# AssemblyAI-Community/MinImagen

Hardware: NVIDIA B200
Metric: denoising steps/sec (SR256 U-Net, batch 32 per GPU per step) (higher is better)
Workload: dtype f16 tensor-core operands, f32 accumulate / residual stream

## Files before the change

### include/minimagen_b200.h

```cpp
#ifndef MINIMAGEN_B200_H_
#define MINIMAGEN_B200_H_

#include <stdint.h>

#ifdef __cplusplus
extern "C" {
#endif

#define MI_ABI_VERSION 2

int mi_abi_version(void);
const char* mi_last_error(void);
int mi_device_ok(void);
int mi_set_launch_mode(int programmatic_dependent_launch);

int mi_pack_conv_weight_f16(const float* w_oihw, int c_out, int c_in, int kh, int kw, float scale, void* out_f16,
                            void* stream);

int mi_pack_conv_weight_dgrad_f16(const float* w_oihw, int c_out, int c_in, int kh, int kw, void* out_f16, void* stream);

int mi_conv2d_igemm_supported(int H, int W, int c_in, int c_out);
int mi_conv2d_igemm_f16(const void* act_f16, int B, int H, int W, int lda, int c_off, int c_in, const void* act2_f16,
                        int lda2, int c_off2, int c_in1, const void* w_f16, int c_out, int kh, int kw, int mode,
                        const float* bias, const float* residual, float* out_f32, void* out_f16, double* out_stats,
                        long long out_sb, long long out_sh, long long out_sw, long long out_sc, int n_valid,
                        int block_n, int* err_flag, void* workspace, long long workspace_bytes, void* stream);
int mi_conv3x3_res1x1_supported(int H, int W, int c_in, int c_out, int x_cin);
int mi_conv3x3_res1x1_f16(const void* act_f16, int B, int H, int W, int lda, int c_in, const void* act2_f16, int lda2,
                          int c_in1, const void* x_f16, int ldx, int x_cin, const void* x2_f16, int ldx2, int x_cin1,
                          const void* w_f16, int c_out, const float* bias, const float* residual, float* out_f32,
                          void* out_f16, double* out_stats, int* err_flag, void* stream);
long long mi_conv2d_igemm_workspace_bytes(void);

int mi_conv3x3_gn_supported(int H, int W, int c0, int c1, int c_out, int groups);
int mi_conv3x3_gn_silu_f16(const float* src0, int c0, const float* src1, int c1, float scale1, int B, int H, int W,
                           int groups, const double* stats0, const double* stats1, const float* gamma,
                           const float* beta, const float* scale_shift, int scale_shift_ld, float eps,
                           const void* w_f16, int c_out, const float* bias, const float* residual, float* out_f32,
                           void* out_f16, double* out_stats, int* err_flag, void* stream);

int mi_conv2d_direct_f32(const float* in, int B, int Hin, int Win, int c_in, int ldi, const float* w_oihw, int c_out,
                         int kh, int kw, int stride, int pad, const float* bias, const float* residual, float* out,
                         int Hout, int Wout, long long out_sb, long long out_sh, long long out_sw, long long out_sc,
                         void* stream);

int mi_gn_stats(const void* src0, int c0, const void* src1, int c1, float scale1, int in_is_f16, int B, int hw,
                int groups, double* sums, void* stream);
int mi_gn_apply_silu(const void* src0, int c0, const void* src1, int c1, float scale1, int in_is_f16, int B, int hw,
                     int groups, const double* stats0, int stats0_block, const double* stats1, int stats1_block,
                     const float* gamma, const float* beta, const float* scale_shift, int scale_shift_ld, float eps,
                     void* out, int out_is_f16, void* stream);
int mi_cast_act(const void* src0, int c0, const void* src1, int c1, float scale1, int in_is_f16, int B, int H, int W,
                int mode, void* out, int out_is_f16, void* stream);
int mi_ln_rows(const float* in, long long rows, int C, const float* gamma, const float* beta, float eps, int pre_gelu,
               const float* residual, float* out_f32, void* out_f16, void* stream);

int mi_linear_f32(const float* in, int M, int K, const float* W, const float* bias, int N, int in_act, int out_act,
                  const float* addend, float* out_f32, void* out_f16, float out_scale, void* stream);
int mi_sinusoidal_posemb(const long long* t, int B, int dim, float* out, void* stream);
int mi_text_tokens(const float* proj, int B, int L, int D, const uint8_t* mask, const uint8_t* keep,
                   const float* null_embed, int max_len, float* c_out, int m, int row_off, float* pooled,
                   void* stream);
int mi_place_rows(const float* src, int B, int r, int D, float* dst, int m, int row_off, void* stream);
int mi_select_rows(const float* a, const float* null_row, const uint8_t* keep, const float* addend, int B, int N,
                   float* out, void* stream);
int mi_nchw_to_nhwc(const float* a, int ca, const float* b, int cb, int B, int hw, int c_pad, float* out,
                    void* stream);

int mi_stem_unroll_f16(const float* a, int ca, const float* b, int cb, int B, int H, int W, void* out_f16,
                       void* stream);
int mi_silu_f32(const float* in, long long n, float* out, void* stream);

int mi_resize_separable(const float* in, long long planes, int h_in, int w_in, float* out, int h_out, int w_out,
                        const int* iy, const float* wy, int taps_y, const int* ix, const float* wx, int taps_x,
                        int has_clamp, float lo, float hi, void* stream);

long long mi_attention_workspace_bytes(int B, int heads, int kv_head_stride, int m);
int mi_attention_fwd(const void* q_f16, long long q_bs, int ldq, const void* k_f16, const void* v_f16, long long kv_bs,
                     int ldkv, int kv_head_stride, const float* null_kv, const uint8_t* key_mask, int B, int heads,
                     int n, int m, void* out_f16, long long o_bs, int ldo, void* workspace, long long workspace_bytes,
                     void* stream);

int mi_step_x0(const float* x_t, const float* eps_cond, const float* eps_null, float cond_scale, const long long* t,
               const float* sqrt_recip_alphas_cumprod, const float* sqrt_recipm1_alphas_cumprod, int B, int n,
               float* x0, void* stream);
int mi_step_quantile(const float* x0, int B, int n, int rank_lo, int rank_hi, float weight, float min_s, float* s,
                     void* stream);
int mi_step_posterior(const float* x0, const float* x_t, const float* noise, const float* s, const long long* t,
                      const float* posterior_mean_coef1, const float* posterior_mean_coef2, const float* sigma, int B,
                      int n, float* out, void* stream);
long long mi_step_epilogue_workspace_floats(int B, int n);
int mi_step_epilogue(const float* x_t, const float* eps_cond, const float* eps_null, float cond_scale, const long long* t,
                     const float* sqrt_recip_alphas_cumprod, const float* sqrt_recipm1_alphas_cumprod,
                     const float* posterior_mean_coef1, const float* posterior_mean_coef2, const float* sigma,
                     const float* noise, int B, int n, int rank_lo, int rank_hi, float weight, float min_s, float* out,
                     float* s_out, float* x0_workspace, void* stream);
int mi_step_advance_t(long long* t, int B, void* stream);
int mi_step_finalize(const float* x, long long n, int unnormalize, float* out, void* stream);
int mi_q_sample(const float* x0, const float* noise, const long long* t, const float* sqrt_alphas_cumprod,
                const float* sqrt_one_minus_alphas_cumprod, int B, int n, float post_scale, float post_shift,
                float* out, void* stream);


int mi_gemm_f32(const float* A, const float* B, float* C, int M, int N, int K, long long a_sm, long long a_sk,
                long long b_sk, long long b_sn, long long c_sm, long long c_sn, int Z1, int Z2, long long a_b1,
                long long a_b2, long long b_b1, long long b_b2, long long c_b1, long long c_b2, float alpha,
                int accumulate, void* stream);
int mi_colsum_f32(const float* x, long long M, int N, float* out, int accumulate, void* stream);
int mi_conv2d_dgrad_f32(const float* dy, int B, int Hout, int Wout, int c_out, const float* w_oihw, int c_in, int kh, int kw,
                        int stride, int pad, float* dx, int Hin, int Win, void* stream);
int mi_conv2d_wgrad_f32(const float* dy, const float* x, int B, int Hin, int Win, int c_in, int Hout, int Wout, int c_out,
                        int kh, int kw, int stride, int pad, float* dw, void* stream);
int mi_conv2d_wgrad_f16_supported(int Hout, int Wout, int c_in, int c_out, int kh, int kw, int stride);
long long mi_conv2d_wgrad_f16_workspace_bytes(int B, int Hout, int Wout, int c_in, int c_out, int kh, int kw, int stride);
int mi_conv2d_wgrad_f16(const void* dy_f16, const void* x_f16, int B, int Hout, int Wout, int c_in, int c_out, int kh, int kw,
                        int stride, float* dw, float* workspace, long long workspace_bytes, void* stream);
int mi_gn_silu_bwd(const float* x, const float* dy, const double* sums, int B, int hw, int C, int groups,
                   const float* gamma, const float* beta, const float* scale_shift, int scale_shift_ld, float eps,
                   float* dx, float* dgamma, float* dbeta, float* d_scale_shift, int d_scale_shift_ld, float* workspace,
                   void* stream);
int mi_ln_rows_bwd(const float* in, const float* dy, long long rows, int C, const float* gamma, float eps, int pre_gelu,
                   float* dx, float* dgamma, float* dbeta, void* stream);
int mi_softmax_rows(float* s, long long R, int L, void* stream);
int mi_softmax_rows_bwd(const float* P, float* dP, long long R, int L, void* stream);
int mi_upsample2x_bwd(const float* dy, int B, int H, int W, int C, float* dx, void* stream);

#ifdef __cplusplus
}
#endif
#endif
```

### minimagen_b200/Unet.py

```python
from typing import Union

import torch
from torch import nn

from .helpers import cast_tuple, default, exists, prob_mask_like
from .layers import (Attention, Cat, Context, Conv2d, CrossEmbedLayer, Downsample, Identity, Parallel, ResnetBlock,
                     SinusoidalPosEmb, TokenView, TransformerBlock, Upsample, _no_grad_check, _ResidualAttention)
from . import _native
from .ops import get_ops
from .t5 import get_encoded_dim

F32 = torch.float32


class Unet(nn.Module):
    def __init__(
            self,
            *,
            dim: int = 128,
            dim_mults: tuple = (1, 2, 4),
            channels: int = 3,
            channels_out: int = None,
            cond_dim: int = None,
            text_embed_dim=get_encoded_dim('t5_small'),
# ... 57 lines not shown

        self.skip_connect_scale = 2 ** -0.5
        self.downs = nn.ModuleList([])
        self.ups = nn.ModuleList([])
        layer_params = [num_resnet_blocks, resnet_groups, layer_attns, layer_cross_attns]
        reversed_layer_params = list(map(reversed, layer_params))

        skip_connect_dims = []
        for ind, ((dim_in, dim_out), n_blocks, groups, layer_attn, layer_cross_attn) in enumerate(
                zip(in_out, *layer_params)):
            is_last = ind == (num_resolutions - 1)
            layer_cond_dim = cond_dim if layer_cross_attn else None
            transformer_klass = TransformerBlock if layer_attn else Identity
            current_dim = dim_in
            pre_downsample = None
            if memory_efficient:
                pre_downsample = Downsample(dim_in, dim_out)
                current_dim = dim_out
            skip_connect_dims.append(current_dim)
            post_downsample = None
            if not memory_efficient:
                post_downsample = Downsample(current_dim, dim_out) if not is_last else Parallel(
                    Conv2d(dim_in, dim_out, 3, padding=1), Conv2d(dim_in, dim_out, 1))
            self.downs.append(nn.ModuleList([
                pre_downsample,
                ResnetBlock(current_dim, current_dim, cond_dim=layer_cond_dim, time_cond_dim=time_cond_dim,
                            groups=groups),
                nn.ModuleList([ResnetBlock(current_dim, current_dim, time_cond_dim=time_cond_dim, groups=groups)
                               for _ in range(n_blocks)]),
                transformer_klass(dim=current_dim, heads=attn_heads, dim_head=ATTN_DIM_HEAD),
                post_downsample,
            ]))

        mid_dim = dims[-1]
        self.mid_block1 = ResnetBlock(mid_dim, mid_dim, cond_dim=cond_dim, time_cond_dim=time_cond_dim,
                                      groups=resnet_groups[-1])
        self.mid_attn = TokenView(_ResidualAttention(
            Attention(mid_dim, heads=attn_heads, dim_head=ATTN_DIM_HEAD))) if attend_at_middle else None
        self.mid_block2 = ResnetBlock(mid_dim, mid_dim, cond_dim=cond_dim, time_cond_dim=time_cond_dim,
                                      groups=resnet_groups[-1])

        for ind, ((dim_in, dim_out), n_blocks, groups, layer_attn, layer_cross_attn) in enumerate(
                zip(reversed(in_out), *reversed_layer_params)):
            is_last = ind == (num_resolutions - 1)
            layer_cond_dim = cond_dim if layer_cross_attn else None
            transformer_klass = TransformerBlock if layer_attn else Identity
            skip_connect_dim = skip_connect_dims.pop()
            self.ups.append(nn.ModuleList([
                ResnetBlock(dim_out + skip_connect_dim, dim_out, cond_dim=layer_cond_dim,
                            time_cond_dim=time_cond_dim, groups=groups),
                nn.ModuleList([ResnetBlock(dim_out + skip_connect_dim, dim_out, time_cond_dim=time_cond_dim,
                                           groups=groups) for _ in range(n_blocks)]),
                transformer_klass(dim=dim_out, heads=attn_heads, dim_head=ATTN_DIM_HEAD),
                Upsample(dim_out, dim_in) if not is_last or memory_efficient else Identity()
            ]))

        self.init_conv_to_final_conv_residual = False
        self.final_res_block = ResnetBlock(dim, dim, time_cond_dim=time_cond_dim, groups=resnet_groups[0])
        self.final_conv = Conv2d(dim, self.channels_out, 3, padding=3 // 2)

    def _cast_model_parameters(self, *, lowres_cond, text_embed_dim, channels, channels_out):
        if lowres_cond == self.lowres_cond and channels == self.channels and \
                text_embed_dim == self.text_embed_dim and channels_out == self.channels_out:
            return self
        updated = dict(lowres_cond=lowres_cond, text_embed_dim=text_embed_dim, channels=channels,
                       channels_out=channels_out)
        return self.__class__(**{**self._locals, **updated})

    def forward(self, x, time, *, lowres_cond_img=None, lowres_noise_times=None, text_embeds=None, text_mask=None,
                cond_drop_prob: float = 0.):
        return self._forward_impl(x, time, lowres_cond_img=lowres_cond_img, lowres_noise_times=lowres_noise_times,
                                  text_embeds=text_embeds, text_mask=text_mask, cond_drop_prob=cond_drop_prob)

    def _forward_impl(self, x, *args, **kwargs):
        with _native.device_of(x):
            if torch.is_grad_enabled() and (x.requires_grad or any(p.requires_grad for p in self.parameters())):
                from .train_path import unet_forward_train
                return unet_forward_train(self, x, *args, **kwargs)
            return self._forward_dev(x, *args, **kwargs)

    def _forward_dev(self, x, time, *, lowres_cond_img=None, lowres_noise_times=None, text_embeds=None, text_mask=None,
                      cond_drop_prob: float = 0., cond_keep=None):
        assert not (self.lowres_cond and not exists(lowres_cond_img)), \
            'low resolution conditioning image must be present'
        assert not (self.lowres_cond and not exists(lowres_noise_times)), \
            'low resolution conditioning noise time must be present'
        B, Cx, H, W = x.shape
        device = x.device
        x = x.to(F32).contiguous()
        lowres = lowres_cond_img.to(F32).contiguous() if exists(lowres_cond_img) else None

        t, time_tokens = self._generate_t_tokens(time, lowres_noise_times)
        t, c = self._text_condition(text_embeds, B, cond_drop_prob, device, text_mask, t, time_tokens, cond_keep)
        ss = self._all_scale_shifts(t)

        out = torch.empty((B, self.channels_out, H, W), dtype=F32, device=device)
        chunks = self._batch_chunks(B, x.is_cuda)
        if len(chunks) == 1:
            self._forward_body(x, lowres, t, c, ss, out)
            return out
        main = torch.cuda.current_stream(device)
        streams = self._side_streams(len(chunks), device)
        for (b0, b1), s in zip(chunks, streams):
            s.wait_stream(main)
            with torch.cuda.stream(s):
                self._forward_body(x[b0:b1], lowres[b0:b1] if exists(lowres) else None, t[b0:b1], c[b0:b1],
                                   {k: v[b0:b1] for k, v in ss.items()}, out[b0:b1])
        for s in streams:
            main.wait_stream(s)
        return out

    batch_streams = 1
    min_chunk_batch = 8

    def _batch_chunks(self, B, is_cuda):
        n = self.batch_streams if is_cuda else 1
        while n > 1 and (B % n != 0 or B // n < self.min_chunk_batch):
            n -= 1
        per = B // n
        return [(i * per, (i + 1) * per) for i in range(n)]

    def _side_streams(self, n, device):
        key = (n, str(device))
        if getattr(self, "_streams_key", None) != key:
            self._streams = [torch.cuda.Stream(device=device) for _ in range(n)]
            self._streams_key = key
        return self._streams

    def _forward_body(self, x, lowres, t, c, ss, out):
        from . import layers as _layers
        ops = get_ops()
        B, _, H, W = x.shape
        device = x.device
        ctx = Context(c)
        n_res = sum(1 for m in self.modules() if isinstance(m, ResnetBlock))
        if x.is_cuda:
            _layers._ARENA = _layers.ZeroArena(device, B * (self.dim * max(8, 1)) // 8 * 4 * (2 * n_res + 8))
        try:
            return self._forward_body_impl(x, lowres, t, c, ss, out, ctx)
        finally:
            _layers._ARENA = None

    def _forward_body_impl(self, x, lowres, t, c, ss, out, ctx):
        ops = get_ops()
        B, _, H, W = x.shape
        device = x.device

        h = self.init_conv.run_stem(x, lowres)

        hiddens = []
        for pre_downsample, init_block, resnet_blocks, attn_block, post_downsample in self.downs:
            if exists(pre_downsample):
                h = pre_downsample.run(h)
            h = init_block.run(h, t, ctx, ss[init_block])
            for resnet_block in resnet_blocks:
                h = resnet_block.run(h, t, None, ss[resnet_block])
                hiddens.append(h)
            h = attn_block.run(h)
            hiddens.append(h)
            if exists(post_downsample):
                h = post_downsample.run(h)

        h = self.mid_block1.run(h, t, ctx, ss[self.mid_block1])
        if exists(self.mid_attn):
            h = self.mid_attn.run(h)
        h = self.mid_block2.run(h, t, ctx, ss[self.mid_block2])

        skip = lambda cur: Cat(cur, hiddens.pop(), self.skip_connect_scale)
        for init_block, resnet_blocks, attn_block, upsample in self.ups:
            h = init_block.run(skip(h), t, ctx, ss[init_block])
            for resnet_block in resnet_blocks:
                h = resnet_block.run(skip(h), t, None, ss[resnet_block])
            h = attn_block.run(h)
            h = upsample.run(h)

        h = self.final_res_block.run(h, t, None, ss[self.final_res_block], out_f32=False)

        fc = self.final_conv
        if ops.igemm_supported(H, W, fc.in_channels, 16):
            fc.run_prepared_nchw(h.need_f16(), B, H, W, out)
        else:
            fc.run_prepared_nchw(h.need_f32(), B, H, W, out)

    def _all_scale_shifts(self, t):
        from .layers import ResnetBlock
        ops = get_ops()
        blocks = [m for m in self.modules() if isinstance(m, ResnetBlock) and exists(m.time_mlp)]
        key = tuple((m.time_mlp[1].weight.data_ptr(), m.time_mlp[1].weight._version, m.time_mlp[1].bias._version)
                    for m in blocks)
        if getattr(self, "_tm_key", None) != key:
            self._tm_w = torch.cat([m.time_mlp[1].weight.detach() for m in blocks], dim=0).contiguous()
            self._tm_b = torch.cat([m.time_mlp[1].bias.detach() for m in blocks], dim=0).contiguous()
            self._tm_key = key
        B, tcd = t.shape
        total = self._tm_w.shape[0]
        st = torch.empty_like(t)
        ops.silu(t.contiguous(), st)
        buf = torch.empty((B, total), dtype=F32, device=t.device)
        ops.linear_f32(st, B, tcd, self._tm_w, self._tm_b, total, 0, 0, None, buf, None)
        out, off = {}, 0
        for m in blocks:
            n = m.time_mlp[1].out_features
            out[m] = buf[:, off:off + n]
            off += n
        return out

    def forward_with_cond_scale(self, *args, cond_scale: float = 1., **kwargs):
        logits = self.forward(*args, **kwargs)
        if cond_scale == 1:
            return logits
        null_logits = self.forward(*args, cond_drop_prob=1., **kwargs)
        return null_logits + (logits - null_logits) * cond_scale

    def _time_branch(self, times, hiddens_seq, cond_seq, tokens_seq, t_addend):
        ops = get_ops()
        B = times.shape[0]
        dev = times.device
        tcd, D, nt = self.time_cond_dim, self.cond_dim, self.num_time_tokens
        pos = hiddens_seq[0](times)
        lin = hiddens_seq[1]
        hid = torch.empty((B, tcd), dtype=F32, device=dev)
        ops.linear_f32(pos, B, lin.in_features, lin.weight, lin.bias, tcd, 0, 1, None, hid, None)
        lin = cond_seq[0]
        t = torch.empty((B, tcd), dtype=F32, device=dev)
        ops.linear_f32(hid, B, tcd, lin.weight, lin.bias, tcd, 0, 0, t_addend, t, None)
        lin = tokens_seq[0]
        tok = torch.empty((B, nt * D), dtype=F32, device=dev)
        ops.linear_f32(hid, B, tcd, lin.weight, lin.bias, nt * D, 0, 0, None, tok, None)
        return t, tok.reshape(B, nt, D)

    def _generate_t_tokens(self, time, lowres_noise_times):
        t, tokens = self._time_branch(time, self.to_time_hiddens, self.to_time_cond, self.to_time_tokens, None)
        if self.lowres_cond:
            t, lowres_tokens = self._time_branch(lowres_noise_times, self.to_lowres_time_hiddens,
                                                 self.to_lowres_time_cond, self.to_lowres_time_tokens, t)
            tokens = torch.cat((tokens, lowres_tokens), dim=-2)
        return t, tokens

    def _text_condition(self, text_embeds, batch_size, cond_drop_prob, device, text_mask, t, time_tokens, cond_keep=None):
        ops = get_ops()
        B, D, tcd = batch_size, self.cond_dim, self.time_cond_dim
        nt = time_tokens.shape[1]
        has_text = exists(text_embeds)
        m = nt + (self.max_text_len if has_text else 0)
        c_pre = torch.empty((B, m, D), dtype=F32, device=device)
        ops.place_rows(time_tokens.contiguous(), B, nt, D, c_pre, m, 0)
        if has_text:
            L, E = text_embeds.shape[1], text_embeds.shape[2]
            proj = self._static_text_proj(text_embeds)
            if proj is None:
                proj = torch.empty((B * L, D), dtype=F32, device=device)
                ops.linear_f32(text_embeds.to(F32).contiguous().reshape(B * L, E), B * L, E, self.text_to_cond.weight,
                               self.text_to_cond.bias, D, 0, 0, None, proj, None)
            keep = (cond_keep.to(device=device, dtype=torch.uint8).contiguous() if exists(cond_keep)
                    else prob_mask_like((B,), 1 - cond_drop_prob, device=device).to(torch.uint8))
            mask_u8 = text_mask.to(torch.uint8).contiguous() if exists(text_mask) else None
            pooled = torch.empty((B, D), dtype=F32, device=device)
            ops.text_tokens(proj, B, L, D, mask_u8, keep, self.null_text_embed.detach().reshape(self.max_text_len, D),
                            self.max_text_len, c_pre, m, nt, pooled)
            ln, lin1, _, lin2 = self.to_text_non_attn_cond
            pn = torch.empty((B, D), dtype=F32, device=device)
            ops.ln_rows(pooled, B, D, ln.weight, ln.bias, ln.eps, 0, None, pn, None)
            h1 = torch.empty((B, tcd), dtype=F32, device=device)
            ops.linear_f32(pn, B, D, lin1.weight, lin1.bias, tcd, 0, 1, None, h1, None)
            h2 = torch.empty((B, tcd), dtype=F32, device=device)
            ops.linear_f32(h1, B, tcd, lin2.weight, lin2.bias, tcd, 0, 0, None, h2, None)
            t_new = torch.empty((B, tcd), dtype=F32, device=device)
            ops.select_rows(h2, self.null_text_hidden.detach().reshape(tcd), keep, t, B, tcd, t_new)
            t = t_new
        c = torch.empty((B, m, D), dtype=F32, device=device)
        ops.ln_rows(c_pre.reshape(B * m, D), B * m, D, self.norm_cond.weight, self.norm_cond.bias, self.norm_cond.eps,
                    0, None, c.reshape(B * m, D), None)
        return t, c


    def register_static_text(self, text_embeds):
        ops = get_ops()
        B, L, E = text_embeds.shape
        cache = self.__dict__.setdefault("_static_text", {})
        entry = cache.get(text_embeds.data_ptr())
        buf = entry[0] if entry is not None and entry[0].shape == (B * L, self.cond_dim) else \
            torch.empty((B * L, self.cond_dim), dtype=F32, device=text_embeds.device)
        with _native.device_of(text_embeds):
            ops.linear_f32(text_embeds.reshape(B * L, E), B * L, E, self.text_to_cond.weight, self.text_to_cond.bias,
                           self.cond_dim, 0, 0, None, buf, None)
        cache[text_embeds.data_ptr()] = (buf, text_embeds._version, self.text_to_cond.weight._version)
        return buf

    def unregister_static_text(self, text_embeds=None):
        cache = self.__dict__.get("_static_text", {})
        if text_embeds is None:
            cache.clear()
        else:
            cache.pop(text_embeds.data_ptr(), None)

    def _static_text_proj(self, text_embeds):
        entry = self.__dict__.get("_static_text", {}).get(text_embeds.data_ptr())
        if entry is None or text_embeds.dtype != F32 or not text_embeds.is_contiguous():
            return None
        buf, version, wversion = entry
        B, L, _ = text_embeds.shape
        if version != text_embeds._version or wversion != self.text_to_cond.weight._version or buf.shape[0] != B * L:
            return None
        return buf


class Base(Unet):
    defaults = dict(
        dim=512,
        dim_mults=(1, 2, 3, 4),
# ... 51 lines not shown
```

### minimagen_b200/_native.py

```python
import ctypes
import os
from ctypes import c_char_p, c_float, c_int, c_longlong, c_void_p

import torch

_HERE = os.path.dirname(os.path.abspath(__file__))
LIB_PATH = os.path.join(_HERE, "lib", "libminimagen_b200.so")

_P, _I, _L, _F = c_void_p, c_int, c_longlong, c_float

SIGNATURES = {
    "mi_abi_version": [],
    "mi_last_error": [],
    "mi_device_ok": [],
    "mi_set_launch_mode": [_I],
    "mi_pack_conv_weight_f16": [_P, _I, _I, _I, _I, _F, _P, _P],
    "mi_pack_conv_weight_dgrad_f16": [_P, _I, _I, _I, _I, _P, _P],
    "mi_conv2d_igemm_supported": [_I, _I, _I, _I],
    "mi_conv2d_igemm_f16": [_P, _I, _I, _I, _I, _I, _I, _P, _I, _I, _I, _P, _I, _I, _I, _I, _P, _P, _P, _P, _P, _L, _L, _L, _L,
                            _I, _I, _P, _P, _L, _P],
    "mi_conv3x3_res1x1_supported": [_I, _I, _I, _I, _I],
    "mi_conv3x3_res1x1_f16": [_P, _I, _I, _I, _I, _I, _P, _I, _I, _P, _I, _I, _P, _I, _I, _P, _I, _P, _P, _P, _P, _P, _P, _P],
    "mi_conv2d_igemm_workspace_bytes": [],
    "mi_conv3x3_gn_supported": [_I, _I, _I, _I, _I, _I],
    "mi_conv3x3_gn_silu_f16": [_P, _I, _P, _I, _F, _I, _I, _I, _I, _P, _P, _P, _P, _P, _I, _F, _P, _I, _P, _P, _P, _P, _P, _P,
                               _P],
    "mi_conv2d_direct_f32": [_P, _I, _I, _I, _I, _I, _P, _I, _I, _I, _I, _I, _P, _P, _P, _I, _I, _L, _L, _L, _L, _P],
    "mi_gn_stats": [_P, _I, _P, _I, _F, _I, _I, _I, _I, _P, _P],
    "mi_gn_apply_silu": [_P, _I, _P, _I, _F, _I, _I, _I, _I, _P, _I, _P, _I, _P, _P, _P, _I, _F, _P, _I, _P],
    "mi_cast_act": [_P, _I, _P, _I, _F, _I, _I, _I, _I, _I, _P, _I, _P],
    "mi_ln_rows": [_P, _L, _I, _P, _P, _F, _I, _P, _P, _P, _P],
    "mi_linear_f32": [_P, _I, _I, _P, _P, _I, _I, _I, _P, _P, _P, _F, _P],
    "mi_sinusoidal_posemb": [_P, _I, _I, _P, _P],
    "mi_text_tokens": [_P, _I, _I, _I, _P, _P, _P, _I, _P, _I, _I, _P, _P],
    "mi_place_rows": [_P, _I, _I, _I, _P, _I, _I, _P],
    "mi_select_rows": [_P, _P, _P, _P, _I, _I, _P, _P],
    "mi_nchw_to_nhwc": [_P, _I, _P, _I, _I, _I, _I, _P, _P],
    "mi_stem_unroll_f16": [_P, _I, _P, _I, _I, _I, _I, _P, _P],
    "mi_resize_separable": [_P, _L, _I, _I, _P, _I, _I, _P, _P, _I, _P, _P, _I, _I, _F, _F, _P],
    "mi_silu_f32": [_P, _L, _P, _P],
    "mi_attention_workspace_bytes": [_I, _I, _I, _I],
    "mi_attention_fwd": [_P, _L, _I, _P, _P, _L, _I, _I, _P, _P, _I, _I, _I, _I, _P, _L, _I, _P, _L, _P],
    "mi_step_x0": [_P, _P, _P, _F, _P, _P, _P, _I, _I, _P, _P],
    "mi_step_quantile": [_P, _I, _I, _I, _I, _F, _F, _P, _P],
    "mi_step_posterior": [_P, _P, _P, _P, _P, _P, _P, _P, _I, _I, _P, _P],
    "mi_step_epilogue_workspace_floats": [_I, _I],
    "mi_step_epilogue": [_P, _P, _P, _F, _P, _P, _P, _P, _P, _P, _P, _I, _I, _I, _I, _F, _F, _P, _P, _P, _P],
    "mi_step_advance_t": [_P, _I, _P],
    "mi_step_finalize": [_P, _L, _I, _P, _P],
    "mi_q_sample": [_P, _P, _P, _P, _P, _I, _I, _F, _F, _P, _P],
    "mi_gemm_f32": [_P, _P, _P, _I, _I, _I, _L, _L, _L, _L, _L, _L, _I, _I, _L, _L, _L, _L, _L, _L, _F, _I, _P],
    "mi_colsum_f32": [_P, _L, _I, _P, _I, _P],
    "mi_conv2d_dgrad_f32": [_P, _I, _I, _I, _I, _P, _I, _I, _I, _I, _I, _P, _I, _I, _P],
    "mi_conv2d_wgrad_f32": [_P, _P, _I, _I, _I, _I, _I, _I, _I, _I, _I, _I, _I, _P, _P],
    "mi_conv2d_wgrad_f16_supported": [_I, _I, _I, _I, _I, _I, _I],
    "mi_conv2d_wgrad_f16_workspace_bytes": [_I, _I, _I, _I, _I, _I, _I, _I],
    "mi_conv2d_wgrad_f16": [_P, _P, _I, _I, _I, _I, _I, _I, _I, _I, _P, _P, _L, _P],
    "mi_gn_silu_bwd": [_P, _P, _P, _I, _I, _I, _I, _P, _P, _P, _I, _F, _P, _P, _P, _P, _I, _P, _P],
    "mi_ln_rows_bwd": [_P, _P, _L, _I, _P, _F, _I, _P, _P, _P, _P],
    "mi_softmax_rows": [_P, _L, _I, _P],
    "mi_softmax_rows_bwd": [_P, _P, _L, _I, _P],
    "mi_upsample2x_bwd": [_P, _I, _I, _I, _I, _P, _P],
}
_RESTYPES = {"mi_last_error": c_char_p, "mi_conv2d_igemm_workspace_bytes": c_longlong,
             "mi_attention_workspace_bytes": c_longlong, "mi_conv2d_wgrad_f16_workspace_bytes": c_longlong, "mi_step_epilogue_workspace_floats": c_longlong}

_lib = None
launch_count = 0


def load():
    global _lib
    if _lib is not None:
        return _lib
    if not os.path.exists(LIB_PATH):
        raise RuntimeError(
            f"minimagen_b200: native library not found at {LIB_PATH}. Build it with "
            f"`python -m minimagen_b200.build_ext` (or __graft_entry__.build()). There is no CPU fallback.")
    lib = ctypes.CDLL(LIB_PATH)
    for name, argtypes in SIGNATURES.items():
        fn = getattr(lib, name)
        fn.argtypes = argtypes
        fn.restype = _RESTYPES.get(name, c_int)
    if lib.mi_abi_version() != 2:
        raise RuntimeError("minimagen_b200: ABI version mismatch between _native.py and the shared library")
    _lib = lib
    return lib


def last_error():
    return load().mi_last_error().decode()


_FN = {}


def call(name, *args):
    global launch_count
    fn = _FN.get(name)
    if fn is None:
        fn = _FN[name] = getattr(load(), name)
    rc = fn(*args)
    if rc != 0:
        raise RuntimeError(f"minimagen_b200.{name} failed: {last_error()}")
    launch_count += 1
    return rc


_cur_dev = getattr(torch._C, "_cuda_getDevice", None) or torch.cuda.current_device
_raw_stream = getattr(torch._C, "_cuda_getCurrentRawStream", None)


def ptr(t):
    if t is None:
        return None
    d = t.get_device()
    if d < 0:
        raise RuntimeError("minimagen_b200: tensor is not on a CUDA device; the kernels have no CPU fallback")
    if d != _cur_dev():
        raise RuntimeError(
            f"minimagen_b200: tensor lives on {t.device} but the current CUDA device is cuda:{torch.cuda.current_device()}; "
            f"enter `torch.cuda.device(tensor.device)` (Unet.forward / Imagen.sample do this for their inputs)")
    return t.data_ptr()


def stream():
    if _raw_stream is not None:
        return _raw_stream(_cur_dev())
    return torch.cuda.current_stream().cuda_stream


def device_of(*tensors):
    for t in tensors:
        if t is not None and getattr(t, "is_cuda", False):
            return torch.cuda.device(t.device)
    import contextlib
    return contextlib.nullcontext()
```

### minimagen_b200/csrc/capi.cu

```cuda
#include "../../include/minimagen_b200.h"

#include <cuda_runtime.h>
#include <stdio.h>
#include <stdlib.h>
#include <string.h>
#include <string>

#include "conv_tc.cuh"
#include "kernels.cuh"

namespace {

thread_local char g_err[256] = "ok";

int fail(int code, const char* what) {
    snprintf(g_err, sizeof(g_err), "%s (code %d)", what, code);
    return code;
}
int check(int rc, const char* fn) {
    if (rc == 0) return 0;
    if (rc == -1) return fail(rc, (std::string(fn) + ": unsupported shape / alignment").c_str());
    if (rc == -2) {
        cudaError_t e = cudaGetLastError();
        return fail(rc, (std::string(fn) + ": kernel launch failed: " + cudaGetErrorString(e)).c_str());
    }
    return fail(rc, (std::string(fn) + ": error").c_str());
}
inline cudaStream_t S(void* s) { return reinterpret_cast<cudaStream_t>(s); }

}

namespace mi {
static bool g_pdl = false;
bool pdl_enabled() { return g_pdl; }
}

extern "C" {

int mi_abi_version(void) { return MI_ABI_VERSION; }
int mi_set_launch_mode(int programmatic_dependent_launch) {
    mi::g_pdl = programmatic_dependent_launch != 0;
    return 0;
}
const char* mi_last_error(void) { return g_err; }

int mi_device_ok(void) {
    int dev = 0, major = 0;
    if (cudaGetDevice(&dev) != cudaSuccess) return 0;
    if (cudaDeviceGetAttribute(&major, cudaDevAttrComputeCapabilityMajor, dev) != cudaSuccess) return 0;
    return major == 10;
}

int mi_pack_conv_weight_dgrad_f16(const float* w, int c_out, int c_in, int kh, int kw, void* out, void* stream) {
    return check(mi::pack_conv_weight_dgrad(w, c_out, c_in, kh, kw, (__half*)out, S(stream)), "mi_pack_conv_weight_dgrad_f16");
}
int mi_pack_conv_weight_f16(const float* w, int c_out, int c_in, int kh, int kw, float scale, void* out, void* stream) {
    return check(mi::pack_conv_weight(w, c_out, c_in, kh, kw, scale, (__half*)out, S(stream)), "mi_pack_conv_weight_f16");
}

int mi_conv2d_igemm_supported(int H, int W, int c_in, int c_out) { return mi::conv_tc_supported(H, W, c_in, c_out) ? 1 : 0; }

static int igemm_common(const void* act, int B, int H, int W, int lda, int c_off, int c_in, const void* act2, int lda2,
                        int c_off2, int c_in1, const void* w, int c_out, int kh, int kw, int mode, const float* bias,
                        const float* residual, float* out_f32, void* out_f16, double* out_stats, long long out_sb,
                        long long out_sh, long long out_sw, long long out_sc, int n_valid, int block_n, int* err_flag,
                        void* workspace, long long workspace_bytes, const void* x_act, int ldx, int x_off, int x_cin,
                        const void* x_act2, int ldx2, int x_off2, int x_cin1, void* stream) {
    mi::ConvTcProblem p{};
    p.x_act = x_act; p.x_lda = ldx; p.x_chan_off = x_off; p.Cx = x_cin;
    p.x_act2 = x_act2; p.x_lda2 = ldx2; p.x_chan_off2 = x_off2; p.Cx1 = x_cin1;
    if (x_act && !(mode == 0 && kh == 3 && kw == 3)) return fail(-9, "mi_conv3x3_res1x1_f16: the folded 1x1 operand needs a 3x3 stride-1 conv");
    (void)workspace; (void)workspace_bytes;
    p.act = act; p.B = B; p.H = H; p.W = W; p.lda = lda; p.a_channels = lda; p.a_chan_off = c_off; p.Cin = c_in;
    p.wpacked = w; p.Cout = c_out;
    p.act2 = act2; p.lda2 = lda2; p.a_chan_off2 = c_off2; p.Cin1 = c_in1; p.stats = out_stats;
    if (out_stats && (out_sc > 1 || (c_out % 32) != 0)) return fail(-8, "mi_conv2d_igemm_f16: out_stats needs channel-contiguous output and c_out % 32 == 0");
    if (out_stats && ((long long)H * W) % 32 != 0)
        return fail(-8, "mi_conv2d_igemm_f16: out_stats needs H*W % 32 == 0 (a warp's 32 output rows must belong to one image)");
    p.out_f32 = out_f32; p.out_f16 = (__half*)out_f16; p.bias = bias; p.residual = residual;
    p.out_sb = out_sb; p.out_sh = out_sh; p.out_sw = out_sw; p.out_sc = out_sc; p.n_valid = n_valid;
    p.block_n_hint = block_n; p.err_flag = err_flag;
    if (mode == 0) {
        if (!(kh & 1) || !(kw & 1) || kh * kw > mi::kConvMaxTaps) return fail(-4, "mi_conv2d_igemm_f16: mode 0 needs odd kh,kw with kh*kw <= 16");
        p.phases = 1; p.num_taps = kh * kw;
        for (int r = 0; r < kh; ++r)
            for (int s = 0; s < kw; ++s) {
                const int t = r * kw + s;
                p.dh[t] = (int8_t)(r - kh / 2); p.dw[t] = (int8_t)(s - kw / 2); p.ph[t] = 0;
            }
    } else if (mode == 1) {
        if (kh != 4 || kw != 4) return fail(-4, "mi_conv2d_igemm_f16: mode 1 is the 4x4 stride-2 pad-1 conv");
        p.phases = 4; p.num_taps = 16;
        for (int r = 0; r < 4; ++r)
            for (int s = 0; s < 4; ++s) {
                const int t = r * 4 + s, rr = r - 1, ss = s - 1;
                p.dh[t] = (int8_t)(rr < 0 ? -1 : (rr >> 1)); p.dw[t] = (int8_t)(ss < 0 ? -1 : (ss >> 1));
                p.ph[t] = (int8_t)((rr & 1) * 2 + (ss & 1));
            }
    } else if (mode == 6) {
        if (kh != 4 || kw != 4) return fail(-4, "mi_conv2d_igemm_f16: mode 6 is the 4x4 stride-2 pad-1 conv");
        if (act2) return fail(-4, "mi_conv2d_igemm_f16: mode 6 takes one activation tensor");
        p.phases = 1; p.num_taps = 16; p.in_stride = 2;
        for (int r = 0; r < 4; ++r)
            for (int s = 0; s < 4; ++s) {
                const int t = r * 4 + s;
                p.dh[t] = (int8_t)(r - 1); p.dw[t] = (int8_t)(s - 1); p.ph[t] = 0;
            }
    } else if (mode >= 2 && mode <= 5) {
        if (kh != 2 || kw != 2) return fail(-4, "mi_conv2d_igemm_f16: modes 2..5 take the 2x2 phase kernel");
        const int a = (mode - 2) >> 1, b = (mode - 2) & 1;
        p.phases = 1; p.num_taps = 4;
        for (int r = 0; r < 2; ++r)
            for (int s = 0; s < 2; ++s) {
                const int t = r * 2 + s;
                p.dh[t] = (int8_t)(a - 1 + r); p.dw[t] = (int8_t)(b - 1 + s); p.ph[t] = 0;
            }
    } else {
        return fail(-4, "mi_conv2d_igemm_f16: unknown mode");
    }
    if (out_sc <= 1 && ((out_sw % 4) || (out_sh % 4) || (out_sb % 4)))
        return fail(-8, "mi_conv2d_igemm_f16: channel-contiguous output strides must be multiples of 4 elements");
    if (out_sc > 1 && residual) return fail(-8, "mi_conv2d_igemm_f16: residual needs channel-contiguous output");
    p.halo = (mode == 0 && kh == 3 && kw == 3) ? 1 : ((mode == 0 && kh == 15 && kw == 1) ? 3 : 0);
    if (mode >= 2 && mode <= 5 && !getenv("MI_SUBPIX_PAIR")) p.halo = 4;
    const int rc = mi::conv_tc_launch(p, S(stream));
    if (rc != 0) return fail(rc, mi::conv_tc_strerror(rc));
    return 0;
}

int mi_conv2d_igemm_f16(const void* act, int B, int H, int W, int lda, int c_off, int c_in, const void* act2, int lda2,
                        int c_off2, int c_in1, const void* w, int c_out, int kh, int kw, int mode, const float* bias,
                        const float* residual, float* out_f32, void* out_f16, double* out_stats, long long out_sb,
                        long long out_sh, long long out_sw, long long out_sc, int n_valid, int block_n, int* err_flag,
                        void* workspace, long long workspace_bytes, void* stream) {
    return igemm_common(act, B, H, W, lda, c_off, c_in, act2, lda2, c_off2, c_in1, w, c_out, kh, kw, mode, bias, residual,
                        out_f32, out_f16, out_stats, out_sb, out_sh, out_sw, out_sc, n_valid, block_n, err_flag, workspace,
                        workspace_bytes, nullptr, 0, 0, 0, nullptr, 0, 0, 0, stream);
}

int mi_conv3x3_res1x1_supported(int H, int W, int c_in, int c_out, int x_cin) {
    const bool t16 = W == 16 && H % 16 == 0, t32 = !t16 && H % 32 == 0 && W % 8 == 0;
    return (t16 || t32) && c_in > 0 && c_in % 64 == 0 && x_cin > 0 && x_cin % 64 == 0 && c_out % 128 == 0;
}

int mi_conv3x3_res1x1_f16(const void* act, int B, int H, int W, int lda, int c_in, const void* act2, int lda2, int c_in1,
                          const void* x_act, int ldx, int x_cin, const void* x_act2, int ldx2, int x_cin1, const void* w,
                          int c_out, const float* bias, const float* residual, float* out_f32, void* out_f16,
                          double* out_stats, int* err_flag, void* stream) {
    if (!mi_conv3x3_res1x1_supported(H, W, c_in, c_out, x_cin))
        return fail(-9, "mi_conv3x3_res1x1_f16: unsupported geometry (see mi_conv3x3_res1x1_supported)");
    return igemm_common(act, B, H, W, lda, 0, c_in, act2, lda2, 0, c_in1, w, c_out, 3, 3, 0, bias, residual, out_f32, out_f16,
                        out_stats, (long long)H * W * c_out, (long long)W * c_out, c_out, 1, 0, 0, err_flag, nullptr, 0, x_act,
                        ldx, 0, x_cin, x_act2, ldx2, 0, x_cin1, stream);
}

long long mi_conv2d_igemm_workspace_bytes(void) { return 0; }

int mi_conv3x3_gn_supported(int H, int W, int c0, int c1, int c_out, int groups) {
    return mi::conv_gn_supported(H, W, c0, c1, c_out, groups) ? 1 : 0;
}

int mi_conv3x3_gn_silu_f16(const float* src0, int c0, const float* src1, int c1, float scale1, int B, int H, int W,
                           int groups, const double* stats0, const double* stats1, const float* gamma,
                           const float* beta, const float* scale_shift, int scale_shift_ld, float eps, const void* w,
                           int c_out, const float* bias, const float* residual, float* out_f32, void* out_f16,
                           double* out_stats, int* err_flag, void* stream) {
    mi::ConvGnProblem p{};
    p.src0 = src0; p.C0 = c0; p.src1 = src1; p.C1 = c1; p.scale1 = scale1; p.B = B; p.H = H; p.W = W; p.groups = groups;
    p.stats0 = stats0; p.stats1 = stats1; p.gamma = gamma; p.beta = beta; p.scale_shift = scale_shift;
    p.ss_ld = scale_shift_ld; p.eps = eps; p.wpacked = w; p.Cout = c_out; p.bias = bias; p.residual = residual;
    p.out_f32 = out_f32; p.out_f16 = (__half*)out_f16; p.out_stats = out_stats; p.err_flag = err_flag;
    if (scale_shift && scale_shift_ld < 2 * (c0 + c1)) return fail(-8, "mi_conv3x3_gn_silu_f16: scale_shift_ld < 2*C");
    const bool pair = mi::conv_gn_pair_supported(H, W, c0, c1, c_out, groups) && !getenv("MI_GN_NO_PAIR");
    const int rc = pair ? mi::conv_gn_pair_launch(p, S(stream)) : mi::conv_gn_launch(p, S(stream));
    if (rc != 0) return fail(rc, rc == -3 ? "mi_conv3x3_gn_silu_f16: unsupported geometry (see mi_conv3x3_gn_supported)"
                                          : mi::conv_tc_strerror(rc));
    return 0;
}

int mi_conv2d_direct_f32(const float* in, int B, int Hin, int Win, int c_in, int ldi, const float* w, int c_out, int kh,
                         int kw, int stride, int pad, const float* bias, const float* residual, float* out, int Hout,
                         int Wout, long long out_sb, long long out_sh, long long out_sw, long long out_sc,
                         void* stream) {
    return check(mi::conv_direct_f32(in, B, Hin, Win, c_in, ldi, w, c_out, kh, kw, stride, pad, bias, residual, out,
                                     Hout, Wout, out_sb, out_sh, out_sw, out_sc, S(stream)),
                 "mi_conv2d_direct_f32");
}

int mi_gn_stats(const void* src0, int c0, const void* src1, int c1, float scale1, int in_is_f16, int B, int hw,
                int groups, double* sums, void* stream) {
    return check(mi::gn_stats(src0, c0, src1, c1, scale1, in_is_f16, B, hw, groups, sums, S(stream)), "mi_gn_stats");
}
int mi_gn_apply_silu(const void* src0, int c0, const void* src1, int c1, float scale1, int in_is_f16, int B, int hw,
                     int groups, const double* stats0, int stats0_block, const double* stats1, int stats1_block,
                     const float* gamma, const float* beta, const float* scale_shift, int scale_shift_ld, float eps,
                     void* out, int out_is_f16, void* stream) {
    return check(mi::gn_apply_silu(src0, c0, src1, c1, scale1, in_is_f16, B, hw, groups, stats0, stats0_block, stats1,
                                   stats1_block, gamma, beta, scale_shift, scale_shift_ld, eps, out, out_is_f16,
                                   S(stream)),
                 "mi_gn_apply_silu");
}
int mi_cast_act(const void* src0, int c0, const void* src1, int c1, float scale1, int in_is_f16, int B, int H, int W,
                int mode, void* out, int out_is_f16, void* stream) {
    return check(mi::cast_act(src0, c0, src1, c1, scale1, in_is_f16, B, H, W, mode, out, out_is_f16, S(stream)),
                 "mi_cast_act");
}
int mi_ln_rows(const float* in, long long rows, int C, const float* gamma, const float* beta, float eps, int pre_gelu,
               const float* residual, float* out_f32, void* out_f16, void* stream) {
    return check(mi::ln_rows(in, rows, C, gamma, beta, eps, pre_gelu, residual, out_f32, (__half*)out_f16, S(stream)),
                 "mi_ln_rows");
}
int mi_linear_f32(const float* in, int M, int K, const float* W, const float* bias, int N, int in_act, int out_act,
                  const float* addend, float* out_f32, void* out_f16, float out_scale, void* stream) {
    return check(mi::linear_f32(in, M, K, W, bias, N, in_act, out_act, addend, out_f32, (__half*)out_f16, out_scale,
                                S(stream)),
                 "mi_linear_f32");
}
int mi_sinusoidal_posemb(const long long* t, int B, int dim, float* out, void* stream) {
    return check(mi::posemb(t, B, dim, out, S(stream)), "mi_sinusoidal_posemb");
}
int mi_text_tokens(const float* proj, int B, int L, int D, const uint8_t* mask, const uint8_t* keep,
                   const float* null_embed, int max_len, float* c_out, int m, int row_off, float* pooled, void* stream) {
    return check(mi::text_tokens(proj, B, L, D, mask, keep, null_embed, max_len, c_out, m, row_off, pooled, S(stream)),
                 "mi_text_tokens");
}
int mi_place_rows(const float* src, int B, int r, int D, float* dst, int m, int row_off, void* stream) {
    return check(mi::place_rows(src, B, r, D, dst, m, row_off, S(stream)), "mi_place_rows");
}
int mi_select_rows(const float* a, const float* null_row, const uint8_t* keep, const float* addend, int B, int N,
                   float* out, void* stream) {
    return check(mi::select_rows(a, null_row, keep, addend, B, N, out, S(stream)), "mi_select_rows");
}
int mi_nchw_to_nhwc(const float* a, int ca, const float* b, int cb, int B, int hw, int c_pad, float* out, void* stream) {
    return check(mi::nchw_to_nhwc(a, ca, b, cb, B, hw, c_pad, out, S(stream)), "mi_nchw_to_nhwc");
}
int mi_stem_unroll_f16(const float* a, int ca, const float* b, int cb, int B, int H, int W, void* out, void* stream) {
    return check(mi::stem_unroll(a, ca, b, cb, B, H, W, (__half*)out, S(stream)), "mi_stem_unroll_f16");
}
int mi_resize_separable(const float* in, long long planes, int h_in, int w_in, float* out, int h_out, int w_out,
                        const int* iy, const float* wy, int taps_y, const int* ix, const float* wx, int taps_x,
                        int has_clamp, float lo, float hi, void* stream) {
    return check(mi::resize_sep(in, planes, h_in, w_in, out, h_out, w_out, iy, wy, taps_y, ix, wx, taps_x, has_clamp, lo, hi,
                                S(stream)),
                 "mi_resize_separable");
}
int mi_silu_f32(const float* in, long long n, float* out, void* stream) {
    return check(mi::silu_f32(in, n, out, S(stream)), "mi_silu_f32");
}
long long mi_attention_workspace_bytes(int B, int heads, int kv_head_stride, int m) {
    return mi::attention_tc_workspace_bytes(B, heads, kv_head_stride, m);
}
int mi_attention_fwd(const void* q, long long q_bs, int ldq, const void* k, const void* v, long long kv_bs, int ldkv,
                     int kv_head_stride, const float* null_kv, const uint8_t* key_mask, int B, int heads, int n, int m,
                     void* out, long long o_bs, int ldo, void* workspace, long long workspace_bytes, void* stream) {
    if (workspace && m >= 128 && mi::attention_tc_supported(n, ldq, ldo, q_bs, key_mask) &&
        workspace_bytes >= mi::attention_tc_workspace_bytes(B, heads, kv_head_stride, m))
        return check(mi::attention_tc_fwd((const __half*)q, q_bs, ldq, (const __half*)k, (const __half*)v, kv_bs, ldkv,
                                          kv_head_stride, null_kv, key_mask, B, heads, n, m, (__half*)out, o_bs, ldo, workspace,
                                          workspace_bytes, nullptr, S(stream)),
                     "mi_attention_fwd (tcgen05)");
    return check(mi::attention_fwd((const __half*)q, q_bs, ldq, (const __half*)k, (const __half*)v, kv_bs, ldkv,
                                   kv_head_stride, null_kv, key_mask, B, heads, n, m, (__half*)out, o_bs, ldo, S(stream)),
                 "mi_attention_fwd");
}
int mi_step_x0(const float* x_t, const float* eps_cond, const float* eps_null, float cond_scale, const long long* t,
               const float* tab_a, const float* tab_b, int B, int n, float* x0, void* stream) {
    return check(mi::step_x0(x_t, eps_cond, eps_null, cond_scale, t, tab_a, tab_b, B, n, x0, S(stream)), "mi_step_x0");
}
int mi_step_quantile(const float* x0, int B, int n, int rank_lo, int rank_hi, float weight, float min_s, float* s,
                     void* stream) {
    return check(mi::step_quantile(x0, B, n, rank_lo, rank_hi, weight, min_s, s, S(stream)), "mi_step_quantile");
}
int mi_step_posterior(const float* x0, const float* x_t, const float* noise, const float* s, const long long* t,
                      const float* c1, const float* c2, const float* sigma, int B, int n, float* out, void* stream) {
    return check(mi::step_posterior(x0, x_t, noise, s, t, c1, c2, sigma, B, n, out, S(stream)), "mi_step_posterior");
}
long long mi_step_epilogue_workspace_floats(int B, int n) {
    return mi::step_epilogue_fused_ok(n) ? 0 : (long long)B * n;
}
int mi_step_epilogue(const float* x_t, const float* eps_cond, const float* eps_null, float cond_scale, const long long* t,
                     const float* tab_a, const float* tab_b, const float* c1, const float* c2, const float* sigma,
                     const float* noise, int B, int n, int rank_lo, int rank_hi, float weight, float min_s, float* out,
                     float* s_out, float* x0_workspace, void* stream) {
    return check(mi::step_epilogue(x_t, eps_cond, eps_null, cond_scale, t, tab_a, tab_b, c1, c2, sigma, noise, B, n, rank_lo,
                                   rank_hi, weight, min_s, out, s_out, x0_workspace, S(stream)),
                 "mi_step_epilogue");
}
int mi_step_advance_t(long long* t, int B, void* stream) {
    return check(mi::step_advance_t(t, B, S(stream)), "mi_step_advance_t");
}
int mi_step_finalize(const float* x, long long n, int unnormalize, float* out, void* stream) {
    return check(mi::step_finalize(x, n, unnormalize, out, S(stream)), "mi_step_finalize");
// ... 63 lines not shown
```

### minimagen_b200/csrc/conv_tc.cu

```cuda
#include "conv_tc.cuh"

#include <cuda_runtime.h>
#include <mutex>
#include <stdio.h>

#include "conv_epilogue.cuh"
#include "kernels.cuh"
#include "ptx.cuh"
#include "launch.cuh"
#include "sat_half.cuh"

namespace mi {

namespace {

constexpr int kNumThreads = 128 + 32 * 8;
constexpr uint32_t kABytes = kConvBlockM * kConvBlockK * 2;
constexpr uint32_t kRingBudget = 192 * 1024;

template <int BLOCK_N>
struct Cfg {
    static constexpr uint32_t kBBytes = BLOCK_N * kConvBlockK * 2;
    static constexpr uint32_t kStageBytes = kABytes + kBBytes;
    static constexpr int kStages = (kRingBudget / kStageBytes) > 8 ? 8 : (kRingBudget / kStageBytes);
// ... 393 lines not shown

    if (warp == 0 && lane == 0) {
        ptx::prefetch_tensormap(&tmA);
        ptx::prefetch_tensormap(&tmB);
    }
    if (warp == 1 && lane == 0) {
        for (int i = 0; i < NA; ++i) { ptx::mbar_init(&fullA[i], 1); ptx::mbar_init(&emptyA[i], 1); }
        for (int i = 0; i < NBB; ++i) { ptx::mbar_init(&fullB[i], 1); ptx::mbar_init(&emptyB[i], 1); }
        for (int i = 0; i < 2; ++i) { ptx::mbar_init(&tfull_bar[i], 1); ptx::mbar_init(&tempty_bar[i], 32 * kEpiWarps); }
        ptx::fence_barrier_init();
    }
    if (warp == 2) {
        ptx::tmem_alloc(tmem_ptr_smem, C::kTmemCols);
        ptx::tmem_relinquish();
    }
    ptx::tc_fence_before();
    __syncthreads();
    ptx::tc_fence_after();
    const uint32_t tmem_base = *tmem_ptr_smem;
    pdl_wait();

    const int chunks = args.chunks_per_tap;
    const int tiles_m = args.tiles_w * args.tiles_h * args.tiles_b;
    const int total_tiles = tiles_m * args.tiles_n;
    const int Cin = chunks * kConvBlockK;

    if (warp == 0) {
        int sa = 0, sb = 0;
        uint32_t pa = 0, pb = 0;
        if constexpr (C::kBRes) {
            if (ptx::elect_one()) {
                ptx::mbar_arrive_expect_tx(&fullB[0], 9 * chunks * C::kBBytes);
                for (int j = 0; j < chunks; ++j)
                    for (int t = 0; t < 9; ++t)
                        ptx::tma_load_2d(&tmB, &fullB[0], smem_b + (j * 9 + t) * C::kBBytes, t * Cin + j * kConvBlockK, 0);
            }
        }
        for (int tile = blockIdx.x; tile < total_tiles; tile += gridDim.x) {
            const int nt = tile % args.tiles_n;
            const int mt = tile / args.tiles_n;
            const int w0 = (mt % args.tiles_w) * kHaloTW;
            const int h0 = ((mt / args.tiles_w) % args.tiles_h) * kHaloTH;
            const int b0 = mt / (args.tiles_w * args.tiles_h);
            const int n0 = nt * BLOCK_N;
            for (int j = 0; j < chunks; ++j) {
                ptx::mbar_wait(&emptyA[sa], pa ^ 1, err, 2100 + sa);
                if (ptx::elect_one()) {
                    ptx::mbar_arrive_expect_tx(&fullA[sa], kHaloABytes);
                    ptx::tma_load_5d(&tmA, &fullA[sa], smem + sa * kHaloAStride, args.a_chan_off + j * kConvBlockK,
                                     w0 - 1, h0 - 1, 0, b0);
                }
                if (++sa == NA) { sa = 0; pa ^= 1; }
                if constexpr (!C::kBRes) {
                    for (int t = 0; t < 9; ++t) {
                        ptx::mbar_wait(&emptyB[sb], pb ^ 1, err, 2200 + sb);
                        if (ptx::elect_one()) {
                            ptx::mbar_arrive_expect_tx(&fullB[sb], C::kBBytes);
                            ptx::tma_load_2d(&tmB, &fullB[sb], smem_b + sb * C::kBBytes, t * Cin + j * kConvBlockK, n0);
                        }
                        if (++sb == NB) { sb = 0; pb ^= 1; }
                    }
                }
            }
        }
        pdl_trigger();
    } else if (warp == 1) {
        constexpr uint32_t idesc = ptx::make_idesc_f16(kConvBlockM, BLOCK_N, 0);
        int sa = 0, sb = 0;
        uint32_t pa = 0, pb = 0;
        int iter = 0;
        if constexpr (C::kBRes) ptx::mbar_wait(&fullB[0], 0, err, 2500);
        for (int tile = blockIdx.x; tile < total_tiles; tile += gridDim.x, ++iter) {
            const int as = iter & 1;
            const uint32_t aphase = (iter >> 1) & 1;
            ptx::mbar_wait(&tempty_bar[as], aphase ^ 1, err, 2300 + as);
            ptx::tc_fence_after();
            const uint32_t tmem_d = tmem_base + as * BLOCK_N;
            for (int j = 0; j < chunks; ++j) {
                ptx::mbar_wait(&fullA[sa], pa, err, 2400 + sa);
                const uint32_t a_base = ptx::smem_u32(smem + sa * kHaloAStride);
                for (int t = 0; t < 9; ++t) {
                    if constexpr (C::kBRes) sb = j * 9 + t;
                    else ptx::mbar_wait(&fullB[sb], pb, err, 2500 + sb);
                    ptx::tc_fence_after();
                    if (ptx::elect_one()) {
                        const uint32_t a_win = a_base + ((t / 3) * kHaloW + (t % 3)) * 128;
                        const uint64_t da = make_halo_desc(a_win);
                        const uint64_t db = ptx::make_kmajor_sw128_desc(ptx::smem_u32(smem_b + sb * C::kBBytes));
#pragma unroll
                        for (int k = 0; k < kConvBlockK / 16; ++k)
                            ptx::umma_f16(tmem_d, da + 2 * k, db + 2 * k, idesc, (j | t | k) != 0);
                        if constexpr (!C::kBRes) ptx::umma_commit(&emptyB[sb]);
                    }
                    if constexpr (!C::kBRes) {
                        if (++sb == NB) { sb = 0; pb ^= 1; }
                    }
                }
                if (ptx::elect_one()) ptx::umma_commit(&emptyA[sa]);
                if (++sa == NA) { sa = 0; pa ^= 1; }
            }
            if (ptx::elect_one()) ptx::umma_commit(&tfull_bar[as]);
        }
    } else if (warp >= 4) {
        const int ew = warp & 3;
        const int c_half = BLOCK_N / 2;
        const int c_begin = warp >= 8 ? c_half : 0;
        const int c_end = c_begin + c_half;
        const int m = ew * 32 + lane;
        const int bw = m & (kHaloTW - 1);
        const int bh = m >> 3;
        int iter = 0;
        for (int tile = blockIdx.x; tile < total_tiles; tile += gridDim.x, ++iter) {
            const int nt = tile % args.tiles_n;
            const int mt = tile / args.tiles_n;
            const int w = (mt % args.tiles_w) * kHaloTW + bw;
            const int h = ((mt / args.tiles_w) % args.tiles_h) * kHaloTH + bh;
            const int b = mt / (args.tiles_w * args.tiles_h);
            const int n0 = nt * BLOCK_N;
            const bool valid = (b < args.B) && (h < args.H) && (w < args.W);
            const long long pix = (long long)b * args.out_sb + (long long)h * args.out_sh + (long long)w * args.out_sw;
            const int as = iter & 1;
            const uint32_t aphase = (iter >> 1) & 1;
            ptx::mbar_wait(&tfull_bar[as], aphase, err, 2600 + as);
            ptx::tc_fence_after();
            const uint32_t taddr = tmem_base + (static_cast<uint32_t>(ew * 32) << 16) + as * BLOCK_N;
            epilogue_tile<BLOCK_N>(args, taddr, n0, pix, valid, epi_stage, c_begin, c_end, b);
            ptx::tc_fence_before();
            ptx::mbar_arrive(&tempty_bar[as]);
        }
    }
    ptx::tc_fence_before();
    __syncthreads();
    if (warp == 2) {
        ptx::tc_fence_after();
        ptx::tmem_dealloc(tmem_base, C::kTmemCols);
    }
}

constexpr int kHtPix = 256;
enum { kG32x8 = 0, kG16x16 = 1, kGV15 = 2, kGSub = 4 };
template <int G>
struct CfgT {
    static constexpr bool kW16 = G == kG16x16;
    static constexpr int kTaps = G == kGV15 ? 15 : (G == kGSub ? 4 : 9);
    static constexpr int kTH = kW16 ? 16 : 32, kTW = kW16 ? 16 : 8;
    static constexpr int kBoxH = G == kGV15 ? kTH + 14 : (G == kGSub ? kTH + 1 : kTH + 2);
    static constexpr int kBoxW = G == kG32x8 ? 10 : (kW16 ? 16 : (G == kGSub ? 9 : 8));
    static constexpr uint32_t kHaloBytes = kBoxH * kBoxW * 128;
    static constexpr uint32_t kHaloStride = (kHaloBytes + 1023) & ~1023u;
    static constexpr uint32_t kWBytes = 128 * kConvBlockK * 2;
    static constexpr int kHStages = kW16 ? 3 : 2;
    static constexpr int kWStages = (kRingBudget - kHStages * kHaloStride) / kWBytes;
    static constexpr uint32_t kTmemCols = 2 * kHtPix;
    static constexpr uint32_t kSmemBytes = kHStages * kHaloStride + kWStages * kWBytes + 1024 + 256;
};

__device__ __forceinline__ uint64_t make_halo_t_desc(uint32_t smem_addr, uint32_t sbo_bytes) {
    uint64_t d = 0;
    d |= static_cast<uint64_t>((smem_addr >> 4) & 0x3FFF);
    d |= static_cast<uint64_t>(sbo_bytes >> 4) << 32;
    d |= static_cast<uint64_t>(1) << 46;
    d |= static_cast<uint64_t>(2) << 61;
    return d;
}

template <int G>
__global__ void __launch_bounds__(kNumThreads, 1)
conv3x3_halo_t_kernel(const __grid_constant__ CUtensorMap tmA, const __grid_constant__ CUtensorMap tmA2,
                      const __grid_constant__ CUtensorMap tmB, const __grid_constant__ CUtensorMap tmX,
                      const __grid_constant__ CUtensorMap tmX2, const __grid_constant__ ConvTcArgs args) {
    using C = CfgT<G>;
    constexpr bool kW16 = C::kW16;
    constexpr int NH = C::kHStages, NW = C::kWStages;
    constexpr int kLoads = kW16 ? 3 : 1;
    constexpr int kTapsPerLoad = C::kTaps / kLoads;
    extern __shared__ uint8_t smem_raw[];
    uint8_t* smem = reinterpret_cast<uint8_t*>((reinterpret_cast<uintptr_t>(smem_raw) + 1023) & ~uintptr_t(1023));
    uint8_t* smem_w = smem + NH * C::kHaloStride;
    uint64_t* bars = reinterpret_cast<uint64_t*>(smem_w + NW * C::kWBytes);
    uint64_t* fullH = bars;
    uint64_t* emptyH = bars + NH;
    uint64_t* fullW = bars + 2 * NH;
    uint64_t* emptyW = bars + 2 * NH + NW;
    uint64_t* tfull_bar = bars + 2 * NH + 2 * NW;
    uint64_t* tempty_bar = tfull_bar + 2;
    uint32_t* tmem_ptr_smem = reinterpret_cast<uint32_t*>(tempty_bar + 2);
    static_assert((2 * NH + 2 * NW + 4) * 8 + 8 <= 256, "barrier block too large");

    const int warp = threadIdx.x >> 5;
    const int lane = threadIdx.x & 31;
    int* err = args.err_flag;

    if (warp == 0 && lane == 0) {
        ptx::prefetch_tensormap(&tmA);
        ptx::prefetch_tensormap(&tmB);
    }
    if (warp == 1 && lane == 0) {
        for (int i = 0; i < NH; ++i) { ptx::mbar_init(&fullH[i], 1); ptx::mbar_init(&emptyH[i], 1); }
        for (int i = 0; i < NW; ++i) { ptx::mbar_init(&fullW[i], 1); ptx::mbar_init(&emptyW[i], 1); }
        for (int i = 0; i < 2; ++i) { ptx::mbar_init(&tfull_bar[i], 1); ptx::mbar_init(&tempty_bar[i], 32 * kEpiWarps); }
        ptx::fence_barrier_init();
    }
    if (warp == 2) {
        ptx::tmem_alloc(tmem_ptr_smem, C::kTmemCols);
        ptx::tmem_relinquish();
    }
    ptx::tc_fence_before();
    __syncthreads();
    ptx::tc_fence_after();
    const uint32_t tmem_base = *tmem_ptr_smem;
    pdl_wait();

    const int chunks = args.chunks_per_tap;
    const int tiles_m = args.tiles_w * args.tiles_h * args.tiles_b;
    const int total_tiles = tiles_m * args.tiles_n;
    const int Cin = chunks * kConvBlockK;

    if (warp == 0) {
        int sh = 0, sw = 0;
        uint32_t ph = 0, pw = 0;
        for (int tile = blockIdx.x; tile < total_tiles; tile += gridDim.x) {
            const int nt = tile % args.tiles_n;
            const int mt = tile / args.tiles_n;
            const int w0 = (mt % args.tiles_w) * C::kTW;
            const int h0 = ((mt / args.tiles_w) % args.tiles_h) * C::kTH;
            const int b0 = mt / (args.tiles_w * args.tiles_h);
            const int n0 = nt * 128;
            for (int j = 0; j < chunks; ++j) {
                for (int l = 0; l < kLoads; ++l) {
                    ptx::mbar_wait(&emptyH[sh], ph ^ 1, err, 3100 + sh);
                    if (ptx::elect_one()) {
                        const int wc = kW16 ? w0 + l - 1 : (G == kGV15 ? w0 : (G == kGSub ? w0 + args.dw[0] : w0 - 1));
                        const int hc = G == kGV15 ? h0 - 7 : (G == kGSub ? h0 + args.dh[0] : h0 - 1);
                        ptx::mbar_arrive_expect_tx(&fullH[sh], C::kHaloBytes);
                        if (j < args.a_split)
                            ptx::tma_load_5d(&tmA, &fullH[sh], smem + sh * C::kHaloStride,
                                             args.a_chan_off + j * kConvBlockK, wc, hc, 0, b0);
                        else
                            ptx::tma_load_5d(&tmA2, &fullH[sh], smem + sh * C::kHaloStride,
                                             args.a_chan_off2 + (j - args.a_split) * kConvBlockK, wc, hc, 0, b0);
                    }
                    if (++sh == NH) { sh = 0; ph ^= 1; }
                    for (int u = 0; u < kTapsPerLoad; ++u) {
                        const int t = kW16 ? u * 3 + l : u;
                        ptx::mbar_wait(&emptyW[sw], pw ^ 1, err, 3200 + sw);
                        if (ptx::elect_one()) {
                            ptx::mbar_arrive_expect_tx(&fullW[sw], C::kWBytes);
                            ptx::tma_load_2d(&tmB, &fullW[sw], smem_w + sw * C::kWBytes, t * Cin + j * kConvBlockK, n0);
                        }
                        if (++sw == NW) { sw = 0; pw ^= 1; }
                    }
                }
            }
            if constexpr (G == kG32x8 || G == kG16x16) {
                for (int jx = 0; jx < args.x_chunks; ++jx) {
                    ptx::mbar_wait(&emptyH[sh], ph ^ 1, err, 3150 + sh);
                    if (ptx::elect_one()) {
                        ptx::mbar_arrive_expect_tx(&fullH[sh], C::kHaloBytes);
                        if (jx < args.x_split)
                            ptx::tma_load_5d(&tmX, &fullH[sh], smem + sh * C::kHaloStride, args.x_chan_off + jx * kConvBlockK,
                                             kW16 ? w0 : w0 - 1, h0 - 1, 0, b0);
                        else
                            ptx::tma_load_5d(&tmX2, &fullH[sh], smem + sh * C::kHaloStride,
                                             args.x_chan_off2 + (jx - args.x_split) * kConvBlockK, kW16 ? w0 : w0 - 1, h0 - 1, 0, b0);
                    }
                    if (++sh == NH) { sh = 0; ph ^= 1; }
                    ptx::mbar_wait(&emptyW[sw], pw ^ 1, err, 3250 + sw);
                    if (ptx::elect_one()) {
                        ptx::mbar_arrive_expect_tx(&fullW[sw], C::kWBytes);
                        ptx::tma_load_2d(&tmB, &fullW[sw], smem_w + sw * C::kWBytes, C::kTaps * Cin + jx * kConvBlockK, n0);
                    }
                    if (++sw == NW) { sw = 0; pw ^= 1; }
                }
            }
        }
        pdl_trigger();
    } else if (warp == 1) {
        constexpr uint32_t idesc = ptx::make_idesc_f16(128, kHtPix, 0);
        int sh = 0, sw = 0;
        uint32_t ph = 0, pw = 0;
        int iter = 0;
        for (int tile = blockIdx.x; tile < total_tiles; tile += gridDim.x, ++iter) {
            const int as = iter & 1;
            const uint32_t aphase = (iter >> 1) & 1;
            ptx::mbar_wait(&tempty_bar[as], aphase ^ 1, err, 3300 + as);
            ptx::tc_fence_after();
            const uint32_t tmem_d = tmem_base + as * kHtPix;
            for (int j = 0; j < chunks; ++j) {
                for (int l = 0; l < kLoads; ++l) {
                    ptx::mbar_wait(&fullH[sh], ph, err, 3400 + sh);
                    const uint32_t h_base = ptx::smem_u32(smem + sh * C::kHaloStride);
                    for (int u = 0; u < kTapsPerLoad; ++u) {
                        ptx::mbar_wait(&fullW[sw], pw, err, 3500 + sw);
                        ptx::tc_fence_after();
                        if (ptx::elect_one()) {
                            const uint64_t da = ptx::make_kmajor_sw128_desc(ptx::smem_u32(smem_w + sw * C::kWBytes));
                            const uint64_t db = kW16 ? make_halo_t_desc(h_base + u * 16 * 128, 1024)
                                : (G == kGV15 ? make_halo_t_desc(h_base + u * 8 * 128, 1024)
                                : G == kGSub ? make_halo_t_desc(h_base + ((u >> 1) * C::kBoxW + (u & 1)) * 128, C::kBoxW * 128)
                                              : make_halo_t_desc(h_base + ((u / 3) * C::kBoxW + (u % 3)) * 128, C::kBoxW * 128));
#pragma unroll
                            for (int k = 0; k < kConvBlockK / 16; ++k)
                                ptx::umma_f16(tmem_d, da + 2 * k, db + 2 * k, idesc, (j | l | u | k) != 0);
                            ptx::umma_commit(&emptyW[sw]);
                        }
                        if (++sw == NW) { sw = 0; pw ^= 1; }
                    }
                    if (ptx::elect_one()) ptx::umma_commit(&emptyH[sh]);
                    if (++sh == NH) { sh = 0; ph ^= 1; }
                }
            }
            if constexpr (G == kG32x8 || G == kG16x16) {
                for (int jx = 0; jx < args.x_chunks; ++jx) {
                    ptx::mbar_wait(&fullH[sh], ph, err, 3450 + sh);
                    const uint32_t h_base = ptx::smem_u32(smem + sh * C::kHaloStride);
                    ptx::mbar_wait(&fullW[sw], pw, err, 3550 + sw);
                    ptx::tc_fence_after();
                    if (ptx::elect_one()) {
                        const uint64_t da = ptx::make_kmajor_sw128_desc(ptx::smem_u32(smem_w + sw * C::kWBytes));
                        const uint64_t db = kW16 ? make_halo_t_desc(h_base + 16 * 128, 1024)
                                                 : make_halo_t_desc(h_base + (C::kBoxW + 1) * 128, C::kBoxW * 128);
#pragma unroll
                        for (int k = 0; k < kConvBlockK / 16; ++k) ptx::umma_f16(tmem_d, da + 2 * k, db + 2 * k, idesc, 1);
                        ptx::umma_commit(&emptyW[sw]);
                        ptx::umma_commit(&emptyH[sh]);
                    }
                    if (++sw == NW) { sw = 0; pw ^= 1; }
                    if (++sh == NH) { sh = 0; ph ^= 1; }
                }
            }
            if (ptx::elect_one()) ptx::umma_commit(&tfull_bar[as]);
        }
    } else if (warp >= 4) {
        constexpr int kTwLog2 = kW16 ? 4 : 3;
        const int q = warp & 3;
        const int half = warp >= 8 ? 1 : 0;
        int iter = 0;
        for (int tile = blockIdx.x; tile < total_tiles; tile += gridDim.x, ++iter) {
            const int nt = tile % args.tiles_n;
            const int mt = tile / args.tiles_n;
            const int w0 = (mt % args.tiles_w) * C::kTW;
            const int h0 = ((mt / args.tiles_w) % args.tiles_h) * C::kTH;
            const int b = mt / (args.tiles_w * args.tiles_h);
            const int n = nt * 128 + q * 32 + lane;
            const float bias_v = args.bias ? __ldg(args.bias + n) : 0.f;
            const long long base = (long long)b * args.out_sb + (long long)(h0 + half * (C::kTH / 2)) * args.out_sh +
                                   (long long)w0 * args.out_sw + n;
            const int as = iter & 1;
            const uint32_t aphase = (iter >> 1) & 1;
            ptx::mbar_wait(&tfull_bar[as], aphase, err, 3600 + as);
            ptx::tc_fence_after();
            const uint32_t taddr = tmem_base + (static_cast<uint32_t>(q * 32) << 16) + as * kHtPix + half * 128;
            float st_s = 0.f, st_q = 0.f;
#pragma unroll 1
            for (int c = 0; c < 128; c += 32) {
                uint32_t v0[16], v1[16];
                ptx::tmem_ld_x16(taddr + c, v0);
                ptx::tmem_ld_x16(taddr + c + 16, v1);
                const long long rowb = base + (long long)(c >> kTwLog2) * args.out_sh;
                float r[32];
                if (args.residual) {
#pragma unroll
                    for (int i = 0; i < 32; ++i)
                        r[i] = args.residual[rowb + (long long)(i >> kTwLog2) * args.out_sh +
                                             (long long)(i & (C::kTW - 1)) * args.out_sw];
                }
                ptx::tmem_ld_wait();
#pragma unroll
                for (int i = 0; i < 32; ++i) {
                    float f = __uint_as_float(i < 16 ? v0[i] : v1[i - 16]) + bias_v;
                    if (args.residual) f += r[i];
                    st_s += f;
                    st_q += f * f;
                    const long long o = rowb + (long long)(i >> kTwLog2) * args.out_sh +
                                        (long long)(i & (C::kTW - 1)) * args.out_sw;
                    if (args.out_f32) args.out_f32[o] = f;
                    if (args.out_f16) args.out_f16[o] = sat_half(f);
                }
            }
            if (args.stats) {
#pragma unroll
                for (int o = 1; o <= 8; o <<= 1) {
                    st_s += __shfl_xor_sync(0xffffffffu, st_s, o);
                    st_q += __shfl_xor_sync(0xffffffffu, st_q, o);
                }
                if ((lane & 15) == 0) {
                    double* dst = args.stats + ((long long)b * args.stats_blocks + (n >> 4)) * 2;
                    atomicAdd(dst, (double)st_s);
                    atomicAdd(dst + 1, (double)st_q);
                }
            }
            ptx::tc_fence_before();
            ptx::mbar_arrive(&tempty_bar[as]);
        }
    }
    ptx::tc_fence_before();
    __syncthreads();
    if (warp == 2) {
        ptx::tc_fence_after();
        ptx::tmem_dealloc(tmem_base, C::kTmemCols);
    }
}


typedef CUresult (*PFN_encodeTiled)(CUtensorMap*, CUtensorMapDataType, cuuint32_t, void*, const cuuint64_t*,
                                    const cuuint64_t*, const cuuint32_t*, const cuuint32_t*, CUtensorMapInterleave,
                                    CUtensorMapSwizzle, CUtensorMapL2promotion, CUtensorMapFloatOOBfill);

PFN_encodeTiled get_encode() {
    static PFN_encodeTiled fn = nullptr;
    static std::once_flag once;
    std::call_once(once, [] {
        void* p = nullptr;
        cudaDriverEntryPointQueryResult q;
        if (cudaGetDriverEntryPoint("cuTensorMapEncodeTiled", &p, cudaEnableDefault, &q) == cudaSuccess &&
            q == cudaDriverEntryPointSuccess)
            fn = reinterpret_cast<PFN_encodeTiled>(p);
    });
    return fn;
}

int ilog2_exact(int v) {
    int l = 0;
    while ((1 << l) < v) ++l;
    return ((1 << l) == v) ? l : -1;
}

template <int BLOCK_N>
int launch(const CUtensorMap& tmA, const CUtensorMap& tmA2, const CUtensorMap& tmB, const ConvTcArgs& args,
           int total_tiles, int num_sms, cudaStream_t stream) {
    using C = Cfg<BLOCK_N>;
    static bool attr_set = false;
    if (!attr_set) {
        cudaError_t e = cudaFuncSetAttribute(conv_tc_kernel<BLOCK_N>, cudaFuncAttributeMaxDynamicSharedMemorySize,
                                             C::kSmemBytes);
        if (e != cudaSuccess) return -10;
        attr_set = true;
    }
    const int grid = total_tiles < num_sms ? total_tiles : num_sms;
    launch_k(conv_tc_kernel<BLOCK_N>, grid, kNumThreads, C::kSmemBytes, stream, tmA, tmA2, tmB, args);
    return cudaGetLastError() == cudaSuccess ? 0 : -11;
}

template <int BLOCK_N, int KC>
int launch2(const CUtensorMap& tmA, const CUtensorMap& tmA2, const CUtensorMap& tmB, const ConvTcArgs& args,
            int total_pairs, int num_sms, cudaStream_t stream) {
    using C = Cfg2<BLOCK_N, KC>;
    static bool attr_set = false;
    if (!attr_set) {
        if (cudaFuncSetAttribute(conv_tc2_kernel<BLOCK_N, KC>, cudaFuncAttributeMaxDynamicSharedMemorySize, C::kSmemBytes) !=
            cudaSuccess)
            return -10;
        attr_set = true;
    }
    int clusters = num_sms / 2;
    if (clusters > total_pairs) clusters = total_pairs;
    launch_k(conv_tc2_kernel<BLOCK_N, KC>, 2 * clusters, kNumThreads, C::kSmemBytes, stream, tmA, tmA2, tmB, args);
    return cudaGetLastError() == cudaSuccess ? 0 : -11;
}

template <int BLOCK_N>
int launch_halo(const CUtensorMap& tmA, const CUtensorMap& tmB, const ConvTcArgs& args, int total_tiles, int num_sms,
                cudaStream_t stream) {
    using C = CfgH<BLOCK_N>;
    static bool attr_set = false;
    if (!attr_set) {
        if (cudaFuncSetAttribute(conv3x3_halo_kernel<BLOCK_N>, cudaFuncAttributeMaxDynamicSharedMemorySize,
                                 C::kSmemBytes) != cudaSuccess)
            return -10;
        attr_set = true;
    }
    const int grid = total_tiles < num_sms ? total_tiles : num_sms;
    launch_k(conv3x3_halo_kernel<BLOCK_N>, grid, kNumThreads, C::kSmemBytes, stream, tmA, tmB, args);
    return cudaGetLastError() == cudaSuccess ? 0 : -11;
}

template <int G>
int launch_halo_t(const CUtensorMap& tmA, const CUtensorMap& tmA2, const CUtensorMap& tmB, const CUtensorMap& tmX,
                  const CUtensorMap& tmX2, const ConvTcArgs& args, int total_tiles, int num_sms, cudaStream_t stream) {
    using C = CfgT<G>;
    static bool attr_set = false;
    if (!attr_set) {
        if (cudaFuncSetAttribute(conv3x3_halo_t_kernel<G>, cudaFuncAttributeMaxDynamicSharedMemorySize,
                                 C::kSmemBytes) != cudaSuccess)
            return -10;
        attr_set = true;
    }
    const int grid = total_tiles < num_sms ? total_tiles : num_sms;
    launch_k(conv3x3_halo_t_kernel<G>, grid, kNumThreads, C::kSmemBytes, stream, tmA, tmA2, tmB, tmX, tmX2, args);
    return cudaGetLastError() == cudaSuccess ? 0 : -11;
}

}

PFN_tmaEncodeTiled get_tma_encode() { return get_encode(); }

const char* conv_tc_strerror(int code) {
    switch (code) {
        case 0: return "ok";
        case -1: return "conv_tc: C_in (per tap) must be a positive multiple of 64";
        case -2: return "conv_tc: C_out must be a multiple of 16";
        case -3: return "conv_tc: W must be a power of two >= 8 or a multiple of 128; H*W tiling unsupported";
        case -4: return "conv_tc: too many taps (max 16)";
        case -5: return "conv_tc: cuTensorMapEncodeTiled unavailable";
        case -6: return "conv_tc: tensor map encode failed (activations)";
        case -7: return "conv_tc: tensor map encode failed (weights)";
        case -8: return "conv_tc: pointer/stride alignment (16 B) violated";
        case -9: return "conv_tc: folded 1x1 operand needs the swapped-operand 3x3 kernel (C_out % 128, H % 32 / W % 8 or 16x16 tiles)";
        case -10: return "conv_tc: cudaFuncSetAttribute(max dynamic smem) failed";
        case -11: return "conv_tc: kernel launch failed";
        default: return "conv_tc: unknown error";
    }
}

bool conv_tc_supported(int H, int W, int Cin, int Cout) {
    if (Cin <= 0 || Cin % kConvBlockK != 0 || Cout <= 0 || Cout % 16 != 0) return false;
    if (W >= 128) return true;
    if (ilog2_exact(W) < 3) return false;
    const int bh = 128 / W;
    if (H >= bh) return H % bh == 0;
    return ilog2_exact(H) >= 0;
}

int conv_tc_launch(const ConvTcProblem& p, cudaStream_t stream) {
    if (p.Cin <= 0 || p.Cin % kConvBlockK != 0) return -1;
    if (p.Cout % 16 != 0) return -2;
    if (p.num_taps < 1 || p.num_taps > kConvMaxTaps) return -4;
    if (!conv_tc_supported(p.H, p.W, p.Cin, p.Cout)) return -3;
    if ((reinterpret_cast<uintptr_t>(p.act) & 15) || (reinterpret_cast<uintptr_t>(p.wpacked) & 15) ||
        (p.lda % 8) != 0)
        return -8;
    PFN_encodeTiled enc = get_encode();
    if (!enc) return -5;

    const bool t16 = p.W == 16 && p.H % 16 == 0;
    const bool t32 = !t16 && p.H % 32 == 0 && p.W % 8 == 0;
    const bool v15 = p.halo == 3 && p.num_taps == 15 && t32 && !p.act2;
    const bool sub = p.halo == 4 && p.num_taps == 4 && t32 && !p.act2 && !p.x_act;
    if (p.halo && p.halo != 2 && (v15 || sub || (p.halo != 3 && p.halo != 4 && p.num_taps == 9)) && p.phases == 1 && (t16 || t32) &&
        p.Cout % 128 == 0 && p.out_sc <= 1 && (p.n_valid == 0 || p.n_valid == p.Cout) && p.dbg == 0) {
        bool canon = true;
        if (v15) for (int t = 0; t < 15; ++t) canon = canon && p.dh[t] == t - 7 && p.dw[t] == 0 && p.ph[t] == 0;
        else if (sub) for (int t = 0; t < 4; ++t) canon = canon && p.dh[t] == p.dh[0] + (t >> 1) && p.dw[t] == p.dw[0] + (t & 1) && p.ph[t] == 0;
        else for (int t = 0; t < 9; ++t) canon = canon && p.dh[t] == t / 3 - 1 && p.dw[t] == t % 3 - 1 && p.ph[t] == 0;
        if (p.act2 && (p.Cin1 <= 0 || p.Cin1 % kConvBlockK || p.Cin1 >= p.Cin || (p.lda2 % 8) ||
                       (reinterpret_cast<uintptr_t>(p.act2) & 15)))
            return -8;
        if (canon) {
            ConvTcArgs h{};
            h.num_taps = p.num_taps; h.chunks_per_tap = p.Cin / kConvBlockK;
            h.tiles_w = t16 ? 1 : p.W / 8; h.tiles_h = t16 ? p.H / 16 : p.H / 32; h.tiles_b = p.B; h.tiles_n = p.Cout / 128;
            h.B = p.B; h.H = p.H; h.W = p.W; h.a_chan_off = p.a_chan_off;
            h.a_split = (p.act2 ? p.Cin1 : p.Cin) / kConvBlockK; h.a_chan_off2 = p.a_chan_off2;
            h.out_sb = p.out_sb; h.out_sh = p.out_sh; h.out_sw = p.out_sw; h.out_sc = 1; h.n_valid = p.Cout;
            h.out_f32 = p.out_f32; h.out_f16 = p.out_f16; h.bias = p.bias; h.residual = p.residual; h.err_flag = p.err_flag;
            h.stats = p.stats; h.stats_blocks = p.Cout / 16;
            h.dh[0] = p.dh[0]; h.dw[0] = p.dw[0];
            int dev = 0, num_sms = 148;
            cudaGetDevice(&dev);
            cudaDeviceGetAttribute(&num_sms, cudaDevAttrMultiProcessorCount, dev);
            CUtensorMap tmA, tmA2, tmB;
            cuuint32_t box[5] = {kConvBlockK, (cuuint32_t)(t16 ? 16 : (v15 ? 8 : (sub ? 9 : 10))),
                                 (cuuint32_t)(t16 ? 18 : (v15 ? 46 : (sub ? 33 : 34))), 1, 1};
            cuuint32_t estr[5] = {1, 1, 1, 1, 1};
            {
                cuuint64_t gdim[5] = {(cuuint64_t)p.a_channels, (cuuint64_t)p.W, (cuuint64_t)p.H, 1, (cuuint64_t)p.B};
                cuuint64_t gstr[4] = {(cuuint64_t)p.lda * 2, (cuuint64_t)p.W * p.lda * 2, (cuuint64_t)p.H * p.W * p.lda * 2,
                                      (cuuint64_t)p.H * p.W * p.lda * 2};
                if (enc(&tmA, CU_TENSOR_MAP_DATA_TYPE_FLOAT16, 5, const_cast<void*>(p.act), gdim, gstr, box, estr,
                        CU_TENSOR_MAP_INTERLEAVE_NONE, CU_TENSOR_MAP_SWIZZLE_128B, CU_TENSOR_MAP_L2_PROMOTION_L2_256B,
                        CU_TENSOR_MAP_FLOAT_OOB_FILL_NONE) != CUDA_SUCCESS)
                    return -6;
            }
            tmA2 = tmA;
            if (p.act2) {
                cuuint64_t gdim[5] = {(cuuint64_t)p.lda2, (cuuint64_t)p.W, (cuuint64_t)p.H, 1, (cuuint64_t)p.B};
                cuuint64_t gstr[4] = {(cuuint64_t)p.lda2 * 2, (cuuint64_t)p.W * p.lda2 * 2, (cuuint64_t)p.H * p.W * p.lda2 * 2,
                                      (cuuint64_t)p.H * p.W * p.lda2 * 2};
                if (enc(&tmA2, CU_TENSOR_MAP_DATA_TYPE_FLOAT16, 5, const_cast<void*>(p.act2), gdim, gstr, box, estr,
                        CU_TENSOR_MAP_INTERLEAVE_NONE, CU_TENSOR_MAP_SWIZZLE_128B, CU_TENSOR_MAP_L2_PROMOTION_L2_256B,
                        CU_TENSOR_MAP_FLOAT_OOB_FILL_NONE) != CUDA_SUCCESS)
                    return -6;
            }
            CUtensorMap tmX = tmA, tmX2 = tmA;
            if (p.x_act) {
                if (v15 || p.Cx <= 0 || p.Cx % kConvBlockK || (p.x_lda % 8) || (reinterpret_cast<uintptr_t>(p.x_act) & 15)) return -8;
                if (p.x_act2 && (p.Cx1 <= 0 || p.Cx1 % kConvBlockK || p.Cx1 >= p.Cx || (p.x_lda2 % 8) ||
                                 (reinterpret_cast<uintptr_t>(p.x_act2) & 15)))
                    return -8;
                h.x_chunks = p.Cx / kConvBlockK;
                h.x_split = (p.x_act2 ? p.Cx1 : p.Cx) / kConvBlockK;
                h.x_chan_off = p.x_chan_off; h.x_chan_off2 = p.x_chan_off2;
                for (int which = 0; which < (p.x_act2 ? 2 : 1); ++which) {
                    const void* ptr = which ? p.x_act2 : p.x_act;
                    const cuuint64_t ld = which ? p.x_lda2 : p.x_lda;
                    cuuint64_t gdim[5] = {ld, (cuuint64_t)p.W, (cuuint64_t)p.H, 1, (cuuint64_t)p.B};
                    cuuint64_t gstr[4] = {ld * 2, (cuuint64_t)p.W * ld * 2, (cuuint64_t)p.H * p.W * ld * 2,
                                          (cuuint64_t)p.H * p.W * ld * 2};
                    if (enc(which ? &tmX2 : &tmX, CU_TENSOR_MAP_DATA_TYPE_FLOAT16, 5, const_cast<void*>(ptr), gdim, gstr, box, estr,
                            CU_TENSOR_MAP_INTERLEAVE_NONE, CU_TENSOR_MAP_SWIZZLE_128B, CU_TENSOR_MAP_L2_PROMOTION_L2_256B,
                            CU_TENSOR_MAP_FLOAT_OOB_FILL_NONE) != CUDA_SUCCESS)
                        return -6;
                }
                if (!p.x_act2) tmX2 = tmX;
            }
            const cuuint64_t K = (cuuint64_t)p.num_taps * p.Cin + (p.x_act ? (cuuint64_t)p.Cx : 0);
            cuuint64_t wdim[2] = {K, (cuuint64_t)p.Cout};
            cuuint64_t wstr[1] = {K * 2};
            cuuint32_t wbox[2] = {kConvBlockK, 128};
            cuuint32_t westr[2] = {1, 1};
            if (enc(&tmB, CU_TENSOR_MAP_DATA_TYPE_FLOAT16, 2, const_cast<void*>(p.wpacked), wdim, wstr, wbox, westr,
                    CU_TENSOR_MAP_INTERLEAVE_NONE, CU_TENSOR_MAP_SWIZZLE_128B, CU_TENSOR_MAP_L2_PROMOTION_L2_256B,
                    CU_TENSOR_MAP_FLOAT_OOB_FILL_NONE) != CUDA_SUCCESS)
                return -7;
            const int total = h.tiles_w * h.tiles_h * h.tiles_b * h.tiles_n;
            if (v15) return launch_halo_t<kGV15>(tmA, tmA2, tmB, tmX, tmX2, h, total, num_sms, stream);
            if (sub) return launch_halo_t<kGSub>(tmA, tmA2, tmB, tmX, tmX2, h, total, num_sms, stream);
            return t16 ? launch_halo_t<kG16x16>(tmA, tmA2, tmB, tmX, tmX2, h, total, num_sms, stream)
                       : launch_halo_t<kG32x8>(tmA, tmA2, tmB, tmX, tmX2, h, total, num_sms, stream);
        }
    }

    if (p.x_act) return -9;

    if (p.halo && !p.act2 && p.num_taps == 9 && p.phases == 1 && p.H % kHaloTH == 0 && p.W % kHaloTW == 0 &&
        ((p.Cout % 128 == 0 && (p.halo == 2 || p.Cout % 256 != 0)) ||
         (p.Cout == 16 && p.Cin <= kHaloResChunks * kConvBlockK))) {
        bool canon = true;
        for (int t = 0; t < 9; ++t) canon = canon && p.dh[t] == t / 3 - 1 && p.dw[t] == t % 3 - 1 && p.ph[t] == 0;
        if (canon) {
            ConvTcArgs h{};
            h.num_taps = 9; h.chunks_per_tap = p.Cin / kConvBlockK;
            h.tiles_w = p.W / kHaloTW; h.tiles_h = p.H / kHaloTH; h.tiles_b = p.B;
            h.B = p.B; h.H = p.H; h.W = p.W; h.a_chan_off = p.a_chan_off;
            h.out_sb = p.out_sb; h.out_sh = p.out_sh; h.out_sw = p.out_sw;
            h.out_sc = p.out_sc > 0 ? p.out_sc : 1; h.n_valid = p.n_valid > 0 ? p.n_valid : p.Cout;
            h.out_f32 = p.out_f32; h.out_f16 = p.out_f16; h.bias = p.bias; h.residual = p.residual; h.err_flag = p.err_flag;
            h.stats = p.stats; h.stats_blocks = p.Cout / 16;
            int dev = 0, num_sms = 148;
            cudaGetDevice(&dev);
            cudaDeviceGetAttribute(&num_sms, cudaDevAttrMultiProcessorCount, dev);
            const int bn = p.Cout == 16 ? 16 : ((p.Cout % 256 == 0 && p.block_n_hint != 128) ? 256 : 128);
            h.tiles_n = p.Cout / bn;
            CUtensorMap tmA, tmB;
            cuuint64_t gdim[5] = {(cuuint64_t)p.a_channels, (cuuint64_t)p.W, (cuuint64_t)p.H, 1, (cuuint64_t)p.B};
            cuuint64_t gstr[4] = {(cuuint64_t)p.lda * 2, (cuuint64_t)p.W * p.lda * 2, (cuuint64_t)p.H * p.W * p.lda * 2,
                                  (cuuint64_t)p.H * p.W * p.lda * 2};
            cuuint32_t box[5] = {kConvBlockK, kHaloW, kHaloH, 1, 1};
            cuuint32_t estr[5] = {1, 1, 1, 1, 1};
            if (enc(&tmA, CU_TENSOR_MAP_DATA_TYPE_FLOAT16, 5, const_cast<void*>(p.act), gdim, gstr, box, estr,
                    CU_TENSOR_MAP_INTERLEAVE_NONE, CU_TENSOR_MAP_SWIZZLE_128B, CU_TENSOR_MAP_L2_PROMOTION_L2_256B,
                    CU_TENSOR_MAP_FLOAT_OOB_FILL_NONE) != CUDA_SUCCESS)
                return -6;
            const cuuint64_t K = (cuuint64_t)9 * p.Cin;
            cuuint64_t wdim[2] = {K, (cuuint64_t)p.Cout};
            cuuint64_t wstr[1] = {K * 2};
            cuuint32_t wbox[2] = {kConvBlockK, (cuuint32_t)bn};
            cuuint32_t westr[2] = {1, 1};
            if (enc(&tmB, CU_TENSOR_MAP_DATA_TYPE_FLOAT16, 2, const_cast<void*>(p.wpacked), wdim, wstr, wbox, westr,
                    CU_TENSOR_MAP_INTERLEAVE_NONE, CU_TENSOR_MAP_SWIZZLE_128B, CU_TENSOR_MAP_L2_PROMOTION_L2_256B,
                    CU_TENSOR_MAP_FLOAT_OOB_FILL_NONE) != CUDA_SUCCESS)
                return -7;
            const int total = h.tiles_w * h.tiles_h * h.tiles_b * h.tiles_n;
            if (bn == 16) return launch_halo<16>(tmA, tmB, h, total, num_sms, stream);
            return bn == 256 ? launch_halo<256>(tmA, tmB, h, total, num_sms, stream)
                             : launch_halo<128>(tmA, tmB, h, total, num_sms, stream);
        }
    }

    ConvTcArgs a{};
    a.num_taps = p.num_taps;
    a.chunks_per_tap = p.Cin / kConvBlockK;
    int BW = p.W >= 128 ? 128 : p.W;
    int BH = 128 / BW;
    if (BH > p.H) BH = p.H;
    int BB = 128 / (BW * BH);
    a.bw_log2 = ilog2_exact(BW);
    a.bh_log2 = ilog2_exact(BH);
    a.tiles_w = (p.W + BW - 1) / BW;
    a.tiles_h = p.H / BH;
    a.tiles_b = (p.B + BB - 1) / BB;
    a.B = p.B; a.H = p.H; a.W = p.W;
    a.a_chan_off = p.a_chan_off;
    a.in_stride = p.in_stride == 2 ? 2 : 1;
    a.out_sb = p.out_sb; a.out_sh = p.out_sh; a.out_sw = p.out_sw;
    a.out_sc = p.out_sc > 0 ? p.out_sc : 1;
    a.n_valid = p.n_valid > 0 ? p.n_valid : p.Cout;
    a.out_f32 = p.out_f32; a.out_f16 = p.out_f16; a.bias = p.bias; a.residual = p.residual;
    a.err_flag = p.err_flag;
    a.dbg = p.dbg;
    a.stats = p.stats; a.stats_blocks = p.Cout / 16;
    for (int t = 0; t < p.num_taps; ++t) { a.dh[t] = p.dh[t]; a.dw[t] = p.dw[t]; a.ph[t] = p.ph[t]; }

    int dev = 0;
    cudaGetDevice(&dev);
    static int num_sms_cache[64] = {0};
    if (dev < 64 && num_sms_cache[dev] == 0)
        cudaDeviceGetAttribute(&num_sms_cache[dev], cudaDevAttrMultiProcessorCount, dev);
    const int num_sms = dev < 64 ? num_sms_cache[dev] : 148;
    const int tiles_m = a.tiles_w * a.tiles_h * a.tiles_b;
    int block_n = 0;
    const int cands[5] = {256, 128, 64, 32, 16};
    bool pair = false;
    if (p.cta_pair != 1 && p.block_n_hint >= 0) {
        const int pairs_m = (tiles_m + 1) / 2;
        int want = (p.block_n_hint == 128 || p.block_n_hint == 256) ? p.block_n_hint : (p.Cout % 256 == 0 ? 256 : 128);
        if (p.Cout % want == 0 && (p.cta_pair == 2 || (p.num_taps > 1 && pairs_m * (p.Cout / want) >= num_sms / 4))) {
            pair = true;
            block_n = want;
        }
    }
    const int hint = p.block_n_hint < 0 ? -p.block_n_hint : p.block_n_hint;
    if (!pair && hint > 0 && p.Cout % hint == 0) {
        for (int i = 0; i < 5; ++i)
            if (cands[i] == hint) block_n = cands[i];
    }
    if (block_n == 0) {
        for (int i = 0; i < 5; ++i) {
            if (p.Cout % cands[i] != 0) continue;
            block_n = cands[i];
            if (tiles_m * (p.Cout / cands[i]) >= num_sms || cands[i] <= 64) break;
        }
    }
    a.tiles_n = p.Cout / block_n;
    const int total_tiles = tiles_m * a.tiles_n;

    CUtensorMap tmA, tmA2, tmB;
    a.a_split = (p.act2 ? p.Cin1 : p.Cin) / kConvBlockK;
    a.a_chan_off2 = p.a_chan_off2;
    if (p.act2) {
        if (p.Cin1 <= 0 || p.Cin1 % kConvBlockK || p.Cin1 >= p.Cin || (p.lda2 % 8) || (reinterpret_cast<uintptr_t>(p.act2) & 15) ||
            a.in_stride != 1)
            return -8;
        cuuint64_t gdim[5] = {(cuuint64_t)p.lda2, (cuuint64_t)p.W, (cuuint64_t)p.H, (cuuint64_t)p.phases, (cuuint64_t)p.B};
        cuuint64_t gstr[4] = {(cuuint64_t)p.lda2 * 2, (cuuint64_t)p.W * p.lda2 * 2, (cuuint64_t)p.H * p.W * p.lda2 * 2,
                              (cuuint64_t)p.phases * p.H * p.W * p.lda2 * 2};
        cuuint32_t box[5] = {kConvBlockK, (cuuint32_t)BW, (cuuint32_t)BH, 1, (cuuint32_t)BB};
        cuuint32_t estr[5] = {1, 1, 1, 1, 1};
        if (enc(&tmA2, CU_TENSOR_MAP_DATA_TYPE_FLOAT16, 5, const_cast<void*>(p.act2), gdim, gstr, box, estr,
                CU_TENSOR_MAP_INTERLEAVE_NONE, CU_TENSOR_MAP_SWIZZLE_128B, CU_TENSOR_MAP_L2_PROMOTION_L2_256B,
                CU_TENSOR_MAP_FLOAT_OOB_FILL_NONE) != CUDA_SUCCESS)
            return -6;
    }
    {
        const cuuint64_t IS = a.in_stride;
        cuuint64_t gdim[5] = {(cuuint64_t)p.a_channels, (cuuint64_t)p.W * IS, (cuuint64_t)p.H * IS, (cuuint64_t)p.phases,
                              (cuuint64_t)p.B};
        cuuint64_t gstr[4] = {(cuuint64_t)p.lda * 2, (cuuint64_t)p.W * IS * p.lda * 2,
                              (cuuint64_t)p.H * IS * p.W * IS * p.lda * 2,
                              (cuuint64_t)p.phases * p.H * IS * p.W * IS * p.lda * 2};
        cuuint32_t box[5] = {kConvBlockK, (cuuint32_t)(BW * IS), (cuuint32_t)(BH * IS), 1, (cuuint32_t)BB};
        cuuint32_t estr[5] = {1, (cuuint32_t)IS, (cuuint32_t)IS, 1, 1};
        CUresult r = enc(&tmA, CU_TENSOR_MAP_DATA_TYPE_FLOAT16, 5, const_cast<void*>(p.act), gdim, gstr, box, estr,
                         CU_TENSOR_MAP_INTERLEAVE_NONE, CU_TENSOR_MAP_SWIZZLE_128B, CU_TENSOR_MAP_L2_PROMOTION_L2_256B,
                         CU_TENSOR_MAP_FLOAT_OOB_FILL_NONE);
        if (r != CUDA_SUCCESS) return -6;
        if (!p.act2) tmA2 = tmA;
    }
    {
        const cuuint64_t K = (cuuint64_t)p.num_taps * p.Cin;
        cuuint64_t gdim[2] = {K, (cuuint64_t)p.Cout};
        cuuint64_t gstr[1] = {K * 2};
        cuuint32_t box[2] = {kConvBlockK, (cuuint32_t)(pair ? block_n / 2 : block_n)};
        cuuint32_t estr[2] = {1, 1};
        CUresult r = enc(&tmB, CU_TENSOR_MAP_DATA_TYPE_FLOAT16, 2, const_cast<void*>(p.wpacked), gdim, gstr, box, estr,
                         CU_TENSOR_MAP_INTERLEAVE_NONE, CU_TENSOR_MAP_SWIZZLE_128B, CU_TENSOR_MAP_L2_PROMOTION_L2_256B,
                         CU_TENSOR_MAP_FLOAT_OOB_FILL_NONE);
        if (r != CUDA_SUCCESS) return -7;
    }

    if (pair) {
        const int total_pairs = ((tiles_m + 1) / 2) * a.tiles_n;
        const bool kc2 = p.kmerge != 1 && (a.chunks_per_tap % 2 == 0) && (a.a_split % 2 == 0);
        if (block_n == 256)
            return kc2 ? launch2<256, 2>(tmA, tmA2, tmB, a, total_pairs, num_sms, stream)
                       : launch2<256, 1>(tmA, tmA2, tmB, a, total_pairs, num_sms, stream);
// ... 14 lines not shown
```

### minimagen_b200/csrc/conv_tc.cuh

```cuda
#pragma once
#include <cuda_fp16.h>
#include <cuda_runtime.h>
#include <stdint.h>

namespace mi {

constexpr int kConvBlockM = 128;
constexpr int kConvBlockK = 64;
constexpr int kConvMaxTaps = 16;

struct ConvTcArgs {
    int num_taps, chunks_per_tap;
    int bw_log2, bh_log2;
    int tiles_w, tiles_h, tiles_b, tiles_n;
    int B, H, W;
    int a_chan_off;
    int in_stride;
    int a_split, a_chan_off2;
    int x_chunks, x_split;
    int x_chan_off, x_chan_off2;
    long long out_sb, out_sh, out_sw;
    long long out_sc;
    int n_valid;
    float* out_f32;
    __half* out_f16;
    const float* bias;
    const float* residual;
    int* err_flag;
    int dbg;
    double* stats;
    int stats_blocks;
    int8_t dh[kConvMaxTaps], dw[kConvMaxTaps], ph[kConvMaxTaps];
};

struct ConvTcProblem {
    const void* act;
    int B, H, W;
    int phases;
    int in_stride;
    int lda;
    int a_channels;
    int a_chan_off;
    int Cin;
    const void* act2;
    int lda2, a_chan_off2, Cin1;
    const void* wpacked;
    int Cout;
    const void* x_act; int x_lda, x_chan_off, Cx;
    const void* x_act2; int x_lda2, x_chan_off2, Cx1;
    int num_taps;
    int8_t dh[kConvMaxTaps], dw[kConvMaxTaps], ph[kConvMaxTaps];
    float* out_f32; __half* out_f16; const float* bias; const float* residual;
    long long out_sb, out_sh, out_sw;
    long long out_sc;
    int n_valid;
    int block_n_hint;
    int cta_pair;
    int halo;
    int kmerge;
    int dbg;
    double* stats;
    int* err_flag;
};

struct GnPrologueArgs {
    const float* src0;
    const float* src1;
    int C0, C1, groups;
    float scale1, eps;
    const double* stats0;
    const double* stats1;
    const float* gamma;
    const float* beta;
    const float* scale_shift;
    int ss_ld;
};

struct ConvGnProblem {
    const float* src0; int C0;
    const float* src1; int C1;
    float scale1;
    int B, H, W, groups;
    const double* stats0; const double* stats1;
    const float* gamma; const float* beta; const float* scale_shift; int ss_ld; float eps;
    const void* wpacked; int Cout;
    const float* bias; const float* residual;
    float* out_f32; __half* out_f16; double* out_stats;
    int* err_flag;
};

bool conv_gn_supported(int H, int W, int C0, int C1, int Cout, int groups);
int conv_gn_launch(const ConvGnProblem& p, cudaStream_t stream);
bool conv_gn_pair_supported(int H, int W, int C0, int C1, int Cout, int groups);
int conv_gn_pair_launch(const ConvGnProblem& p, cudaStream_t stream);

bool conv_tc_supported(int H, int W, int Cin, int Cout);
int conv_tc_launch(const ConvTcProblem& p, cudaStream_t stream);
const char* conv_tc_strerror(int code);

}
```

### minimagen_b200/csrc/launch.cuh

```cuda
#pragma once
#include <cuda_runtime.h>

namespace mi {

bool pdl_enabled();

__device__ __forceinline__ void pdl_wait() { asm volatile("griddepcontrol.wait;" ::: "memory"); }
__device__ __forceinline__ void pdl_trigger() {
#ifndef MI_PDL_NO_EARLY_TRIGGER
    asm volatile("griddepcontrol.launch_dependents;" ::: "memory");
#endif
}

template <typename... KArgs, typename... Args>
inline cudaError_t launch_k(void (*kernel)(KArgs...), dim3 grid, dim3 block, size_t smem, cudaStream_t stream,
                            Args&&... args) {
    cudaLaunchConfig_t cfg{};
    cfg.gridDim = grid;
    cfg.blockDim = block;
    cfg.dynamicSmemBytes = smem;
    cfg.stream = stream;
    cudaLaunchAttribute attr[1];
    attr[0].id = cudaLaunchAttributeProgrammaticStreamSerialization;
    attr[0].val.programmaticStreamSerializationAllowed = 1;
    cfg.attrs = attr;
    cfg.numAttrs = pdl_enabled() ? 1 : 0;
    return cudaLaunchKernelEx(&cfg, kernel, static_cast<KArgs>(args)...);
}

}
```

### minimagen_b200/csrc/ptx.cuh

```cuda
#pragma once
#include <cuda.h>
#include <cuda_fp16.h>
#include <stdint.h>

namespace mi {
namespace ptx {

__device__ __forceinline__ uint32_t smem_u32(const void* p) {
    return static_cast<uint32_t>(__cvta_generic_to_shared(p));
}

__device__ __forceinline__ void mbar_init(uint64_t* bar, uint32_t count) {
    asm volatile("mbarrier.init.shared::cta.b64 [%0], %1;" ::"r"(smem_u32(bar)), "r"(count));
}
__device__ __forceinline__ void fence_barrier_init() {
    asm volatile("fence.mbarrier_init.release.cluster;" ::: "memory");
}
__device__ __forceinline__ void fence_proxy_async_smem() {
    asm volatile("fence.proxy.async.shared::cta;" ::: "memory");
}
__device__ __forceinline__ void mbar_arrive(uint64_t* bar) {
    asm volatile("mbarrier.arrive.shared::cta.b64 _, [%0];" ::"r"(smem_u32(bar)) : "memory");
}
__device__ __forceinline__ void mbar_arrive_expect_tx(uint64_t* bar, uint32_t bytes) {
// ... 41 lines not shown
    asm volatile("ld.acquire.gpu.global.s32 %0, [%1];" : "=r"(v) : "l"(p) : "memory");
    return v;
}

__device__ __forceinline__ void prefetch_tensormap(const CUtensorMap* m) {
    asm volatile("prefetch.tensormap [%0];" ::"l"(reinterpret_cast<uint64_t>(m)) : "memory");
}
__device__ __forceinline__ void tma_load_2d(const CUtensorMap* m, uint64_t* bar, void* dst, int c0, int c1) {
    asm volatile(
        "cp.async.bulk.tensor.2d.shared::cluster.global.mbarrier::complete_tx::bytes [%0], [%1, {%3, %4}], [%2];"
        ::"r"(smem_u32(dst)), "l"(reinterpret_cast<uint64_t>(m)), "r"(smem_u32(bar)), "r"(c0), "r"(c1)
        : "memory");
}
__device__ __forceinline__ void tma_load_5d(const CUtensorMap* m, uint64_t* bar, void* dst, int c0, int c1, int c2,
                                            int c3, int c4) {
    asm volatile(
        "cp.async.bulk.tensor.5d.shared::cluster.global.mbarrier::complete_tx::bytes [%0], [%1, {%3, %4, %5, %6, "
        "%7}], [%2];"
        ::"r"(smem_u32(dst)), "l"(reinterpret_cast<uint64_t>(m)), "r"(smem_u32(bar)), "r"(c0), "r"(c1), "r"(c2),
        "r"(c3), "r"(c4)
        : "memory");
}

__device__ __forceinline__ void tmem_alloc(uint32_t* dst_smem, uint32_t ncols) {
    asm volatile("tcgen05.alloc.cta_group::1.sync.aligned.shared::cta.b32 [%0], %1;" ::"r"(smem_u32(dst_smem)),
                 "r"(ncols)
                 : "memory");
}
__device__ __forceinline__ void tmem_relinquish() {
    asm volatile("tcgen05.relinquish_alloc_permit.cta_group::1.sync.aligned;" ::: "memory");
}
__device__ __forceinline__ void tmem_dealloc(uint32_t taddr, uint32_t ncols) {
    asm volatile("tcgen05.dealloc.cta_group::1.sync.aligned.b32 %0, %1;" ::"r"(taddr), "r"(ncols) : "memory");
}
__device__ __forceinline__ void tc_fence_before() { asm volatile("tcgen05.fence::before_thread_sync;" ::: "memory"); }
__device__ __forceinline__ void tc_fence_after() { asm volatile("tcgen05.fence::after_thread_sync;" ::: "memory"); }

__device__ __forceinline__ void umma_f16(uint32_t tmem_d, uint64_t desc_a, uint64_t desc_b, uint32_t idesc,
                                         uint32_t accumulate) {
    asm volatile(
        "{\n\t"
        ".reg .pred p;\n\t"
        "setp.ne.b32 p, %4, 0;\n\t"
        "tcgen05.mma.cta_group::1.kind::f16 [%0], %1, %2, %3, p;\n\t"
        "}"
        ::"r"(tmem_d), "l"(desc_a), "l"(desc_b), "r"(idesc), "r"(accumulate)
        : "memory");
}
__device__ __forceinline__ void umma_f16_ts(uint32_t tmem_d, uint32_t tmem_a, uint64_t desc_b, uint32_t idesc,
                                            uint32_t accumulate) {
    asm volatile(
        "{\n\t"
        ".reg .pred p;\n\t"
        "setp.ne.b32 p, %4, 0;\n\t"
        "tcgen05.mma.cta_group::1.kind::f16 [%0], [%1], %2, %3, p;\n\t"
        "}"
        ::"r"(tmem_d), "r"(tmem_a), "l"(desc_b), "r"(idesc), "r"(accumulate)
        : "memory");
}
__device__ __forceinline__ void umma_commit(uint64_t* bar) {
    asm volatile("tcgen05.commit.cta_group::1.mbarrier::arrive::one.shared::cluster.b64 [%0];" ::"r"(smem_u32(bar))
                 : "memory");
}
__device__ __forceinline__ void tmem_ld_x16(uint32_t taddr, uint32_t (&v)[16]) {
    asm volatile(
        "tcgen05.ld.sync.aligned.32x32b.x16.b32 "
        "{%0, %1, %2, %3, %4, %5, %6, %7, %8, %9, %10, %11, %12, %13, %14, %15}, [%16];"
        : "=r"(v[0]), "=r"(v[1]), "=r"(v[2]), "=r"(v[3]), "=r"(v[4]), "=r"(v[5]), "=r"(v[6]), "=r"(v[7]),
          "=r"(v[8]), "=r"(v[9]), "=r"(v[10]), "=r"(v[11]), "=r"(v[12]), "=r"(v[13]), "=r"(v[14]), "=r"(v[15])
        : "r"(taddr)
        : "memory");
}
__device__ __forceinline__ void tmem_ld_wait() { asm volatile("tcgen05.wait::ld.sync.aligned;" ::: "memory"); }
__device__ __forceinline__ void tmem_st_x16(uint32_t taddr, const uint32_t (&v)[16]) {
    asm volatile(
        "tcgen05.st.sync.aligned.32x32b.x16.b32 [%0], {%1, %2, %3, %4, %5, %6, %7, %8, %9, %10, %11, %12, %13, %14, %15, %16};"
        ::"r"(taddr), "r"(v[0]), "r"(v[1]), "r"(v[2]), "r"(v[3]), "r"(v[4]), "r"(v[5]), "r"(v[6]), "r"(v[7]), "r"(v[8]),
          "r"(v[9]), "r"(v[10]), "r"(v[11]), "r"(v[12]), "r"(v[13]), "r"(v[14]), "r"(v[15])
        : "memory");
}
__device__ __forceinline__ void tmem_st_wait() { asm volatile("tcgen05.wait::st.sync.aligned;" ::: "memory"); }

__device__ __forceinline__ uint64_t make_kmajor_sw128_desc(uint32_t smem_addr) {
    uint64_t d = 0;
    d |= static_cast<uint64_t>((smem_addr >> 4) & 0x3FFF);
    d |= static_cast<uint64_t>(1024u >> 4) << 32;
    d |= static_cast<uint64_t>(1) << 46;
    d |= static_cast<uint64_t>(2) << 61;
    return d;
}
__host__ __device__ constexpr uint32_t make_idesc_f16(uint32_t M, uint32_t N, uint32_t ab_fmt = 0) {
    return (1u << 4) | (ab_fmt << 7) | (ab_fmt << 10) | ((N >> 3) << 17) | ((M >> 4) << 24);
}

}
}

namespace mi {
namespace ptx {

constexpr uint32_t kPeerBitMask = 0xFEFFFFFFu;

__device__ __forceinline__ uint32_t cluster_ctarank() {
    uint32_t r;
    asm volatile("mov.u32 %0, %%cluster_ctarank;" : "=r"(r));
    return r;
}
__device__ __forceinline__ void cluster_sync_all() {
    asm volatile("barrier.cluster.arrive.aligned;\n\tbarrier.cluster.wait.aligned;" ::: "memory");
}
__device__ __forceinline__ void mbar_arrive_cluster(uint64_t* bar, uint32_t cta) {
    asm volatile(
        "{\n\t"
        ".reg .b32 remAddr32;\n\t"
        "mapa.shared::cluster.u32 remAddr32, %0, %1;\n\t"
        "mbarrier.arrive.shared::cluster.b64 _, [remAddr32];\n\t"
        "}"
        ::"r"(smem_u32(bar)), "r"(cta)
        : "memory");
}
__device__ __forceinline__ void mbar_arrive_release_cluster(uint64_t* bar, uint32_t cta) {
    asm volatile(
        "{\n\t"
        ".reg .b32 remAddr32;\n\t"
        "mapa.shared::cluster.u32 remAddr32, %0, %1;\n\t"
        "mbarrier.arrive.release.cluster.shared::cluster.b64 _, [remAddr32];\n\t"
        "}"
        ::"r"(smem_u32(bar)), "r"(cta)
        : "memory");
}
__device__ __forceinline__ bool mbar_try_wait_acquire_cluster(uint64_t* bar, uint32_t parity) {
    uint32_t ok;
    asm volatile(
        "{\n\t"
        ".reg .pred p;\n\t"
        "mbarrier.try_wait.parity.acquire.cluster.shared::cta.b64 p, [%1], %2;\n\t"
        "selp.u32 %0, 1, 0, p;\n\t"
        "}"
        : "=r"(ok)
        : "r"(smem_u32(bar)), "r"(parity)
        : "memory");
    return ok != 0;
}
__device__ __forceinline__ void mbar_wait_acquire_cluster(uint64_t* bar, uint32_t parity, int* err, int code) {
    if (mbar_try_wait_acquire_cluster(bar, parity)) return;
    const long long t0 = clock64();
    while (!mbar_try_wait_acquire_cluster(bar, parity)) {
        if (clock64() - t0 > 4000000000LL) {
            if (err) { atomicExch(err, code); __threadfence_system(); }
            __trap();
        }
    }
}
__device__ __forceinline__ void tma_load_2d_2sm(const CUtensorMap* m, uint64_t* bar, void* dst, int c0, int c1) {
    asm volatile(
        "cp.async.bulk.tensor.2d.cta_group::2.shared::cluster.global.mbarrier::complete_tx::bytes [%0], [%1, {%3, %4}], "
        "[%2];"
        ::"r"(smem_u32(dst)), "l"(reinterpret_cast<uint64_t>(m)), "r"(smem_u32(bar) & kPeerBitMask), "r"(c0), "r"(c1)
        : "memory");
}
__device__ __forceinline__ void tma_load_5d_2sm(const CUtensorMap* m, uint64_t* bar, void* dst, int c0, int c1, int c2,
                                                int c3, int c4) {
    asm volatile(
        "cp.async.bulk.tensor.5d.cta_group::2.shared::cluster.global.mbarrier::complete_tx::bytes [%0], [%1, {%3, %4, "
        "%5, %6, %7}], [%2];"
        ::"r"(smem_u32(dst)), "l"(reinterpret_cast<uint64_t>(m)), "r"(smem_u32(bar) & kPeerBitMask), "r"(c0), "r"(c1),
        "r"(c2), "r"(c3), "r"(c4)
        : "memory");
}
__device__ __forceinline__ void tmem_alloc_2sm(uint32_t* dst_smem, uint32_t ncols) {
    asm volatile("tcgen05.alloc.cta_group::2.sync.aligned.shared::cta.b32 [%0], %1;" ::"r"(smem_u32(dst_smem)),
                 "r"(ncols)
                 : "memory");
}
__device__ __forceinline__ void tmem_relinquish_2sm() {
    asm volatile("tcgen05.relinquish_alloc_permit.cta_group::2.sync.aligned;" ::: "memory");
}
__device__ __forceinline__ void tmem_dealloc_2sm(uint32_t taddr, uint32_t ncols) {
    asm volatile("tcgen05.dealloc.cta_group::2.sync.aligned.b32 %0, %1;" ::"r"(taddr), "r"(ncols) : "memory");
}
__device__ __forceinline__ void umma_f16_2sm(uint32_t tmem_d, uint64_t desc_a, uint64_t desc_b, uint32_t idesc,
                                             uint32_t accumulate) {
    asm volatile(
        "{\n\t"
        ".reg .pred p;\n\t"
        "setp.ne.b32 p, %4, 0;\n\t"
        "tcgen05.mma.cta_group::2.kind::f16 [%0], %1, %2, %3, p;\n\t"
        "}"
        ::"r"(tmem_d), "l"(desc_a), "l"(desc_b), "r"(idesc), "r"(accumulate)
        : "memory");
}
__device__ __forceinline__ void umma_commit_2sm(uint64_t* bar, uint16_t cta_mask) {
    asm volatile(
        "tcgen05.commit.cta_group::2.mbarrier::arrive::one.shared::cluster.multicast::cluster.b64 [%0], %1;"
        ::"r"(smem_u32(bar)), "h"(cta_mask)
        : "memory");
}

}
}
```

### minimagen_b200/layers.py

```python
import math
import os

import torch
from torch import nn

from .helpers import default, exists
from .ops import get_ops

F16, F32, F64 = torch.float16, torch.float32, torch.float64


STATS_BLOCK = 16

GN_INPUT_F32 = True

FUSE_GN_CONV = {"0": False, "1": True, "pair": "pair", "all": "all"}.get(os.environ.get("MI_FUSE_GN_CONV", "0"), False)
FUSE_OVER_FOLD = os.environ.get("MI_FUSE_OVER_FOLD", "1") == "1"


def fuse_block_ok(c_out):
    if not FUSE_GN_CONV:
        return False
    if FUSE_GN_CONV == 'all':
        return True
    return c_out % 256 == 0 or (FUSE_GN_CONV is True and c_out == 128)


FOLD_RES_CONV = os.environ.get("MI_FOLD_RES_CONV", "1") == "1"

SUBPIXEL_UPSAMPLE = True

INPLACE_DOWNSAMPLE = True


class ZeroArena:

    def __init__(self, device, n_doubles):
        self.buf = torch.zeros((n_doubles,), dtype=F64, device=device)
        self.off = 0

    def take(self, shape):
        n = 1
        for d in shape:
            n *= d
        if self.off + n > self.buf.numel():
            return None
        out = self.buf[self.off:self.off + n].view(shape)
        self.off += (n + 1) // 2 * 2
        return out


_ARENA = None


def stats_zeros(shape, device):
    if _ARENA is not None and _ARENA.buf.device == device:
        t = _ARENA.take(shape)
        if t is not None:
            return t
    return torch.zeros(shape, dtype=F64, device=device)


class Act:
    __slots__ = ("f32", "f16", "stats")

    def __init__(self, f32=None, f16=None, stats=None):
        assert f32 is not None or f16 is not None
        self.f32, self.f16, self.stats = f32, f16, stats

    @property
    def any(self):
        return self.f32 if self.f32 is not None else self.f16

    @property
    def shape(self):
        sh = self.any.shape
        return (sh[0], sh[-3], sh[-2], sh[-1])

    @property
    def device(self):
        return self.any.device

    def need_f32(self):
        if self.f32 is None:
            B, H, W, C = self.shape
            self.f32 = torch.empty((B, H, W, C), dtype=F32, device=self.device)
            get_ops().cast_act(self.f16, C, None, 0, 1.0, B, H, W, 0, self.f32)
        return self.f32

    def need_f16(self):
        if self.f16 is None:
            B, H, W, C = self.shape
            self.f16 = torch.empty((B, 1, H, W, C), dtype=F16, device=self.device)
            get_ops().cast_act(self.f32, C, None, 0, 1.0, B, H, W, 0, self.f16)
        return self.f16

    def need_stats(self):
        if self.stats is None:
            B, H, W, C = self.shape
            self.stats = stats_zeros((B, C // STATS_BLOCK, 2), self.device)
            get_ops().gn_stats(self.any, C, None, 0, 1.0, B, H * W, C // STATS_BLOCK, self.stats)
        return self.stats


def as_act(x):
    return x if isinstance(x, (Act, Cat)) else Act(f32=x)


class Cat:

    def __init__(self, a, b, scale):
        a, b = as_act(a), as_act(b)
        assert a.shape[:3] == b.shape[:3]
        self.a, self.b, self.scale = a, b, float(scale)

    @property
    def shape(self):
        return (*self.a.shape[:3], self.a.shape[3] + self.b.shape[3])

    @property
    def device(self):
        return self.a.device


def _srcs(x, prefer_f16):
    parts = [x.a, x.b] if isinstance(x, Cat) else [x]
    use16 = prefer_f16 and all(p.f16 is not None for p in parts)
    if not use16 and not all(p.f32 is not None for p in parts):
        use16 = all(p.f16 is not None for p in parts)
        if not use16:
            for p in parts:
                p.need_f32()
    t = [(p.f16 if use16 else p.f32) for p in parts]
    if isinstance(x, Cat):
        return t[0], x.a.shape[3], t[1], x.b.shape[3], x.scale
    return t[0], x.shape[3], None, 0, 1.0


def _no_grad_check(*tensors):
    if torch.is_grad_enabled() and any(exists(t) and t.requires_grad for t in tensors):
        raise NotImplementedError(
            "minimagen_b200 implements the inference (sampling) hot path only; autograd through the sm_100a kernels "
            "(training, SURVEY.md 8f-2) is not built yet. Call under torch.no_grad().")


def to_nhwc(x):
    return x.permute(0, 2, 3, 1).contiguous()


def to_nchw(x):
    return x.permute(0, 3, 1, 2).contiguous()


class _PackCache:

    def __init__(self):
        self._key = None
        self._val = None

    def get(self, param, scale=1.0):
        key = (param.data_ptr(), param._version, str(param.device), float(scale))
        if key != self._key:
            self._val = get_ops().pack_conv_weight(param, scale)
            self._key = key
        return self._val


def _linear_rows(x_f32, x_f16, M, K, weight, pack, Nout, bias=None, residual=None, want_f16=False, scale=1.0):
    ops = get_ops()
    dev = (x_f32 if x_f32 is not None else x_f16).device
    out = torch.empty((M, Nout), dtype=F16 if want_f16 else F32, device=dev)
    if x_f16 is not None:
        ops.conv_igemm(x_f16, 1, 1, M, K, 0, K, pack.get(weight, scale), Nout, 1, 1, 0, bias, residual,
                       None if want_f16 else out, out if want_f16 else None, (0, 0, Nout))
    else:
        w2 = weight.detach().reshape(Nout, K)
        ops.linear_f32(x_f32, M, K, w2, bias, Nout, 0, 0, residual, None if want_f16 else out,
                       out if want_f16 else None, scale)
    return out


def _tc_linear_ok(M, K, Nout):
    return get_ops().igemm_supported(1, M, K, Nout) and M >= 128


class Identity(nn.Module):

    def __init__(self, *args, **kwargs):
        super().__init__()

    def forward(self, x, *args, **kwargs):
        return x

    def run(self, x, *args, **kwargs):
        return x


class LayerNorm(nn.Module):

    def __init__(self, dim):
        super().__init__()
        self.gamma = nn.Parameter(torch.ones(dim))
        self.register_buffer('beta', torch.zeros(dim))

    def run_rows(self, rows_f32, R, C, residual=None, out_dtype=F32, pre_gelu=False, both=False):
        o32 = torch.empty((R, C), dtype=F32, device=rows_f32.device) if (both or out_dtype == F32) else None
        o16 = torch.empty((R, C), dtype=F16, device=rows_f32.device) if (both or out_dtype == F16) else None
        get_ops().ln_rows(rows_f32, R, C, self.gamma, self.beta, 1e-5, pre_gelu, residual, o32, o16)
        return (o32, o16) if both else (o32 if out_dtype == F32 else o16)

    def forward(self, x):
        _no_grad_check(x, self.gamma)
        C = x.shape[-1]
        return self.run_rows(x.reshape(-1, C).contiguous(), x.numel() // C, C).reshape(x.shape)


class ChanLayerNorm(nn.Module):

    def __init__(self, dim, eps=1e-5):
        super().__init__()
        self.eps = eps
        self.g = nn.Parameter(torch.ones(1, dim, 1, 1))

    def run_rows(self, rows_f32, R, C, out_dtype=F32, pre_gelu=False):
        out = torch.empty((R, C), dtype=out_dtype, device=rows_f32.device)
        get_ops().ln_rows(rows_f32, R, C, self.g.detach().reshape(C), None, self.eps, pre_gelu, None,
                          out if out_dtype == F32 else None, out if out_dtype == F16 else None)
        return out

    def forward(self, x):
        _no_grad_check(x, self.g)
        B, C, H, W = x.shape
        return to_nchw(self.run_rows(to_nhwc(x).reshape(-1, C), B * H * W, C).reshape(B, H, W, C))


class SinusoidalPosEmb(nn.Module):

    def __init__(self, dim):
        super().__init__()
        self.dim = dim

    def forward(self, x):
        B = x.shape[0]
        out = torch.empty((B, self.dim), dtype=F32, device=x.device)
        get_ops().posemb(x.to(torch.int64).contiguous(), B, self.dim, out)
        return out


class Residual(nn.Module):

    def __init__(self, fn):
        super().__init__()
        self.fn = fn

    def forward(self, x, **kwargs):
        return self.fn(x, **kwargs) + x


class Parallel(nn.Module):

    def __init__(self, *fns):
        super().__init__()
        self.fns = nn.ModuleList(fns)

    def run(self, x):
        x = as_act(x)
        out = None
        for i, fn in enumerate(self.fns):
            last = i == len(self.fns) - 1
            out = fn.run(x, residual=out.f32 if exists(out) else None, f32=True, f16=last, stats=last)
        return out

    def forward(self, x):
        _no_grad_check(x)
        return to_nchw(self.run(to_nhwc(x)).need_f32())


class TokenView(nn.Module):

    def __init__(self, fn):
        super().__init__()
        self.fn = fn

    def run(self, x, **kwargs):
        return self.fn.run(x, **kwargs)

    def forward(self, x, **kwargs):
        _no_grad_check(x)
        if "context" in kwargs and not isinstance(kwargs["context"], Context):
            kwargs["context"] = Context(kwargs["context"])
        return to_nchw(self.run(as_act(to_nhwc(x)), **kwargs).need_f32())


class Conv2d(nn.Conv2d):

    def __init__(self, *args, **kwargs):
        super().__init__(*args, **kwargs)
        self._pack = _PackCache()

    @property
    def _geom(self):
        kh, kw = self.kernel_size
        s, p = self.stride[0], self.padding[0]
        if s == 1 and kh == kw and kh % 2 == 1 and p == kh // 2:
            return 'same'
        if s == 2 and kh == 4 and kw == 4 and p == 1:
            return 'down'
        raise NotImplementedError(f"conv geometry k={self.kernel_size} s={self.stride} p={self.padding}")

    def tc_ok(self, H, W):
        kh, kw = self.kernel_size
        return kh * kw <= 16 and get_ops().igemm_supported(H, W, self.in_channels, self.out_channels)

    def _pack_fold(self, rc, c0, scale):
        key = (self.weight.data_ptr(), self.weight._version, rc.weight.data_ptr(), rc.weight._version, c0, float(scale),
               self.bias._version if exists(self.bias) else -1, rc.bias._version if exists(rc.bias) else -1)
        if getattr(self, "_fold_key", None) != key:
            ops = get_ops()
            w1 = rc.weight.detach().clone()
            if c0 is not None:
                w1[:, c0:] *= scale
            self._fold_w = torch.cat((ops.pack_conv_weight(self.weight), ops.pack_conv_weight(w1)), dim=1).contiguous()
            b = torch.zeros((self.out_channels,), dtype=F32, device=self.weight.device)
            if exists(self.bias):
                b = b + self.bias.detach()
            if exists(rc.bias):
                b = b + rc.bias.detach()
            self._fold_b = b.contiguous()
            self._fold_key = key
        return self._fold_w, self._fold_b

    def run_folded(self, a, B, H, W, xsrc, rc, residual=None, f32=True, f16=False, stats=False):
        ops = get_ops()
        Cin, Cout = self.in_channels, self.out_channels
        dev = a.device
        cat = isinstance(xsrc, Cat)
        parts = [xsrc.a, xsrc.b] if cat else [xsrc]
        x0 = parts[0].need_f16()
        x1 = parts[1].need_f16() if cat else None
        c0 = parts[0].shape[3] if cat else None
        wp, bias = self._pack_fold(rc, c0, xsrc.scale if cat else 1.0)
        st = stats_zeros((B, Cout // STATS_BLOCK, 2), dev) if (stats and Cout % 32 == 0 and (H * W) % 32 == 0) else None
        if not f32 and not f16:
            f32 = True
        o32 = torch.empty((B, H, W, Cout), dtype=F32, device=dev) if f32 else None
        o16 = torch.empty((B, 1, H, W, Cout), dtype=F16, device=dev) if f16 else None
        ops.conv_res1x1(a, B, H, W, a.shape[-1], Cin, None, 0, 0, x0, x0.shape[-1], rc.in_channels, x1,
                        x1.shape[-1] if cat else 0, c0 if cat else 0, wp, Cout, bias, residual, o32, o16, st)
        return Act(o32, o16, st)

    def run_prepared(self, a, B, H, W, residual=None, f32=True, f16=False, stats=False, a2=None, c_in1=0, wp=None,
                     in_place_s2=False):
        ops = get_ops()
        Cin, Cout = self.in_channels, self.out_channels
        kh, kw = self.kernel_size
        strides = (H * W * Cout, W * Cout, Cout)
        dev = a.device
        if a.dtype == F16:
            mode = (6 if in_place_s2 else 1) if self._geom == 'down' else 0
            st = stats_zeros((B, Cout // STATS_BLOCK, 2), dev) if (stats and Cout % 32 == 0 and (H * W) % 32 == 0) else None
            if not f32 and not f16:
                f32 = True
            o32 = torch.empty((B, H, W, Cout), dtype=F32, device=dev) if f32 else None
            o16 = torch.empty((B, 1, H, W, Cout), dtype=F16, device=dev) if f16 else None
            lda = a.shape[-1]
            ops.conv_igemm(a, B, H, W, lda, 0, Cin, wp if exists(wp) else self._pack.get(self.weight), Cout, kh, kw, mode,
                           self.bias, residual, o32, o16, strides, act2=a2, lda2=a2.shape[-1] if exists(a2) else 0,
                           c_in1=c_in1, out_stats=st)
            return Act(o32, o16, st)
        out = torch.empty((B, H, W, Cout), dtype=F32, device=dev)
        Hin, Win = a.shape[1], a.shape[2]
        ops.conv_direct(a, B, Hin, Win, Cin, a.shape[3], self.weight.detach(), Cout, kh, kw, self.stride[0],
                        self.padding[0], self.bias, residual, out, H, W, (*strides, 1))
        return Act(f32=out)

    def _run_subpixel(self, x, B, H, W, f32, f16, stats):
        ops = get_ops()
        Cin, Cout = self.in_channels, self.out_channels
        key = (self.weight.data_ptr(), self.weight._version)
        if getattr(self, "_sub_key", None) != key:
            w = self.weight.detach().to(F32)
            rows = ((slice(0, 1), slice(1, 3)), (slice(0, 2), slice(2, 3)))
            self._sub_w = []
            for a in range(2):
                for b in range(2):
                    k = torch.stack([torch.stack([w[:, :, rows[a][r], rows[b][s]].sum(dim=(2, 3)) for s in range(2)], dim=-1)
                                     for r in range(2)], dim=-2)
                    self._sub_w.append(ops.pack_conv_weight(k))
            self._sub_key = key
        dev = x.device
        Ho, Wo = 2 * H, 2 * W
        if not f32 and not f16:
            f32 = True
        st = stats_zeros((B, Cout // STATS_BLOCK, 2), dev) if (stats and Cout % 32 == 0 and (H * W) % 32 == 0) else None
        o32 = torch.empty((B, Ho, Wo, Cout), dtype=F32, device=dev) if f32 else None
        o16 = torch.empty((B, 1, Ho, Wo, Cout), dtype=F16, device=dev) if f16 else None
        a16 = x.need_f16()
        strides = (Ho * Wo * Cout, 2 * Wo * Cout, 2 * Cout)
        for p in range(4):
            off = ((p >> 1) * Wo + (p & 1)) * Cout
            ops.conv_igemm(a16, B, H, W, a16.shape[-1], 0, Cin, self._sub_w[p], Cout, 2, 2, 2 + p, self.bias, None,
                           o32.reshape(-1)[off:] if f32 else None, o16.reshape(-1)[off:] if f16 else None, strides,
                           out_stats=st)
        return Act(o32, o16, st)

    def _pack_cat(self, c0, scale):
        key = (self.weight.data_ptr(), self.weight._version, c0, float(scale))
        if getattr(self, "_cat_key", None) != key:
            w = self.weight.detach().clone()
            w[:, c0:] *= scale
            self._cat_w = get_ops().pack_conv_weight(w)
            self._cat_key = key
        return self._cat_w

    def run_prepared_nchw(self, a, B, H, W, out=None):
        ops = get_ops()
        Cin, Cout = self.in_channels, self.out_channels
        kh, kw = self.kernel_size
        if out is None:
            out = torch.empty((B, Cout, H, W), dtype=F32, device=a.device)
        if a.dtype == F16:
            Np = (Cout + 15) // 16 * 16
            key = (self.weight.data_ptr(), self.weight._version, self.bias._version if exists(self.bias) else -1)
            if getattr(self, "_nchw_key", None) != key:
                wp = torch.zeros((Np, kh * kw * Cin), dtype=F16, device=a.device)
                wp[:Cout] = ops.pack_conv_weight(self.weight)
                bp = torch.zeros((Np,), dtype=F32, device=a.device)
                if exists(self.bias):
                    bp[:Cout] = self.bias.detach()
                self._nchw_w, self._nchw_b, self._nchw_key = wp, bp, key
            ops.conv_igemm(a, B, H, W, Cin, 0, Cin, self._nchw_w, Np, kh, kw, 0, self._nchw_b, None, out, None,
                           (Cout * H * W, W, 1), out_sc=H * W, n_valid=Cout)
        else:
            ops.conv_direct(a, B, H, W, Cin, a.shape[3], self.weight.detach(), Cout, kh, kw, 1, self.padding[0],
                            self.bias, None, out, H, W, (Cout * H * W, W, 1, H * W))
        return out

    def run(self, x, residual=None, upsample=False, f32=True, f16=False, stats=False):
        ops = get_ops()
        x = as_act(x)
        B, H, W, C = x.shape
        assert C == self.in_channels, (C, self.in_channels)
        geom = self._geom
        if upsample:
            assert geom == 'same'
            Ho, Wo = 2 * H, 2 * W
        elif geom == 'down':
            Ho, Wo = H // 2, W // 2
        else:
            Ho, Wo = H, W
        kw = dict(residual=residual, f32=f32, f16=f16, stats=stats)
        if upsample and SUBPIXEL_UPSAMPLE and not isinstance(x, Cat) and residual is None and self.kernel_size == (3, 3) \
                and get_ops().igemm_supported(H, W, C, self.out_channels):
            return self._run_subpixel(x, B, H, W, f32=f32, f16=f16, stats=stats)
        if self.tc_ok(Ho, Wo):
            if not upsample and geom == 'same':
                if isinstance(x, Cat):
                    c0 = x.a.shape[3]
                    if c0 % 64 == 0:
                        return self.run_prepared(x.a.need_f16(), B, H, W, a2=x.b.need_f16(), c_in1=c0,
                                                 wp=self._pack_cat(c0, x.scale), **kw)
                else:
                    return self.run_prepared(x.need_f16(), B, H, W, **kw)
            if geom == 'down' and INPLACE_DOWNSAMPLE and not isinstance(x, Cat) and x.f16 is not None:
                return self.run_prepared(x.f16, B, Ho, Wo, in_place_s2=True, **kw)
            s0, C0, s1, C1, sc = _srcs(x, True)
            mode = 1 if upsample else (2 if geom == 'down' else 0)
            a = torch.empty((B, 4 if mode == 2 else 1, Ho, Wo, C), dtype=F16, device=x.device)
            ops.cast_act(s0, C0, s1, C1, sc, B, H, W, mode, a)
            return self.run_prepared(a, B, Ho, Wo, **kw)
        if upsample or isinstance(x, Cat):
            s0, C0, s1, C1, sc = _srcs(x, False)
            a = torch.empty((B, Ho if upsample else H, Wo if upsample else W, C), dtype=F32, device=x.device)
            ops.cast_act(s0, C0, s1, C1, sc, B, H, W, 1 if upsample else 0, a)
        else:
            a = x.need_f32()
        return self.run_prepared(a, B, Ho, Wo, **kw)

    def forward(self, x):
        _no_grad_check(x, self.weight)
        return to_nchw(self.run(to_nhwc(x)).need_f32())


def Downsample(dim, dim_out=None):
    return Conv2d(dim, default(dim_out, dim), kernel_size=4, stride=2, padding=1)


class _UpsampleSeq(nn.Sequential):

    def run(self, x):
        return self[1].run(x, upsample=True, f32=GN_INPUT_F32, f16=True, stats=True)

    def forward(self, x):
        _no_grad_check(x)
        return to_nchw(self.run(to_nhwc(x)).need_f32())


def Upsample(dim, dim_out=None):
    return _UpsampleSeq(nn.Upsample(scale_factor=2, mode='nearest'), Conv2d(dim, default(dim_out, dim), 3, padding=1))


class CrossEmbedLayer(nn.Module):

    def __init__(self, dim_in, kernel_sizes, dim_out=None, stride=2):
        super().__init__()
        assert all((k % 2) == (stride % 2) for k in kernel_sizes)
        dim_out = default(dim_out, dim_in)
        kernel_sizes = sorted(kernel_sizes)
        num_scales = len(kernel_sizes)
        dim_scales = [int(dim_out / (2 ** i)) for i in range(1, num_scales)]
        dim_scales = [*dim_scales, dim_out - sum(dim_scales)]
        self.dim_in, self.dim_out, self.stride = dim_in, dim_out, stride
        self.convs = nn.ModuleList([
            Conv2d(dim_in, ds, k, stride=stride, padding=(k - stride) // 2) for k, ds in zip(kernel_sizes, dim_scales)])

    def stem_tc_ok(self, H, W):
        ks = [c.kernel_size[0] for c in self.convs]
        return (self.stride == 1 and self.dim_in <= 8 and max(ks) <= 15 and all(k % 2 == 1 for k in ks)
                and get_ops().igemm_supported(H, W, 128, self.dim_out))

    def _stem_weights(self):
        key = tuple((c.weight.data_ptr(), c.weight._version, c.bias._version) for c in self.convs)
        if getattr(self, "_stem_key", None) != key:
            dev = self.convs[0].weight.device
            wm = torch.zeros((self.dim_out, 15, 16, 8), dtype=F32, device=dev)
            off = 0
            for conv in self.convs:
                k, n = conv.kernel_size[0], conv.out_channels
                lo = 7 - k // 2
                wm[off:off + n, lo:lo + k, lo:lo + k, :self.dim_in] = conv.weight.detach().permute(0, 2, 3, 1)
                off += n
            self._stem_w = wm.reshape(self.dim_out, 15 * 128).to(F16).contiguous()
            self._stem_b = torch.cat([c.bias.detach() for c in self.convs]).contiguous()
            self._stem_key = key
        return self._stem_w, self._stem_b

    def run_stem(self, x, lowres=None):
        ops = get_ops()
        B, Cx, H, W = x.shape
        Cl = lowres.shape[1] if exists(lowres) else 0
        assert Cx + Cl == self.dim_in
        x = x.to(F32).contiguous()
        lowres = lowres.to(F32).contiguous() if exists(lowres) else None
        if self.stem_tc_ok(H, W):
            a = torch.empty((B, 1, H, W, 128), dtype=F16, device=x.device)
            ops.stem_unroll(x, Cx, lowres, Cl, B, H, W, a)
            wp, bias = self._stem_weights()
            C = self.dim_out
            out = torch.empty((B, H, W, C), dtype=F32, device=x.device)
            out16 = torch.empty((B, 1, H, W, C), dtype=F16, device=x.device)
            st = stats_zeros((B, C // STATS_BLOCK, 2), x.device) if (C % 32 == 0 and (H * W) % 32 == 0) else None
            ops.conv_igemm(a, B, H, W, 128, 0, 128, wp, C, 15, 1, 0, bias, None, out, out16, (H * W * C, W * C, C),
                           out_stats=st)
            return Act(out, out16, st)
        cp = (self.dim_in + 3) // 4 * 4
        x_pad = torch.empty((B, H, W, cp), dtype=F32, device=x.device)
        ops.nchw_to_nhwc(x, Cx, lowres, Cl, B, H * W, cp, x_pad)
        return Act(f32=self.run_padded(x_pad, B, H, W))

    def run_padded(self, x_pad, B, H, W):
        assert self.stride == 1
        ops = get_ops()
        out = torch.empty((B, H, W, self.dim_out), dtype=F32, device=x_pad.device)
        C = self.dim_out
        off = 0
        for conv in self.convs:
            k = conv.kernel_size[0]
            ops.conv_direct(x_pad, B, H, W, self.dim_in, x_pad.shape[3], conv.weight.detach(), conv.out_channels, k, k,
                            1, conv.padding[0], conv.bias, None, out[..., off:], H, W, (H * W * C, W * C, C, 1))
            off += conv.out_channels
        return out

    def forward(self, x):
        _no_grad_check(x)
        return to_nchw(self.run_stem(x).need_f32())


class Block(nn.Module):

    def __init__(self, dim, dim_out, groups=8, norm=True):
        super().__init__()
        self.groupnorm = nn.GroupNorm(groups, dim) if norm else Identity()
        self.activation = nn.SiLU()
        self.project = Conv2d(dim, dim_out, 3, padding=1)

    def run(self, x, scale_shift=None, residual=None, f32=True, f16=False, stats=False, fold=None):
        ops = get_ops()
        x = as_act(x)
        B, H, W, C = x.shape
        gn = self.groupnorm
        assert isinstance(gn, nn.GroupNorm), "Block(norm=False) is never instantiated by the U-Net"
        G = gn.num_groups
        Cg = C // G
        tc = self.project.tc_ok(H, W)
        parts = [x.a, x.b] if isinstance(x, Cat) else [x]
        block_mode = tc and Cg % STATS_BLOCK == 0 and all(p.shape[3] % STATS_BLOCK == 0 for p in parts)
        if (fold is None and block_mode and fuse_block_ok(self.project.out_channels)
                and all(p.f32 is not None for p in parts)
                and ops.conv_gn_supported(H, W, parts[0].shape[3], parts[1].shape[3] if len(parts) > 1 else 0,
                                          self.project.out_channels, G)):
            conv = self.project
            Cout = conv.out_channels
            dev = x.device
            if not f32 and not f16:
                f32 = True
            o32 = torch.empty((B, H, W, Cout), dtype=F32, device=dev) if f32 else None
            o16 = torch.empty((B, 1, H, W, Cout), dtype=F16, device=dev) if f16 else None
            st = stats_zeros((B, Cout // STATS_BLOCK, 2), dev) if stats else None
            p1 = parts[1] if len(parts) > 1 else None
            ops.conv_gn(parts[0].f32, parts[0].shape[3], p1.f32 if p1 else None, p1.shape[3] if p1 else 0,
                        x.scale if p1 else 1.0, B, H, W, G, parts[0].need_stats(), p1.need_stats() if p1 else None,
                        gn.weight, gn.bias, scale_shift, scale_shift.stride(0) if exists(scale_shift) else 0, gn.eps,
                        conv._pack.get(conv.weight), Cout, conv.bias, residual, o32, o16, st)
            return Act(o32, o16, st)
        s0, C0, s1, C1, sc = _srcs(x, tc and not GN_INPUT_F32)
        if block_mode:
            st0, sb0 = parts[0].need_stats(), STATS_BLOCK
            st1, sb1 = (parts[1].need_stats(), STATS_BLOCK) if len(parts) > 1 else (None, 0)
        else:
            st0 = stats_zeros((B, G, 2), x.device)
            ops.gn_stats(s0, C0, s1, C1, sc, B, H * W, G, st0)
            sb0, st1, sb1 = 0, None, 0
        a = torch.empty((B, 1, H, W, C) if tc else (B, H, W, C), dtype=F16 if tc else F32, device=x.device)
        ss_ld = scale_shift.stride(0) if exists(scale_shift) else 0
        ops.gn_apply_silu(s0, C0, s1, C1, sc, B, H * W, G, st0, sb0, st1, sb1, gn.weight, gn.bias, scale_shift, ss_ld,
                          gn.eps, a)
        if fold is not None:
            return self.project.run_folded(a, B, H, W, fold[0], fold[1], residual, f32=f32, f16=f16, stats=stats)
        return self.project.run_prepared(a, B, H, W, residual, f32=f32, f16=f16, stats=stats)

    def forward(self, x, scale_shift=None):
        _no_grad_check(x)
        ss = None
        if exists(scale_shift):
            scale, shift = scale_shift
            ss = torch.cat((scale.reshape(x.shape[0], -1), shift.reshape(x.shape[0], -1)), dim=1).contiguous()
        return to_nchw(self.run(to_nhwc(x), ss).need_f32())


class ResnetBlock(nn.Module):

    def __init__(self, dim, dim_out, *, cond_dim=None, time_cond_dim=None, groups=8):
        super().__init__()
        self.time_mlp = None
        if exists(time_cond_dim):
            self.time_mlp = nn.Sequential(nn.SiLU(), nn.Linear(time_cond_dim, dim_out * 2))
        self.cross_attn = None
        if exists(cond_dim):
            self.cross_attn = TokenView(CrossAttention(dim=dim_out, context_dim=cond_dim))
        self.block1 = Block(dim, dim_out, groups=groups)
        self.block2 = Block(dim_out, dim_out, groups=groups)
        self.res_conv = Conv2d(dim, dim_out, 1) if dim != dim_out else Identity()

    def run(self, x, time_emb=None, cond=None, scale_shift=None, out_f32=True):
        ops = get_ops()
        B = x.shape[0]
        if not exists(scale_shift) and exists(self.time_mlp) and exists(time_emb):
            lin = self.time_mlp[1]
            scale_shift = torch.empty((B, lin.out_features), dtype=F32, device=time_emb.device)
            ops.linear_f32(time_emb, B, lin.in_features, lin.weight, lin.bias, lin.out_features, 1, 0, None,
                           scale_shift, None)
        x = as_act(x)
        tc = self.block1.project.tc_ok(x.shape[1], x.shape[2]) and self.block2.project.tc_ok(x.shape[1], x.shape[2])
        attn = exists(self.cross_attn)
        keep32 = attn or not tc or GN_INPUT_F32
        h = self.block1.run(x, f32=keep32, f16=not keep32, stats=tc and not attn)
        if attn:
            assert exists(cond)
            h = self.cross_attn.run(h, context=cond)
        if isinstance(self.res_conv, Identity):
            assert not isinstance(x, Cat)
            res = x.need_f32()
        else:
            _, H, W, _ = x.shape
            c2 = self.block2.project
            xparts = [x.a, x.b] if isinstance(x, Cat) else [x]
            fused_gn = FUSE_OVER_FOLD and fuse_block_ok(c2.out_channels) and ops.conv_gn_supported(
                H, W, c2.in_channels, 0, c2.out_channels, self.block2.groupnorm.num_groups)
            if (FOLD_RES_CONV and tc and not fused_gn and self.res_conv.kernel_size == (1, 1)
                    and all(p.shape[3] % 64 == 0 for p in xparts)
                    and ops.conv_res1x1_supported(H, W, c2.in_channels, c2.out_channels, self.res_conv.in_channels)):
                return self.block2.run(h, scale_shift, residual=None, f32=out_f32 or not tc, f16=tc, stats=tc,
                                       fold=(x, self.res_conv))
            res = self.res_conv.run(x, f32=True).f32
        return self.block2.run(h, scale_shift, residual=res, f32=out_f32 or not tc, f16=tc, stats=tc)

    def forward(self, x, time_emb=None, cond=None):
        _no_grad_check(x)
        ctx = Context(cond) if exists(cond) else None
        return to_nchw(self.run(to_nhwc(x), time_emb, ctx).need_f32())


class Context:

    def __init__(self, c_f32):
        self.f32 = c_f32.contiguous()
        self._f16 = None

    @property
    def f16(self):
        if self._f16 is None:
            B, m, D = self.f32.shape
            self._f16 = torch.empty((B * m, D), dtype=F16, device=self.f32.device)
            get_ops().cast_act(self.f32, D, None, 0, 1.0, 1, 1, B * m, 0, self._f16)
        return self._f16


class CrossAttention(nn.Module):

    def __init__(self, dim, *, context_dim=None, dim_head=64, heads=8, norm_context=False):
        super().__init__()
        assert dim_head == 64, "the fused attention kernel is specialised for dim_head = 64 (the reference's constant)"
        self.scale = dim_head ** -0.5
        self.heads = heads
        inner_dim = dim_head * heads
        context_dim = default(context_dim, dim)
        self.norm = LayerNorm(dim)
        self.norm_context = LayerNorm(context_dim) if norm_context else Identity()
        self.null_kv = nn.Parameter(torch.randn(2, dim_head))
        self.to_q = nn.Linear(dim, inner_dim, bias=False)
        self.to_kv = nn.Linear(context_dim, inner_dim * 2, bias=False)
        self.to_out = nn.Sequential(nn.Linear(inner_dim, dim, bias=False), LayerNorm(dim))
        self._pq, self._pkv, self._po = _PackCache(), _PackCache(), _PackCache()

    def run(self, x, context, mask=None, residual=True):
        ops = get_ops()
        x = as_act(x)
        B, H, W, C = x.shape
        n = H * W
        m, D = context.f32.shape[1], context.f32.shape[2]
        inner = self.heads * 64
        rows = x.need_f32().reshape(B * n, C)
        assert isinstance(self.norm_context, Identity)
        tc_q = _tc_linear_ok(B * n, C, inner)
        xn = self.norm.run_rows(rows, B * n, C, out_dtype=F16 if tc_q else F32)
        q = _linear_rows(None if tc_q else xn, xn if tc_q else None, B * n, C, self.to_q.weight, self._pq, inner,
                         want_f16=True, scale=self.scale)
        tc_kv = _tc_linear_ok(B * m, D, 2 * inner)
        kv = _linear_rows(None if tc_kv else context.f32.reshape(B * m, D), context.f16 if tc_kv else None, B * m, D,
                          self.to_kv.weight, self._pkv, 2 * inner, want_f16=True)
        o = torch.empty((B * n, inner), dtype=F16, device=x.device)
        ops.attention(q, n * inner, inner, kv, kv[:, inner:], m * 2 * inner, 2 * inner, 64, self.null_kv, mask, B,
                      self.heads, n, m, o, n * inner, inner)
        tc_o = _tc_linear_ok(B * n, inner, C)
        if tc_o:
            y = _linear_rows(None, o, B * n, inner, self.to_out[0].weight, self._po, C)
        else:
            y = _linear_rows(o.float(), None, B * n, inner, self.to_out[0].weight, self._po, C)
        o32, o16 = self.to_out[1].run_rows(y, B * n, C, residual=rows if residual else None, both=True)
        return Act(o32.reshape(B, H, W, C), o16.reshape(B, 1, H, W, C))

    def forward(self, x, context, mask=None):
        _no_grad_check(x, context)
        B, n, C = x.shape
        xx = x.contiguous().reshape(B, 1, n, C)
        mk = mask.to(torch.uint8).contiguous() if exists(mask) else None
        return self.run(xx, Context(context), mk, residual=False).f32.reshape(B, n, C)


class Attention(nn.Module):

    def __init__(self, dim, *, dim_head=64, heads=8, context_dim=None):
        super().__init__()
        assert dim_head == 64, "the fused attention kernel is specialised for dim_head = 64 (Unet.py:86 ATTN_DIM_HEAD)"
        assert not exists(context_dim), "Attention(context_dim=...) is never instantiated by the U-Net"
        self.scale = dim_head ** -0.5
        self.heads = heads
        inner_dim = dim_head * heads
        self.norm = LayerNorm(dim)
        self.null_kv = nn.Parameter(torch.randn(2, dim_head))
        self.to_q = nn.Linear(dim, inner_dim, bias=False)
        self.to_kv = nn.Linear(dim, dim_head * 2, bias=False)
        self.to_context = None
        self.to_out = nn.Sequential(nn.Linear(inner_dim, dim, bias=False), LayerNorm(dim))
        self._pq, self._pkv, self._po = _PackCache(), _PackCache(), _PackCache()

    def run(self, x, context=None, mask=None, residual=True):
        assert context is None
        ops = get_ops()
        x = as_act(x)
        B, H, W, C = x.shape
        n = H * W
        inner = self.heads * 64
        rows = x.need_f32().reshape(B * n, C)
        tc = _tc_linear_ok(B * n, C, inner) and _tc_linear_ok(B * n, C, 128)
        xn = self.norm.run_rows(rows, B * n, C, out_dtype=F16 if tc else F32)
        q = _linear_rows(None if tc else xn, xn if tc else None, B * n, C, self.to_q.weight, self._pq, inner,
                         want_f16=True, scale=self.scale)
        kv = _linear_rows(None if tc else xn, xn if tc else None, B * n, C, self.to_kv.weight, self._pkv, 128,
                          want_f16=True)
        o = torch.empty((B * n, inner), dtype=F16, device=x.device)
        ops.attention(q, n * inner, inner, kv, kv[:, 64:], n * 128, 128, 0, self.null_kv, mask, B, self.heads, n, n, o,
                      n * inner, inner)
        if _tc_linear_ok(B * n, inner, C):
            y = _linear_rows(None, o, B * n, inner, self.to_out[0].weight, self._po, C)
        else:
            y = _linear_rows(o.float(), None, B * n, inner, self.to_out[0].weight, self._po, C)
        o32, o16 = self.to_out[1].run_rows(y, B * n, C, residual=rows if residual else None, both=True)
        return Act(o32.reshape(B, H, W, C), o16.reshape(B, 1, H, W, C))

    def forward(self, x, context=None, mask=None, attn_bias=None):
        _no_grad_check(x)
        assert context is None and attn_bias is None
        B, n, C = x.shape
        mk = mask.to(torch.uint8).contiguous() if exists(mask) else None
        return self.run(x.contiguous().reshape(B, 1, n, C), mask=mk, residual=False).f32.reshape(B, n, C)


class _ResidualAttention(Residual):

    def run(self, x):
        return self.fn.run(x, residual=True)


def ChanFeedForward(dim, mult=2):
    hidden_dim = int(dim * mult)
    return nn.Sequential(
        ChanLayerNorm(dim),
        Conv2d(dim, hidden_dim, 1, bias=False),
        nn.GELU(),
        ChanLayerNorm(hidden_dim),
        Conv2d(hidden_dim, dim, 1, bias=False))


class TransformerBlock(nn.Module):

    def __init__(self, dim, *, heads=8, dim_head=32, ff_mult=2, context_dim=None):
        super().__init__()
        self.attn = TokenView(Attention(dim=dim, heads=heads, dim_head=dim_head, context_dim=context_dim))
        self.ff = ChanFeedForward(dim=dim, mult=ff_mult)

    def run(self, x, context=None):
        x = as_act(x)
        B, H, W, C = x.shape
        R = B * H * W
        x = self.attn.run(x, residual=True)
        ln1, conv1, _, ln2, conv2 = self.ff
        hid = conv1.out_channels
# ... 15 lines not shown
```

### minimagen_b200/ops.py

```python
import torch

from . import _native as N

F16, F32, F64, I64, U8 = torch.float16, torch.float32, torch.float64, torch.int64, torch.uint8


def _chk(t, dtype, name):
    if t is None:
        return
    if t.dtype != dtype:
        raise TypeError(f"{name}: expected {dtype}, got {t.dtype}")
    if not t.is_contiguous():
        raise ValueError(f"{name}: tensor must be contiguous")


def _chk_out(t, dtype, name):
    if t is not None and t.dtype != dtype:
        raise TypeError(f"{name}: expected {dtype}, got {t.dtype}")


class NativeOps:
    name = "native-sm100a"
    attention_tc = True

    def set_launch_mode(self, pdl):
        N.load().mi_set_launch_mode(int(bool(pdl)))

    def igemm_supported(self, H, W, c_in, c_out):
        return bool(N.load().mi_conv2d_igemm_supported(int(H), int(W), int(c_in), int(c_out)))

    def pack_conv_weight(self, w, scale=1.0):
        if w.dim() == 2:
            w = w[:, :, None, None]
        w = w.detach().to(F32).contiguous()
        O, I, KH, KW = w.shape
        out = torch.empty((O, KH * KW * I), dtype=F16, device=w.device)
        N.call("mi_pack_conv_weight_f16", N.ptr(w), O, I, KH, KW, float(scale), N.ptr(out), N.stream())
        return out

    def pack_conv_weight_dgrad(self, w):
        if w.dim() == 2:
            w = w[:, :, None, None]
        w = w.detach().to(F32).contiguous()
        O, I, KH, KW = w.shape
        out = torch.empty((I, KH * KW * O), dtype=F16, device=w.device)
        N.call("mi_pack_conv_weight_dgrad_f16", N.ptr(w), O, I, KH, KW, N.ptr(out), N.stream())
        return out

    def conv_igemm(self, act, B, H, W, lda, c_off, c_in, wp, c_out, kh, kw, mode, bias, residual, out_f32, out_f16,
                   out_strides, block_n=0, out_sc=1, n_valid=0, act2=None, lda2=0, c_off2=0, c_in1=0, out_stats=None):
        _chk(act, F16, "act"); _chk(act2, F16, "act2"); _chk(wp, F16, "wp"); _chk(bias, F32, "bias")
        _chk_out(residual, F32, "residual"); _chk_out(out_f32, F32, "out_f32"); _chk_out(out_f16, F16, "out_f16")
        _chk(out_stats, F64, "out_stats")
        sb, sh, sw = out_strides
        N.call("mi_conv2d_igemm_f16", N.ptr(act), B, H, W, lda, c_off, c_in, N.ptr(act2), lda2, c_off2, c_in1,
               N.ptr(wp), c_out, kh, kw, mode, N.ptr(bias), N.ptr(residual), N.ptr(out_f32), N.ptr(out_f16),
               N.ptr(out_stats), sb, sh, sw, out_sc, n_valid, block_n, None, None, 0, N.stream())

    def conv_res1x1_supported(self, H, W, c_in, c_out, x_cin):
        return bool(N.load().mi_conv3x3_res1x1_supported(int(H), int(W), int(c_in), int(c_out), int(x_cin)))

    def conv_res1x1(self, act, B, H, W, lda, c_in, act2, lda2, c_in1, x, ldx, x_cin, x2, ldx2, x_cin1, wp, c_out, bias,
                    residual, out_f32, out_f16, out_stats):
        for nm, t in (("act", act), ("act2", act2), ("x", x), ("x2", x2), ("wp", wp)):
            _chk(t, F16, nm)
        _chk(bias, F32, "bias"); _chk(residual, F32, "residual"); _chk(out_f32, F32, "out_f32"); _chk(out_f16, F16, "out_f16")
        _chk(out_stats, F64, "out_stats")
        N.call("mi_conv3x3_res1x1_f16", N.ptr(act), B, H, W, lda, c_in, N.ptr(act2), lda2, c_in1, N.ptr(x), ldx, x_cin,
               N.ptr(x2), ldx2, x_cin1, N.ptr(wp), c_out, N.ptr(bias), N.ptr(residual), N.ptr(out_f32), N.ptr(out_f16),
               N.ptr(out_stats), None, N.stream())

    def conv_gn_supported(self, H, W, c0, c1, c_out, groups):
        return bool(N.load().mi_conv3x3_gn_supported(int(H), int(W), int(c0), int(c1), int(c_out), int(groups)))

    def conv_gn(self, src0, c0, src1, c1, scale1, B, H, W, groups, stats0, stats1, gamma, beta, scale_shift, ss_ld, eps,
                wp, c_out, bias, residual, out_f32, out_f16, out_stats):
        _chk(src0, F32, "src0"); _chk(src1, F32, "src1"); _chk(stats0, F64, "stats0"); _chk(stats1, F64, "stats1")
        _chk(gamma, F32, "gamma"); _chk(beta, F32, "beta"); _chk_out(scale_shift, F32, "scale_shift"); _chk(wp, F16, "wp")
        _chk(bias, F32, "bias"); _chk(residual, F32, "residual"); _chk(out_f32, F32, "out_f32")
        _chk(out_f16, F16, "out_f16"); _chk(out_stats, F64, "out_stats")
        N.call("mi_conv3x3_gn_silu_f16", N.ptr(src0), c0, N.ptr(src1), c1, float(scale1), B, H, W, groups,
               N.ptr(stats0), N.ptr(stats1), N.ptr(gamma), N.ptr(beta), N.ptr(scale_shift), int(ss_ld), float(eps),
               N.ptr(wp), c_out, N.ptr(bias), N.ptr(residual), N.ptr(out_f32), N.ptr(out_f16), N.ptr(out_stats), None,
               N.stream())

    def conv_direct(self, inp, B, Hin, Win, c_in, ldi, w, c_out, kh, kw, stride, pad, bias, residual, out, Hout, Wout,
                    out_strides):
        _chk(inp, F32, "inp"); _chk(w, F32, "w"); _chk(bias, F32, "bias"); _chk_out(residual, F32, "residual")
        if out.dtype != F32:
            raise TypeError("out must be fp32")
        sb, sh, sw, sc = out_strides
        N.call("mi_conv2d_direct_f32", N.ptr(inp), B, Hin, Win, c_in, ldi, N.ptr(w), c_out, kh, kw, stride, pad,
               N.ptr(bias), N.ptr(residual), N.ptr(out), Hout, Wout, sb, sh, sw, sc, N.stream())

    def gn_stats(self, src0, c0, src1, c1, scale1, B, hw, groups, sums):
        _chk(src0, src0.dtype, "src0"); _chk(src1, src0.dtype, "src1"); _chk(sums, F64, "sums")
        N.call("mi_gn_stats", N.ptr(src0), c0, N.ptr(src1), c1, float(scale1), int(src0.dtype == F16), B, hw, groups,
               N.ptr(sums), N.stream())

    def gn_apply_silu(self, src0, c0, src1, c1, scale1, B, hw, groups, stats0, sb0, stats1, sb1, gamma, beta,
                      scale_shift, ss_ld, eps, out):
        in16 = src0.dtype == F16
        _chk(src0, src0.dtype, "src0"); _chk(src1, src0.dtype, "src1"); _chk(stats0, F64, "stats0")
        _chk(stats1, F64, "stats1"); _chk(gamma, F32, "gamma"); _chk(beta, F32, "beta")
        _chk_out(scale_shift, F32, "scale_shift")
        N.call("mi_gn_apply_silu", N.ptr(src0), c0, N.ptr(src1), c1, float(scale1), int(in16), B, hw, groups,
               N.ptr(stats0), int(sb0), N.ptr(stats1), int(sb1), N.ptr(gamma), N.ptr(beta), N.ptr(scale_shift),
               int(ss_ld), float(eps), N.ptr(out), int(out.dtype == F16), N.stream())

    def cast_act(self, src0, c0, src1, c1, scale1, B, H, W, mode, out):
        _chk(src0, src0.dtype, "src0"); _chk(src1, src0.dtype, "src1")
        N.call("mi_cast_act", N.ptr(src0), c0, N.ptr(src1), c1, float(scale1), int(src0.dtype == F16), B, H, W, mode,
               N.ptr(out), int(out.dtype == F16), N.stream())

    def ln_rows(self, inp, rows, C, gamma, beta, eps, pre_gelu, residual, out_f32, out_f16):
        _chk(inp, F32, "inp"); _chk(gamma, F32, "gamma"); _chk(beta, F32, "beta"); _chk(residual, F32, "residual")
        _chk(out_f32, F32, "out_f32"); _chk(out_f16, F16, "out_f16")
        N.call("mi_ln_rows", N.ptr(inp), rows, C, N.ptr(gamma), N.ptr(beta), float(eps), int(pre_gelu), N.ptr(residual),
               N.ptr(out_f32), N.ptr(out_f16), N.stream())

    def linear_f32(self, inp, M, K, W, bias, Nout, in_act, out_act, addend, out_f32, out_f16, out_scale=1.0):
        _chk(inp, F32, "inp"); _chk(W, F32, "W"); _chk(bias, F32, "bias"); _chk(addend, F32, "addend")
        _chk(out_f32, F32, "out_f32"); _chk(out_f16, F16, "out_f16")
        N.call("mi_linear_f32", N.ptr(inp), M, K, N.ptr(W), N.ptr(bias), Nout, in_act, out_act, N.ptr(addend),
               N.ptr(out_f32), N.ptr(out_f16), float(out_scale), N.stream())

    def posemb(self, t, B, dim, out):
        _chk(t, I64, "t"); _chk(out, F32, "out")
        N.call("mi_sinusoidal_posemb", N.ptr(t), B, dim, N.ptr(out), N.stream())

    def text_tokens(self, proj, B, L, D, mask, keep, null_embed, max_len, c_out, m, row_off, pooled):
        _chk(proj, F32, "proj"); _chk(mask, U8, "mask"); _chk(keep, U8, "keep"); _chk(null_embed, F32, "null_embed")
        _chk(c_out, F32, "c_out"); _chk(pooled, F32, "pooled")
        N.call("mi_text_tokens", N.ptr(proj), B, L, D, N.ptr(mask), N.ptr(keep), N.ptr(null_embed), max_len,
               N.ptr(c_out), m, row_off, N.ptr(pooled), N.stream())

    def place_rows(self, src, B, r, D, dst, m, row_off):
        _chk(src, F32, "src"); _chk(dst, F32, "dst")
        N.call("mi_place_rows", N.ptr(src), B, r, D, N.ptr(dst), m, row_off, N.stream())

    def select_rows(self, a, null_row, keep, addend, B, Nn, out):
        _chk(a, F32, "a"); _chk(null_row, F32, "null_row"); _chk(keep, U8, "keep"); _chk(addend, F32, "addend")
        N.call("mi_select_rows", N.ptr(a), N.ptr(null_row), N.ptr(keep), N.ptr(addend), B, Nn, N.ptr(out), N.stream())

    def nchw_to_nhwc(self, a, ca, b, cb, B, hw, c_pad, out):
        _chk(a, F32, "a"); _chk(b, F32, "b"); _chk(out, F32, "out")
        N.call("mi_nchw_to_nhwc", N.ptr(a), ca, N.ptr(b), cb, B, hw, c_pad, N.ptr(out), N.stream())

    def stem_unroll(self, a, ca, b, cb, B, H, W, out):
        _chk(a, F32, "a"); _chk(b, F32, "b"); _chk(out, F16, "out")
        N.call("mi_stem_unroll_f16", N.ptr(a), ca, N.ptr(b), cb, B, H, W, N.ptr(out), N.stream())

    def resize_separable(self, inp, planes, hin, win, out, hout, wout, iy, wy, ix, wx, clamp=None):
        _chk(inp, F32, "inp"); _chk(out, F32, "out"); _chk(wy, F32, "wy"); _chk(wx, F32, "wx")
        _chk(iy, torch.int32, "iy"); _chk(ix, torch.int32, "ix")
        N.call("mi_resize_separable", N.ptr(inp), planes, hin, win, N.ptr(out), hout, wout, N.ptr(iy), N.ptr(wy),
               iy.shape[1], N.ptr(ix), N.ptr(wx), ix.shape[1], int(clamp is not None),
               float(clamp[0]) if clamp is not None else 0.0, float(clamp[1]) if clamp is not None else 0.0, N.stream())

    def silu(self, inp, out):
        _chk(inp, F32, "inp"); _chk(out, F32, "out")
        N.call("mi_silu_f32", N.ptr(inp), inp.numel(), N.ptr(out), N.stream())

    def attention(self, q, q_bs, ldq, k, v, kv_bs, ldkv, kv_hs, null_kv, mask, B, heads, n, m, out, o_bs, ldo):
        if q.dtype != F16 or k.dtype != F16 or v.dtype != F16 or out.dtype != F16:
            raise TypeError("attention operands must be fp16")
        _chk(null_kv, F32, "null_kv"); _chk(mask, U8, "mask")
        ws = None
        if self.attention_tc and n % 128 == 0 and m >= 128:
            nbytes = int(N.load().mi_attention_workspace_bytes(B, heads, kv_hs, m))
            ws = torch.empty(nbytes, dtype=torch.uint8, device=q.device)
        N.call("mi_attention_fwd", N.ptr(q), q_bs, ldq, N.ptr(k), N.ptr(v), kv_bs, ldkv, kv_hs, N.ptr(null_kv),
               N.ptr(mask), B, heads, n, m, N.ptr(out), o_bs, ldo, N.ptr(ws), ws.numel() if ws is not None else 0,
               N.stream())

    def step_x0(self, x_t, eps_cond, eps_null, cond_scale, t, tab_a, tab_b, B, n, x0):
        for nm, tt in (("x_t", x_t), ("eps_cond", eps_cond), ("eps_null", eps_null), ("tab_a", tab_a),
                       ("tab_b", tab_b), ("x0", x0)):
            _chk(tt, F32, nm)
        _chk(t, I64, "t")
        N.call("mi_step_x0", N.ptr(x_t), N.ptr(eps_cond), N.ptr(eps_null), float(cond_scale), N.ptr(t), N.ptr(tab_a),
               N.ptr(tab_b), B, n, N.ptr(x0), N.stream())

    def step_quantile(self, x0, B, n, rank_lo, rank_hi, weight, min_s, s):
        _chk(x0, F32, "x0"); _chk(s, F32, "s")
        N.call("mi_step_quantile", N.ptr(x0), B, n, int(rank_lo), int(rank_hi), float(weight), float(min_s), N.ptr(s),
               N.stream())

    def step_posterior(self, x0, x_t, noise, s, t, c1, c2, sigma, B, n, out):
        for nm, tt in (("x0", x0), ("x_t", x_t), ("noise", noise), ("s", s), ("c1", c1), ("c2", c2), ("sigma", sigma),
                       ("out", out)):
            _chk(tt, F32, nm)
        _chk(t, I64, "t")
        N.call("mi_step_posterior", N.ptr(x0), N.ptr(x_t), N.ptr(noise), N.ptr(s), N.ptr(t), N.ptr(c1), N.ptr(c2),
               N.ptr(sigma), B, n, N.ptr(out), N.stream())

    def step_epilogue(self, x_t, eps_cond, eps_null, cond_scale, t, tab_a, tab_b, c1, c2, sigma, noise, B, n, rank_lo,
                      rank_hi, weight, min_s, out, s_out=None):
        for nm, tt in (("x_t", x_t), ("eps_cond", eps_cond), ("eps_null", eps_null), ("tab_a", tab_a), ("tab_b", tab_b),
                       ("c1", c1), ("c2", c2), ("sigma", sigma), ("noise", noise), ("out", out), ("s_out", s_out)):
            _chk(tt, F32, nm)
        _chk(t, I64, "t")
        ws = None
        nws = int(N.load().mi_step_epilogue_workspace_floats(B, n))
        if nws:
            ws = torch.empty(nws, dtype=F32, device=x_t.device)
            if s_out is None:
                s_out = torch.empty(B, dtype=F32, device=x_t.device)
        N.call("mi_step_epilogue", N.ptr(x_t), N.ptr(eps_cond), N.ptr(eps_null), float(cond_scale), N.ptr(t), N.ptr(tab_a),
               N.ptr(tab_b), N.ptr(c1), N.ptr(c2), N.ptr(sigma), N.ptr(noise), B, n, int(rank_lo), int(rank_hi),
# ... 92 lines not shown
```

Before: 35.89.

## Fuse next GroupNorm+SiLU into 3x3 conv epilogue using cluster-wide statistics

Adds a GroupNorm+SiLU epilogue to the tcgen05 halo conv kernel. The accumulator is stashed back to TMEM, group mean and M2 are reduced across warps and across a CTA cluster through DSMEM and mbarriers, and the normalized f16 operand for the next block is written directly. ResnetBlocks pass the following GroupNorm (block2's, or the next block's block1) so the separate stats and apply passes, plus the intermediate f32/f16 writes, can be skipped. The cost is extra TMEM round trips, cluster synchronization that constrains tile scheduling, and more shared memory and epilogue latency.

```diff
diff --git a/include/minimagen_b200.h b/include/minimagen_b200.h
--- a/include/minimagen_b200.h
+++ b/include/minimagen_b200.h
@@ -25,6 +25,14 @@
                         const float* bias, const float* residual, float* out_f32, void* out_f16, double* out_stats,
                         long long out_sb, long long out_sh, long long out_sw, long long out_sc, int n_valid,
                         int block_n, int* err_flag, void* workspace, long long workspace_bytes, void* stream);
+int mi_conv_gn_epilogue_supported(int H, int W, int c_out, int groups);
+int mi_conv2d_igemm_gn_f16(const void* act_f16, int B, int H, int W, int lda, int c_off, int c_in, const void* act2_f16,
+                           int lda2, int c_off2, int c_in1, const void* w_f16, int c_out, int kh, int kw, int mode,
+                           const float* bias, const float* residual, float* out_f32, void* out_f16, double* out_stats,
+                           long long out_sb, long long out_sh, long long out_sw, long long out_sc, int n_valid,
+                           int block_n, int* err_flag, void* workspace, long long workspace_bytes, int groups,
+                           const float* gamma, const float* beta, const float* scale_shift, int scale_shift_ld, float eps,
+                           void* gn_out_f16, void* stream);
 int mi_conv3x3_res1x1_supported(int H, int W, int c_in, int c_out, int x_cin);
 int mi_conv3x3_res1x1_f16(const void* act_f16, int B, int H, int W, int lda, int c_in, const void* act2_f16, int lda2,
                           int c_in1, const void* x_f16, int ldx, int x_cin, const void* x2_f16, int ldx2, int x_cin1,
diff --git a/minimagen_b200/Unet.py b/minimagen_b200/Unet.py
--- a/minimagen_b200/Unet.py
+++ b/minimagen_b200/Unet.py
@@ -233,10 +233,12 @@
         for pre_downsample, init_block, resnet_blocks, attn_block, post_downsample in self.downs:
             if exists(pre_downsample):
                 h = pre_downsample.run(h)
-            h = init_block.run(h, t, ctx, ss[init_block])
-            for resnet_block in resnet_blocks:
-                h = resnet_block.run(h, t, None, ss[resnet_block])
-                hiddens.append(h)
+            chain = [init_block, *resnet_blocks]
+            for i, blk in enumerate(chain):
+                gn_next = chain[i + 1].block1.groupnorm if i + 1 < len(chain) else None
+                h = blk.run(h, t, ctx if i == 0 else None, ss[blk], gn_next=gn_next)
+                if i > 0:
+                    hiddens.append(h)
             h = attn_block.run(h)
             hiddens.append(h)
             if exists(post_downsample):
diff --git a/minimagen_b200/_native.py b/minimagen_b200/_native.py
--- a/minimagen_b200/_native.py
+++ b/minimagen_b200/_native.py
@@ -19,6 +19,9 @@
     "mi_conv2d_igemm_supported": [_I, _I, _I, _I],
     "mi_conv2d_igemm_f16": [_P, _I, _I, _I, _I, _I, _I, _P, _I, _I, _I, _P, _I, _I, _I, _I, _P, _P, _P, _P, _P, _L, _L, _L, _L,
                             _I, _I, _P, _P, _L, _P],
+    "mi_conv_gn_epilogue_supported": [_I, _I, _I, _I],
+    "mi_conv2d_igemm_gn_f16": [_P, _I, _I, _I, _I, _I, _I, _P, _I, _I, _I, _P, _I, _I, _I, _I, _P, _P, _P, _P, _P, _L, _L, _L,
+                               _L, _I, _I, _P, _P, _L, _I, _P, _P, _P, _I, _F, _P, _P],
     "mi_conv3x3_res1x1_supported": [_I, _I, _I, _I, _I],
     "mi_conv3x3_res1x1_f16": [_P, _I, _I, _I, _I, _I, _P, _I, _I, _P, _I, _I, _P, _I, _I, _P, _I, _P, _P, _P, _P, _P, _P, _P],
     "mi_conv2d_igemm_workspace_bytes": [],
diff --git a/minimagen_b200/csrc/capi.cu b/minimagen_b200/csrc/capi.cu
--- a/minimagen_b200/csrc/capi.cu
+++ b/minimagen_b200/csrc/capi.cu
@@ -65,8 +65,12 @@
                         const float* residual, float* out_f32, void* out_f16, double* out_stats, long long out_sb,
                         long long out_sh, long long out_sw, long long out_sc, int n_valid, int block_n, int* err_flag,
                         void* workspace, long long workspace_bytes, const void* x_act, int ldx, int x_off, int x_cin,
-                        const void* x_act2, int ldx2, int x_off2, int x_cin1, void* stream) {
+                        const void* x_act2, int ldx2, int x_off2, int x_cin1, void* stream, int gn_groups = 0,
+                        const float* gn_gamma = nullptr, const float* gn_beta = nullptr,
+                        const float* gn_ss = nullptr, int gn_ss_ld = 0, float gn_eps = 0.f, void* gn_out = nullptr) {
     mi::ConvTcProblem p{};
+    p.gn_groups = gn_groups; p.gn_gamma = gn_gamma; p.gn_beta = gn_beta; p.gn_ss = gn_ss; p.gn_ss_ld = gn_ss_ld;
+    p.gn_eps = gn_eps; p.gn_out = (__half*)gn_out;
     p.x_act = x_act; p.x_lda = ldx; p.x_chan_off = x_off; p.Cx = x_cin;
     p.x_act2 = x_act2; p.x_lda2 = ldx2; p.x_chan_off2 = x_off2; p.Cx1 = x_cin1;
     if (x_act && !(mode == 0 && kh == 3 && kw == 3)) return fail(-9, "mi_conv3x3_res1x1_f16: the folded 1x1 operand needs a 3x3 stride-1 conv");
@@ -138,6 +142,26 @@
                         workspace_bytes, nullptr, 0, 0, 0, nullptr, 0, 0, 0, stream);
 }
 
+int mi_conv_gn_epilogue_supported(int H, int W, int c_out, int groups) {
+    return mi::conv_gn_epilogue_supported(H, W, c_out, groups) ? 1 : 0;
+}
+
+int mi_conv2d_igemm_gn_f16(const void* act, int B, int H, int W, int lda, int c_off, int c_in, const void* act2, int lda2,
+                           int c_off2, int c_in1, const void* w, int c_out, int kh, int kw, int mode, const float* bias,
+                           const float* residual, float* out_f32, void* out_f16, double* out_stats, long long out_sb,
+                           long long out_sh, long long out_sw, long long out_sc, int n_valid, int block_n, int* err_flag,
+                           void* workspace, long long workspace_bytes, int groups, const float* gamma, const float* beta,
+                           const float* scale_shift, int scale_shift_ld, float eps, void* gn_out_f16, void* stream) {
+    if (!gn_out_f16 || !gamma || !beta) return fail(-12, "mi_conv2d_igemm_gn_f16: gn_out_f16, gamma and beta are required");
+    if (mode != 0 || kh != 3 || kw != 3 || !mi::conv_gn_epilogue_supported(H, W, c_out, groups))
+        return fail(-12, "mi_conv2d_igemm_gn_f16: unsupported geometry (see mi_conv_gn_epilogue_supported)");
+    if (scale_shift && scale_shift_ld < 2 * c_out) return fail(-8, "mi_conv2d_igemm_gn_f16: scale_shift_ld < 2*c_out");
+    return igemm_common(act, B, H, W, lda, c_off, c_in, act2, lda2, c_off2, c_in1, w, c_out, kh, kw, mode, bias, residual,
+                        out_f32, out_f16, out_stats, out_sb, out_sh, out_sw, out_sc, n_valid, block_n, err_flag, workspace,
+                        workspace_bytes, nullptr, 0, 0, 0, nullptr, 0, 0, 0, stream, groups, gamma, beta, scale_shift,
+                        scale_shift_ld, eps, gn_out_f16);
+}
+
 int mi_conv3x3_res1x1_supported(int H, int W, int c_in, int c_out, int x_cin) {
     const bool t16 = W == 16 && H % 16 == 0, t32 = !t16 && H % 32 == 0 && W % 8 == 0;
     return (t16 || t32) && c_in > 0 && c_in % 64 == 0 && x_cin > 0 && x_cin % 64 == 0 && c_out % 128 == 0;
diff --git a/minimagen_b200/csrc/conv_tc.cu b/minimagen_b200/csrc/conv_tc.cu
--- a/minimagen_b200/csrc/conv_tc.cu
+++ b/minimagen_b200/csrc/conv_tc.cu
@@ -569,7 +569,8 @@
     static constexpr int kHStages = kW16 ? 3 : 2;
     static constexpr int kWStages = (kRingBudget - kHStages * kHaloStride) / kWBytes;
     static constexpr uint32_t kTmemCols = 2 * kHtPix;
-    static constexpr uint32_t kSmemBytes = kHStages * kHaloStride + kWStages * kWBytes + 1024 + 256;
+    static constexpr uint32_t kGnBytes = 512;
+    static constexpr uint32_t kSmemBytes = kHStages * kHaloStride + kWStages * kWBytes + 1024 + 256 + kGnBytes;
 };
 
 __device__ __forceinline__ uint64_t make_halo_t_desc(uint32_t smem_addr, uint32_t sbo_bytes) {
@@ -601,12 +602,15 @@
     uint64_t* emptyW = bars + 2 * NH + NW;
     uint64_t* tfull_bar = bars + 2 * NH + 2 * NW;
     uint64_t* tempty_bar = tfull_bar + 2;
-    uint32_t* tmem_ptr_smem = reinterpret_cast<uint32_t*>(tempty_bar + 2);
-    static_assert((2 * NH + 2 * NW + 4) * 8 + 8 <= 256, "barrier block too large");
+    uint64_t* gnx_bar = tempty_bar + 2;
+    uint32_t* tmem_ptr_smem = reinterpret_cast<uint32_t*>(gnx_bar + 2);
+    static_assert((2 * NH + 2 * NW + 6) * 8 + 8 <= 256, "barrier block too large");
 
     const int warp = threadIdx.x >> 5;
     const int lane = threadIdx.x & 31;
     int* err = args.err_flag;
+    const int cs = args.gn_cluster > 1 ? args.gn_cluster : 1;
+    const int crank = cs > 1 ? (int)ptx::cluster_ctarank() : 0;
 
     if (warp == 0 && lane == 0) {
         ptx::prefetch_tensormap(&tmA);
@@ -616,6 +620,7 @@
         for (int i = 0; i < NH; ++i) { ptx::mbar_init(&fullH[i], 1); ptx::mbar_init(&emptyH[i], 1); }
         for (int i = 0; i < NW; ++i) { ptx::mbar_init(&fullW[i], 1); ptx::mbar_init(&emptyW[i], 1); }
         for (int i = 0; i < 2; ++i) { ptx::mbar_init(&tfull_bar[i], 1); ptx::mbar_init(&tempty_bar[i], 32 * kEpiWarps); }
+        for (int i = 0; i < 2; ++i) ptx::mbar_init(&gnx_bar[i], cs);
         ptx::fence_barrier_init();
     }
     if (warp == 2) {
@@ -623,7 +628,8 @@
         ptx::tmem_relinquish();
     }
     ptx::tc_fence_before();
-    __syncthreads();
+    if (cs > 1) ptx::cluster_sync_all();
+    else __syncthreads();
     ptx::tc_fence_after();
     const uint32_t tmem_base = *tmem_ptr_smem;
     pdl_wait();
@@ -632,13 +638,14 @@
     const int tiles_m = args.tiles_w * args.tiles_h * args.tiles_b;
     const int total_tiles = tiles_m * args.tiles_n;
     const int Cin = chunks * kConvBlockK;
+    const int v_first = blockIdx.x / cs, v_step = gridDim.x / cs, v_end = total_tiles / cs;
 
     if (warp == 0) {
         int sh = 0, sw = 0;
         uint32_t ph = 0, pw = 0;
-        for (int tile = blockIdx.x; tile < total_tiles; tile += gridDim.x) {
-            const int nt = tile % args.tiles_n;
-            const int mt = tile / args.tiles_n;
+        for (int v = v_first; v < v_end; v += v_step) {
+            const int nt = v % args.tiles_n;
+            const int mt = (v / args.tiles_n) * cs + crank;
             const int w0 = (mt % args.tiles_w) * C::kTW;
             const int h0 = ((mt / args.tiles_w) % args.tiles_h) * C::kTH;
             const int b0 = mt / (args.tiles_w * args.tiles_h);
@@ -697,7 +704,7 @@
         int sh = 0, sw = 0;
         uint32_t ph = 0, pw = 0;
         int iter = 0;
-        for (int tile = blockIdx.x; tile < total_tiles; tile += gridDim.x, ++iter) {
+        for (int v = v_first; v < v_end; v += v_step, ++iter) {
             const int as = iter & 1;
             const uint32_t aphase = (iter >> 1) & 1;
             ptx::mbar_wait(&tempty_bar[as], aphase ^ 1, err, 3300 + as);
@@ -752,10 +759,13 @@
         constexpr int kTwLog2 = kW16 ? 4 : 3;
         const int q = warp & 3;
         const int half = warp >= 8 ? 1 : 0;
+        const int gcg = args.gn_cg;
+        float* gn_red = reinterpret_cast<float*>(reinterpret_cast<uint8_t*>(bars) + 256);
+        float* gn_slot = gn_red + 16;
         int iter = 0;
-        for (int tile = blockIdx.x; tile < total_tiles; tile += gridDim.x, ++iter) {
-            const int nt = tile % args.tiles_n;
-            const int mt = tile / args.tiles_n;
+        for (int v = v_first; v < v_end; v += v_step, ++iter) {
+            const int nt = v % args.tiles_n;
+            const int mt = (v / args.tiles_n) * cs + crank;
             const int w0 = (mt % args.tiles_w) * C::kTW;
             const int h0 = ((mt / args.tiles_w) % args.tiles_h) * C::kTH;
             const int b = mt / (args.tiles_w * args.tiles_h);
@@ -793,6 +803,96 @@
                                         (long long)(i & (C::kTW - 1)) * args.out_sw;
                     if (args.out_f32) args.out_f32[o] = f;
                     if (args.out_f16) args.out_f16[o] = sat_half(f);
+                    if (i < 16) v0[i] = __float_as_uint(f); else v1[i - 16] = __float_as_uint(f);
+                }
+                if (gcg) {
+                    ptx::tmem_st_x16(taddr + c, v0);
+                    ptx::tmem_st_x16(taddr + c + 16, v1);
+                }
+            }
+            if (gcg) {
+                ptx::tmem_st_wait();
+                const int wi = half * 4 + q;
+                const int nq = gcg >> 5;
+                const int q0 = (q / nq) * nq;
+                const float n_loc = (float)(gcg * kHtPix);
+                float s = st_s;
+#pragma unroll
+                for (int o = 16; o >= 1; o >>= 1) s += __shfl_xor_sync(0xffffffffu, s, o);
+                if (lane == 0) gn_red[wi] = s;
+                ptx::named_bar_sync(1, 32 * kEpiWarps);
+                float gsum = 0.f;
+                for (int qq = q0; qq < q0 + nq; ++qq) gsum += gn_red[qq] + gn_red[4 + qq];
+                const float mean_loc = gsum / n_loc;
+                float m2 = 0.f;
+#pragma unroll 1
+                for (int c = 0; c < 128; c += 32) {
+                    uint32_t v0[16], v1[16];
+                    ptx::tmem_ld_x16(taddr + c, v0);
+                    ptx::tmem_ld_x16(taddr + c + 16, v1);
+                    ptx::tmem_ld_wait();
+#pragma unroll
+                    for (int i = 0; i < 32; ++i) {
+                        const float d = __uint_as_float(i < 16 ? v0[i] : v1[i - 16]) - mean_loc;
+                        m2 = fmaf(d, d, m2);
+                    }
+                }
+#pragma unroll
+                for (int o = 16; o >= 1; o >>= 1) m2 += __shfl_xor_sync(0xffffffffu, m2, o);
+                if (lane == 0) gn_red[8 + wi] = m2;
+                ptx::named_bar_sync(1, 32 * kEpiWarps);
+                float mean = mean_loc, M2 = 0.f, cnt = n_loc;
+                for (int qq = q0; qq < q0 + nq; ++qq) M2 += gn_red[8 + qq] + gn_red[12 + qq];
+                if (cs > 1) {
+                    float* slot = gn_slot + as * 32;
+                    if (threadIdx.x == 128) {
+                        for (int g = 0; g < 4 / nq; ++g) {
+                            float gs = 0.f, gm = 0.f;
+                            for (int qq = g * nq; qq < (g + 1) * nq; ++qq) {
+                                gs += gn_red[qq] + gn_red[4 + qq];
+                                gm += gn_red[8 + qq] + gn_red[12 + qq];
+                            }
+                            for (int r = 0; r < cs; ++r) ptx::st_cluster_f32x2(slot + (crank * 4 + g) * 2, r, gs / n_loc, gm);
+                        }
+                        for (int r = 0; r < cs; ++r) ptx::mbar_arrive_release_cluster(&gnx_bar[as], r);
+                    }
+                    ptx::mbar_wait_acquire_cluster(&gnx_bar[as], aphase, err, 3700 + as);
+                    const int g = q / nq;
+                    mean = slot[g * 2];
+                    M2 = slot[g * 2 + 1];
+                    for (int r = 1; r < cs; ++r) {
+                        const float mb = slot[(r * 4 + g) * 2], m2b = slot[(r * 4 + g) * 2 + 1];
+                        const float tot = cnt + n_loc;
+                        const float d = mb - mean;
+                        mean += d * (n_loc / tot);
+                        M2 += m2b + d * d * (cnt * n_loc / tot);
+                        cnt = tot;
+                    }
+                }
+                const float rstd = 1.0f / sqrtf(M2 / cnt + args.gn_eps);
+                float ga = rstd * __ldg(args.gn_gamma + n);
+                float gb = __ldg(args.gn_beta + n) - mean * ga;
+                if (args.gn_ss) {
+                    const float sc = args.gn_ss[(long long)b * args.gn_ss_ld + n] + 1.0f;
+                    const float sf = args.gn_ss[(long long)b * args.gn_ss_ld + args.tiles_n * 128 + n];
+                    ga *= sc;
+                    gb = gb * sc + sf;
+                }
+#pragma unroll 1
+                for (int c = 0; c < 128; c += 32) {
+                    uint32_t v0[16], v1[16];
+                    ptx::tmem_ld_x16(taddr + c, v0);
+                    ptx::tmem_ld_x16(taddr + c + 16, v1);
+                    const long long rowb = base + (long long)(c >> kTwLog2) * args.out_sh;
+                    ptx::tmem_ld_wait();
+#pragma unroll
+                    for (int i = 0; i < 32; ++i) {
+                        float y = fmaf(__uint_as_float(i < 16 ? v0[i] : v1[i - 16]), ga, gb);
+                        y = __fdividef(y, 1.0f + __expf(-y));
+                        const long long o = rowb + (long long)(i >> kTwLog2) * args.out_sh +
+                                            (long long)(i & (C::kTW - 1)) * args.out_sw;
+                        args.gn_out[o] = sat_half(y);
+                    }
                 }
             }
             if (args.stats) {
@@ -812,7 +912,8 @@
         }
     }
     ptx::tc_fence_before();
-    __syncthreads();
+    if (cs > 1) ptx::cluster_sync_all();
+    else __syncthreads();
     if (warp == 2) {
         ptx::tc_fence_after();
         ptx::tmem_dealloc(tmem_base, C::kTmemCols);
@@ -903,8 +1004,31 @@
             return -10;
         attr_set = true;
     }
-    const int grid = total_tiles < num_sms ? total_tiles : num_sms;
-    launch_k(conv3x3_halo_t_kernel<G>, grid, kNumThreads, C::kSmemBytes, stream, tmA, tmA2, tmB, tmX, tmX2, args);
+    const int cs = args.gn_cluster > 1 ? args.gn_cluster : 1;
+    int grid = total_tiles < num_sms ? total_tiles : num_sms;
+    if (cs > 1) {
+        static int max_clusters = 0;
+        if (max_clusters == 0) {
+            cudaLaunchConfig_t cfg{};
+            cfg.gridDim = dim3(num_sms / cs * cs);
+            cfg.blockDim = dim3(kNumThreads);
+            cfg.dynamicSmemBytes = C::kSmemBytes;
+            cudaLaunchAttribute attr[1];
+            attr[0].id = cudaLaunchAttributeClusterDimension;
+            attr[0].val.clusterDim.x = cs;
+            attr[0].val.clusterDim.y = 1;
+            attr[0].val.clusterDim.z = 1;
+            cfg.attrs = attr;
+            cfg.numAttrs = 1;
+            int n = 0;
+            if (cudaOccupancyMaxActiveClusters(&n, conv3x3_halo_t_kernel<G>, &cfg) != cudaSuccess || n < 1) return -13;
+            max_clusters = n;
+        }
+        const int items = total_tiles / cs;
+        grid = cs * (items < max_clusters ? items : max_clusters);
+    }
+    launch_k_cluster(conv3x3_halo_t_kernel<G>, cs, grid, kNumThreads, C::kSmemBytes, stream, tmA, tmA2, tmB, tmX, tmX2,
+                     args);
     return cudaGetLastError() == cudaSuccess ? 0 : -11;
 }
 
@@ -926,6 +1050,9 @@
         case -9: return "conv_tc: folded 1x1 operand needs the swapped-operand 3x3 kernel (C_out % 128, H % 32 / W % 8 or 16x16 tiles)";
         case -10: return "conv_tc: cudaFuncSetAttribute(max dynamic smem) failed";
         case -11: return "conv_tc: kernel launch failed";
+        case -12: return "conv_tc: GroupNorm epilogue needs a 3x3 conv on 16x16 or 32x32 images, C_out % 128 == 0 and "
+                         "C_out / groups in {32, 64, 128} (see conv_gn_epilogue_supported)";
+        case -13: return "conv_tc: cudaOccupancyMaxActiveClusters failed for the GroupNorm cluster form";
         default: return "conv_tc: unknown error";
     }
 }
@@ -939,11 +1066,22 @@
     return ilog2_exact(H) >= 0;
 }
 
+bool conv_gn_epilogue_supported(int H, int W, int Cout, int groups) {
+    if (!((H == 16 && W == 16) || (H == 32 && W == 32))) return false;
+    if (Cout <= 0 || Cout % 128 != 0 || groups <= 0 || Cout % groups != 0) return false;
+    const int cg = Cout / groups;
+    return cg == 32 || cg == 64 || cg == 128;
+}
+
 int conv_tc_launch(const ConvTcProblem& p, cudaStream_t stream) {
     if (p.Cin <= 0 || p.Cin % kConvBlockK != 0) return -1;
     if (p.Cout % 16 != 0) return -2;
     if (p.num_taps < 1 || p.num_taps > kConvMaxTaps) return -4;
     if (!conv_tc_supported(p.H, p.W, p.Cin, p.Cout)) return -3;
+    if (p.gn_out && (!conv_gn_epilogue_supported(p.H, p.W, p.Cout, p.gn_groups) || p.halo != 1 || p.num_taps != 9 ||
+                     p.phases != 1 || p.out_sc > 1 || (p.n_valid != 0 && p.n_valid != p.Cout) || p.dbg != 0 ||
+                     !p.gn_gamma || !p.gn_beta))
+        return -12;
     if ((reinterpret_cast<uintptr_t>(p.act) & 15) || (reinterpret_cast<uintptr_t>(p.wpacked) & 15) ||
         (p.lda % 8) != 0)
         return -8;
@@ -973,6 +1111,12 @@
             h.out_f32 = p.out_f32; h.out_f16 = p.out_f16; h.bias = p.bias; h.residual = p.residual; h.err_flag = p.err_flag;
             h.stats = p.stats; h.stats_blocks = p.Cout / 16;
             h.dh[0] = p.dh[0]; h.dw[0] = p.dw[0];
+            if (p.gn_out) {
+                h.gn_cg = p.Cout / p.gn_groups;
+                h.gn_cluster = t16 ? 1 : h.tiles_w * h.tiles_h;
+                h.gn_gamma = p.gn_gamma; h.gn_beta = p.gn_beta; h.gn_ss = p.gn_ss; h.gn_ss_ld = p.gn_ss_ld;
+                h.gn_eps = p.gn_eps; h.gn_out = p.gn_out;
+            }
             int dev = 0, num_sms = 148;
             cudaGetDevice(&dev);
             cudaDeviceGetAttribute(&num_sms, cudaDevAttrMultiProcessorCount, dev);
@@ -1039,6 +1183,7 @@
     }
 
     if (p.x_act) return -9;
+    if (p.gn_out) return -12;
 
     if (p.halo && !p.act2 && p.num_taps == 9 && p.phases == 1 && p.H % kHaloTH == 0 && p.W % kHaloTW == 0 &&
         ((p.Cout % 128 == 0 && (p.halo == 2 || p.Cout % 256 != 0)) ||
diff --git a/minimagen_b200/csrc/conv_tc.cuh b/minimagen_b200/csrc/conv_tc.cuh
--- a/minimagen_b200/csrc/conv_tc.cuh
+++ b/minimagen_b200/csrc/conv_tc.cuh
@@ -31,6 +31,14 @@
     double* stats;
     int stats_blocks;
     int8_t dh[kConvMaxTaps], dw[kConvMaxTaps], ph[kConvMaxTaps];
+    int gn_cg;
+    int gn_cluster;
+    const float* gn_gamma;
+    const float* gn_beta;
+    const float* gn_ss;
+    long long gn_ss_ld;
+    float gn_eps;
+    __half* gn_out;
 };
 
 struct ConvTcProblem {
@@ -61,6 +69,9 @@
     int dbg;
     double* stats;
     int* err_flag;
+    int gn_groups;
+    const float* gn_gamma; const float* gn_beta; const float* gn_ss; long long gn_ss_ld; float gn_eps;
+    __half* gn_out;
 };
 
 struct GnPrologueArgs {
@@ -95,6 +106,7 @@
 int conv_gn_pair_launch(const ConvGnProblem& p, cudaStream_t stream);
 
 bool conv_tc_supported(int H, int W, int Cin, int Cout);
+bool conv_gn_epilogue_supported(int H, int W, int Cout, int groups);
 int conv_tc_launch(const ConvTcProblem& p, cudaStream_t stream);
 const char* conv_tc_strerror(int code);
 
diff --git a/minimagen_b200/csrc/launch.cuh b/minimagen_b200/csrc/launch.cuh
--- a/minimagen_b200/csrc/launch.cuh
+++ b/minimagen_b200/csrc/launch.cuh
@@ -13,19 +13,36 @@
 }
 
 template <typename... KArgs, typename... Args>
-inline cudaError_t launch_k(void (*kernel)(KArgs...), dim3 grid, dim3 block, size_t smem, cudaStream_t stream,
-                            Args&&... args) {
+inline cudaError_t launch_k_cluster(void (*kernel)(KArgs...), int cluster_x, dim3 grid, dim3 block, size_t smem,
+                                    cudaStream_t stream, Args&&... args) {
     cudaLaunchConfig_t cfg{};
     cfg.gridDim = grid;
     cfg.blockDim = block;
     cfg.dynamicSmemBytes = smem;
     cfg.stream = stream;
-    cudaLaunchAttribute attr[1];
-    attr[0].id = cudaLaunchAttributeProgrammaticStreamSerialization;
-    attr[0].val.programmaticStreamSerializationAllowed = 1;
+    cudaLaunchAttribute attr[2];
+    int n = 0;
+    if (pdl_enabled()) {
+        attr[n].id = cudaLaunchAttributeProgrammaticStreamSerialization;
+        attr[n].val.programmaticStreamSerializationAllowed = 1;
+        ++n;
+    }
+    if (cluster_x > 1) {
+        attr[n].id = cudaLaunchAttributeClusterDimension;
+        attr[n].val.clusterDim.x = cluster_x;
+        attr[n].val.clusterDim.y = 1;
+        attr[n].val.clusterDim.z = 1;
+        ++n;
+    }
     cfg.attrs = attr;
-    cfg.numAttrs = pdl_enabled() ? 1 : 0;
+    cfg.numAttrs = n;
     return cudaLaunchKernelEx(&cfg, kernel, static_cast<KArgs>(args)...);
 }
 
+template <typename... KArgs, typename... Args>
+inline cudaError_t launch_k(void (*kernel)(KArgs...), dim3 grid, dim3 block, size_t smem, cudaStream_t stream,
+                            Args&&... args) {
+    return launch_k_cluster(kernel, 1, grid, block, smem, stream, static_cast<Args&&>(args)...);
 }
+
+}
diff --git a/minimagen_b200/csrc/ptx.cuh b/minimagen_b200/csrc/ptx.cuh
--- a/minimagen_b200/csrc/ptx.cuh
+++ b/minimagen_b200/csrc/ptx.cuh
@@ -217,6 +217,19 @@
         }
     }
 }
+__device__ __forceinline__ void st_cluster_f32x2(const void* p, uint32_t cta, float a, float b) {
+    asm volatile(
+        "{\n\t"
+        ".reg .b32 remAddr32;\n\t"
+        "mapa.shared::cluster.u32 remAddr32, %0, %1;\n\t"
+        "st.shared::cluster.v2.f32 [remAddr32], {%2, %3};\n\t"
+        "}"
+        ::"r"(smem_u32(p)), "r"(cta), "f"(a), "f"(b)
+        : "memory");
+}
+__device__ __forceinline__ void named_bar_sync(uint32_t id, uint32_t count) {
+    asm volatile("bar.sync %0, %1;" ::"r"(id), "r"(count) : "memory");
+}
 __device__ __forceinline__ void tma_load_2d_2sm(const CUtensorMap* m, uint64_t* bar, void* dst, int c0, int c1) {
     asm volatile(
         "cp.async.bulk.tensor.2d.cta_group::2.shared::cluster.global.mbarrier::complete_tx::bytes [%0], [%1, {%3, %4}], "
diff --git a/minimagen_b200/layers.py b/minimagen_b200/layers.py
--- a/minimagen_b200/layers.py
+++ b/minimagen_b200/layers.py
@@ -62,11 +62,11 @@
 
 
 class Act:
-    __slots__ = ("f32", "f16", "stats")
-
-    def __init__(self, f32=None, f16=None, stats=None):
-        assert f32 is not None or f16 is not None
-        self.f32, self.f16, self.stats = f32, f16, stats
+    __slots__ = ("f32", "f16", "stats", "gn_pre")
+
+    def __init__(self, f32=None, f16=None, stats=None, gn_pre=None):
+        assert f32 is not None or f16 is not None or gn_pre is not None
+        self.f32, self.f16, self.stats, self.gn_pre = f32, f16, stats, gn_pre
 
     @property
     def any(self):
@@ -74,14 +74,21 @@
 
     @property
     def shape(self):
-        sh = self.any.shape
+        sh = (self.any if self.any is not None else self.gn_pre[2]).shape
         return (sh[0], sh[-3], sh[-2], sh[-1])
 
     @property
     def device(self):
-        return self.any.device
+        return (self.any if self.any is not None else self.gn_pre[2]).device
+
+    def pre_applied(self, gn, scale_shift):
+        pre = self.gn_pre
+        if pre is not None and pre[0] is gn and pre[1] is scale_shift:
+            return pre[2]
+        return None
 
     def need_f32(self):
+        assert self.any is not None, "only the GroupNorm-applied operand of this activation exists"
         if self.f32 is None:
             B, H, W, C = self.shape
             self.f32 = torch.empty((B, H, W, C), dtype=F32, device=self.device)
@@ -89,6 +96,7 @@
         return self.f32
 
     def need_f16(self):
+        assert self.any is not None, "only the GroupNorm-applied operand of this activation exists"
         if self.f16 is None:
             B, H, W, C = self.shape
             self.f16 = torch.empty((B, 1, H, W, C), dtype=F16, device=self.device)
@@ -350,7 +358,7 @@
         return Act(o32, o16, st)
 
     def run_prepared(self, a, B, H, W, residual=None, f32=True, f16=False, stats=False, a2=None, c_in1=0, wp=None,
-                     in_place_s2=False):
+                     in_place_s2=False, gn_next=None):
         ops = get_ops()
         Cin, Cout = self.in_channels, self.out_channels
         kh, kw = self.kernel_size
@@ -359,15 +367,22 @@
         if a.dtype == F16:
             mode = (6 if in_place_s2 else 1) if self._geom == 'down' else 0
             st = stats_zeros((B, Cout // STATS_BLOCK, 2), dev) if (stats and Cout % 32 == 0 and (H * W) % 32 == 0) else None
-            if not f32 and not f16:
+            if not f32 and not f16 and gn_next is None:
                 f32 = True
             o32 = torch.empty((B, H, W, Cout), dtype=F32, device=dev) if f32 else None
             o16 = torch.empty((B, 1, H, W, Cout), dtype=F16, device=dev) if f16 else None
             lda = a.shape[-1]
+            gn_kw, pre = {}, None
+            if gn_next is not None:
+                gn, ss = gn_next
+                g16 = torch.empty((B, 1, H, W, Cout), dtype=F16, device=dev)
+                gn_kw = dict(gn_groups=gn.num_groups, gn_gamma=gn.weight, gn_beta=gn.bias, gn_scale_shift=ss,
+                             gn_ss_ld=ss.stride(0) if exists(ss) else 0, gn_eps=gn.eps, gn_out=g16)
+                pre = (gn, ss, g16)
             ops.conv_igemm(a, B, H, W, lda, 0, Cin, wp if exists(wp) else self._pack.get(self.weight), Cout, kh, kw, mode,
                            self.bias, residual, o32, o16, strides, act2=a2, lda2=a2.shape[-1] if exists(a2) else 0,
-                           c_in1=c_in1, out_stats=st)
-            return Act(o32, o16, st)
+                           c_in1=c_in1, out_stats=st, **gn_kw)
+            return Act(o32, o16, st, gn_pre=pre)
         out = torch.empty((B, H, W, Cout), dtype=F32, device=dev)
         Hin, Win = a.shape[1], a.shape[2]
         ops.conv_direct(a, B, Hin, Win, Cin, a.shape[3], self.weight.detach(), Cout, kh, kw, self.stride[0],
@@ -584,12 +599,25 @@
         self.activation = nn.SiLU()
         self.project = Conv2d(dim, dim_out, 3, padding=1)
 
-    def run(self, x, scale_shift=None, residual=None, f32=True, f16=False, stats=False, fold=None):
+    def gn_epilogue_ok(self, H, W, gn):
+        conv = self.project
+        supported = getattr(get_ops(), "conv_gn_epilogue_supported", None)
+        return (supported is not None and not FUSE_GN_CONV and conv.tc_ok(H, W) and conv.in_channels % 64 == 0
+                and supported(H, W, conv.out_channels, gn.num_groups))
+
+    def run(self, x, scale_shift=None, residual=None, f32=True, f16=False, stats=False, fold=None, gn_next=None):
         ops = get_ops()
         x = as_act(x)
         B, H, W, C = x.shape
         gn = self.groupnorm
         assert isinstance(gn, nn.GroupNorm), "Block(norm=False) is never instantiated by the U-Net"
+        if gn_next is not None and (fold is not None or not self.gn_epilogue_ok(H, W, gn_next[0])):
+            gn_next = None
+        a = x.pre_applied(gn, scale_shift) if isinstance(x, Act) else None
+        if a is not None:
+            if fold is not None:
+                return self.project.run_folded(a, B, H, W, fold[0], fold[1], residual, f32=f32, f16=f16, stats=stats)
+            return self.project.run_prepared(a, B, H, W, residual, f32=f32, f16=f16, stats=stats, gn_next=gn_next)
         G = gn.num_groups
         Cg = C // G
         tc = self.project.tc_ok(H, W)
@@ -627,7 +655,7 @@
                           gn.eps, a)
         if fold is not None:
             return self.project.run_folded(a, B, H, W, fold[0], fold[1], residual, f32=f32, f16=f16, stats=stats)
-        return self.project.run_prepared(a, B, H, W, residual, f32=f32, f16=f16, stats=stats)
+        return self.project.run_prepared(a, B, H, W, residual, f32=f32, f16=f16, stats=stats, gn_next=gn_next)
 
     def forward(self, x, scale_shift=None):
         _no_grad_check(x)
@@ -652,7 +680,7 @@
         self.block2 = Block(dim_out, dim_out, groups=groups)
         self.res_conv = Conv2d(dim, dim_out, 1) if dim != dim_out else Identity()
 
-    def run(self, x, time_emb=None, cond=None, scale_shift=None, out_f32=True):
+    def run(self, x, time_emb=None, cond=None, scale_shift=None, out_f32=True, gn_next=None):
         ops = get_ops()
         B = x.shape[0]
         if not exists(scale_shift) and exists(self.time_mlp) and exists(time_emb):
@@ -664,7 +692,13 @@
         tc = self.block1.project.tc_ok(x.shape[1], x.shape[2]) and self.block2.project.tc_ok(x.shape[1], x.shape[2])
         attn = exists(self.cross_attn)
         keep32 = attn or not tc or GN_INPUT_F32
-        h = self.block1.run(x, f32=keep32, f16=not keep32, stats=tc and not attn)
+        gn2 = None
+        if not attn and self.block1.gn_epilogue_ok(x.shape[1], x.shape[2], self.block2.groupnorm):
+            gn2 = (self.block2.groupnorm, scale_shift)
+        if gn2 is not None:
+            h = self.block1.run(x, f32=False, f16=False, stats=False, gn_next=gn2)
+        else:
+            h = self.block1.run(x, f32=keep32, f16=not keep32, stats=tc and not attn)
         if attn:
             assert exists(cond)
             h = self.cross_attn.run(h, context=cond)
@@ -683,7 +717,8 @@
                 return self.block2.run(h, scale_shift, residual=None, f32=out_f32 or not tc, f16=tc, stats=tc,
                                        fold=(x, self.res_conv))
             res = self.res_conv.run(x, f32=True).f32
-        return self.block2.run(h, scale_shift, residual=res, f32=out_f32 or not tc, f16=tc, stats=tc)
+        return self.block2.run(h, scale_shift, residual=res, f32=out_f32 or not tc, f16=tc, stats=tc,
+                               gn_next=(gn_next, None) if gn_next is not None else None)
 
     def forward(self, x, time_emb=None, cond=None):
         _no_grad_check(x)
diff --git a/minimagen_b200/ops.py b/minimagen_b200/ops.py
--- a/minimagen_b200/ops.py
+++ b/minimagen_b200/ops.py
@@ -48,14 +48,27 @@
         return out
 
     def conv_igemm(self, act, B, H, W, lda, c_off, c_in, wp, c_out, kh, kw, mode, bias, residual, out_f32, out_f16,
-                   out_strides, block_n=0, out_sc=1, n_valid=0, act2=None, lda2=0, c_off2=0, c_in1=0, out_stats=None):
+                   out_strides, block_n=0, out_sc=1, n_valid=0, act2=None, lda2=0, c_off2=0, c_in1=0, out_stats=None,
+                   gn_groups=0, gn_gamma=None, gn_beta=None, gn_scale_shift=None, gn_ss_ld=0, gn_eps=1e-5, gn_out=None):
         _chk(act, F16, "act"); _chk(act2, F16, "act2"); _chk(wp, F16, "wp"); _chk(bias, F32, "bias")
         _chk_out(residual, F32, "residual"); _chk_out(out_f32, F32, "out_f32"); _chk_out(out_f16, F16, "out_f16")
         _chk(out_stats, F64, "out_stats")
         sb, sh, sw = out_strides
+        if gn_out is not None:
+            _chk_out(gn_out, F16, "gn_out"); _chk(gn_gamma, F32, "gn_gamma"); _chk(gn_beta, F32, "gn_beta")
+            _chk_out(gn_scale_shift, F32, "gn_scale_shift")
+            N.call("mi_conv2d_igemm_gn_f16", N.ptr(act), B, H, W, lda, c_off, c_in, N.ptr(act2), lda2, c_off2, c_in1,
+                   N.ptr(wp), c_out, kh, kw, mode, N.ptr(bias), N.ptr(residual), N.ptr(out_f32), N.ptr(out_f16),
+                   N.ptr(out_stats), sb, sh, sw, out_sc, n_valid, block_n, None, None, 0, int(gn_groups),
+                   N.ptr(gn_gamma), N.ptr(gn_beta), N.ptr(gn_scale_shift), int(gn_ss_ld), float(gn_eps), N.ptr(gn_out),
+                   N.stream())
+            return
         N.call("mi_conv2d_igemm_f16", N.ptr(act), B, H, W, lda, c_off, c_in, N.ptr(act2), lda2, c_off2, c_in1,
                N.ptr(wp), c_out, kh, kw, mode, N.ptr(bias), N.ptr(residual), N.ptr(out_f32), N.ptr(out_f16),
                N.ptr(out_stats), sb, sh, sw, out_sc, n_valid, block_n, None, None, 0, N.stream())
+
+    def conv_gn_epilogue_supported(self, H, W, c_out, groups):
+        return bool(N.load().mi_conv_gn_epilogue_supported(int(H), int(W), int(c_out), int(groups)))
 
     def conv_res1x1_supported(self, H, W, c_in, c_out, x_cin):
         return bool(N.load().mi_conv3x3_res1x1_supported(int(H), int(W), int(c_in), int(c_out), int(x_cin)))
```

Measured after the change: 36.45 (median of 6 runs). 1.5% higher.
